# king159/Pair-Net

Measured on AMD Instinct MI355X. Metric: images/sec (whole node), 100-query 800x1333, 1/2/4/8 MI355X, higher is better.
Workload: dtype f32

## Files before the change

### include/pairnet_hip.h

```cpp
#ifndef PAIRNET_HIP_H_
#define PAIRNET_HIP_H_

#include <stdint.h>

#ifdef __cplusplus
extern "C" {
#endif

#define PN_ABI_VERSION 29
int pn_abi_version(void);

#define PN_GEMM_RELU       1
#define PN_GEMM_A_COLMAJOR 2
#define PN_GEMM_FORCE_TILE 4
#define PN_GEMM_FORCE_SKINNY 8
#define PN_GEMM_FORCE_TILE64 16
#define PN_GEMM_FORCE_TILE128x64 32
#define PN_GEMM_RELU_AFTER_RES 128
#define PN_GEMM_GELU 256
#define PN_GEMM_RESERVE_SHIFT 16
#define PN_GEMM_RESERVE(n) ((((n) / 8) & 0x3ff) << PN_GEMM_RESERVE_SHIFT)
#define PN_GEMM_KSPLIT_SHIFT 26
#define PN_GEMM_KSPLIT(n) (((n) & 31) << PN_GEMM_KSPLIT_SHIFT)

typedef struct pn_gemm_desc {
  const float* A;     int64_t lda;    int64_t strideA;
  const float* Aadd;  int64_t ldaadd; int32_t aadd_rows;
  int32_t aadd_from_col;
  const float* W;     int64_t ldw;    int64_t strideW;
  const float* bias;
  const float* Res;   int64_t ldres;  int64_t strideRes;
  float*       C;     int64_t ldc;    int64_t strideC;
  int32_t M, N, K, batch, flags;
  float* splitk_scratch;  int64_t splitk_scratch_floats;
} pn_gemm_desc;

int pn_gemm_f32(const pn_gemm_desc* d, void* stream);

int pn_gemm_group_f32(const pn_gemm_desc* d, int count, void* stream);

int pn_gemm_wgs_per_cu(void);

#define PN_GEMM_VARIANT_SKINNY        0
#define PN_GEMM_VARIANT_TILE_128x64   2
#define PN_GEMM_VARIANT_TILE_128x128  4
#define PN_GEMM_VARIANT_TILE_64x64    6
int pn_gemm_variant(const pn_gemm_desc* d);
int pn_gemm_grid_size(const pn_gemm_desc* d);

int pn_conv2d_nhwc_f32(const float* in, const float* Wp, const float* bias,
                       float* out, int B, int H, int W, int Cin, int Cout,
                       int KH, int KW, int pad, int relu, int flags , void* stream);

int pn_winograd_f23_input_f32(const float* in, float* V, int B, int H, int W, int C,
                              void* stream);
int pn_winograd_f23_output_f32(const float* M, const float* bias, float* out, int B, int H,
                               int W, int C, int relu, void* stream);
int pn_winograd_weights_f32(const float* w, float* U, int Co, int Ci, int form, void* stream);
int pn_winograd_f43_input_f32(const float* in, float* V, int B, int H, int W, int C,
                              void* stream);
int pn_winograd_f43_output_f32(const float* M, const float* bias, float* out, int B, int H,
                               int W, int C, int relu, void* stream);

int pn_conv2d_nhwc_ex_f32(const float* in, const float* Wp, const float* bias,
                          const float* res, float* out, int B, int H, int W, int Cin,
                          int Cout, int KH, int KW, int stride, int pad, int flags,
                          float* splitk_scratch ,
                          int64_t splitk_scratch_floats, void* stream);
int pn_stem7x7s2_f32(const float* img_nchw, const float* Wp, const float* bias,
                     float* out, int B, int H, int W, int flags ,
                     void* stream);
int pn_maxpool3x3s2_nhwc_f32(const float* in, float* out, int B, int H, int W, int C,
                             void* stream);

int pn_layernorm_f32(const float* x, const float* gamma, const float* beta,
                     float* y, int64_t rows, int C, float eps, void* stream);

int pn_layernorm_rows_f32(const float* x, int64_t ldx, const float* gamma, const float* beta,
                          float* y, int64_t ldy, int64_t rows, int C, float eps, void* stream);
int pn_layernorm_rows_s3_f32(const float* x, int64_t ldx, const float* gamma, const float* beta,
                             void* y_s3, int64_t rows, int C, float eps, void* stream);

int pn_patch_merge_ln_f32(const float* x, const float* gamma, const float* beta, float* y,
                          int B, int H, int W, int C, float eps, void* stream);

int pn_patch_im2col4_f32(const float* img, float* out, int B, int H, int W, void* stream);

int pn_window_attention_f32(const float* qkv, int64_t ldqkv, const float* qkv_bias,
                            const float* bias_table, float* out, int64_t ldo, int B, int H,
                            int W, int C, int heads, int ws, int shift, float scale,
                            void* stream);
int pn_window_attention_s3_f32(const float* qkv, int64_t ldqkv, const float* qkv_bias,
                               const float* bias_table, void* out_s3, int B, int H, int W, int C,
                               int heads, int ws, int shift, float scale, void* stream);

int pn_groupnorm_nblk(int64_t HW);
int pn_groupnorm_nhwc_f32(const float* x, const float* gamma, const float* beta,
                          float* y, double* partials, int B, int64_t HW, int C,
                          int G, float eps, int relu, int64_t x_bstride,
                          int64_t y_bstride, void* stream);

int pn_linear_res_ln_f32(const float* x, int64_t ldx, const float* W, int64_t ldw,
                         const float* bias , const float* res, int64_t ldres,
                         const float* gamma, const float* beta, float* y, int64_t ldy,
                         int M, int N, int K, float eps, void* stream);

int64_t pn_ffn_scratch_floats(int M, int hidden);
int pn_ffn_ln_f32(const float* x, const float* W1, const float* b1, const float* W2,
                  const float* b2, const float* gamma, const float* beta, float* y,
                  float* scratch, int M, int C, int hidden, float eps, void* stream);
int pn_ffn_ln2_f32(const float* x, const float* W1, const float* b1, const float* W2,
                   const float* b2, const float* gamma, const float* beta, float* y,
                   const float* gamma2, const float* beta2, float* y2, float* scratch, int M,
                   int C, int hidden, float eps, void* stream);

int pn_l2normalize_f32(const float* x, float* y, int64_t rows, int C, float eps,
                       void* stream);

int pn_msda_f32(const float* value, int64_t ld_value, const float* offaw,
                int64_t ld_offaw, float* out, int B, int L,
                const int32_t* level_h , const int32_t* level_w ,
                void* stream);
#define PN_MSDA_PERSISTENT 1
#define PN_MSDA_PERSISTENT_BATCHED 2
#define PN_MSDA_LOW_OCCUPANCY 4
#define PN_MSDA_S3_OUT 8
int pn_msda_ex_f32(const float* value, int64_t ld_value, const float* offaw,
                   int64_t ld_offaw, float* out, int B, int L,
                   const int32_t* level_h , const int32_t* level_w ,
                   int flags, void* stream);

int pn_msda_loc_f32(const float* value, int64_t ld_value, const int64_t* spatial_shapes,
                    const int64_t* level_start_index, const float* sampling_locations,
                    const float* attention_weights, float* out, int B, int N, int Nq, int L,
                    void* stream);

int pn_msda_bwd_f32(const float* value, int64_t ld_value, const int64_t* spatial_shapes,
                    const int64_t* level_start_index, const float* sampling_locations,
                    const float* attention_weights, const float* grad_output, float* grad_value,
                    float* grad_sampling_loc, float* grad_attn_weight, int B, int N, int Nq, int L,
                    void* stream);

int pn_gather_probe_f32(const float* lines, const int32_t* idx, float* out, int workgroups,
                        int line_mask, void* stream);

int pn_sine_pe_f32(float* out, const float* add, int h, int w, int C,
                   float temperature, void* stream);
int pn_sine_pe_offset_f32(float* out, const float* add, int h, int w, int C, float temperature,
                          float offset, void* stream);
int pn_sine_pe_valid_f32(float* out, const float* add, int h, int w, int valid_h, int valid_w,
                         int C, float temperature, float offset, void* stream);

int pn_bilinear_nhwc_f32(const float* in, float* out, int B, int hi, int wi,
                         int ho, int wo, int C, int accumulate, int64_t in_bstride,
                         int64_t out_bstride, void* stream);
int pn_bilinear_planar_f32(const float* in, float* out, int64_t P, int hi,
                           int wi, int ho, int wo, void* stream);
int pn_bilinear_stencil_rows_f32(const float* in, float* out, int B, int hi, int wi, int ho,
                                 int wo, int C, int64_t in_bstride, int64_t out_bstride,
                                 void* stream);
int pn_bilinear_planar_gt0_u8(const float* in, uint8_t* out, int64_t P, int hi,
                              int wi, int ho, int wo, void* stream);

int pn_mask_pack(const float* logits, uint32_t* bits, int32_t* rowall,
                 int64_t R, int Nk, void* stream);
int pn_mask_pack_stencil(const float* logits4, uint32_t* bits, int32_t* rowall, int64_t R,
                         int hi, int wi, int ho, int wo, void* stream);

int pn_mask_stencil_gemm_f32(const float* me, int64_t ld_me, int64_t stride_me, const float* rows,
                             int64_t ld_rows, int64_t stride_rows, uint32_t* bits,
                             int32_t* rowall, int B, int Q, int Nk, int K, int hi, int wi, int ho,
                             int wo, int flags, void* stream);

int64_t pn_attn_scratch_floats(int B, int Q, int Nk);
int pn_attention_f32(const float* q, int64_t ldq, const float* k, int64_t ldk,
                     const float* v, int64_t ldv, const uint32_t* maskbits,
                     const int32_t* rowall, float* out, int64_t ldo,
                     float* scratch, int B, int Q, int Nk, float scale,
                     void* stream);

int pn_mlearner_first_f32(const float* in, const float* w1, const float* b1,
                          float* out, int B, int S, int C, void* stream);
int pn_ppn_front_f32(const float* sub_embed, const float* obj_embed, const float* w1,
                     const float* b1, float* importance_raw, float* c1, int B, int Q, float eps,
                     void* stream);
int pn_mlearner_last_f32(const float* in, const float* w3, const float* b3,
                         float* out, int B, int S, int C, void* stream);

int pn_topk_pairs(const float* scores, int64_t* idx, int64_t* sub, int64_t* obj,
                  int64_t* pair, int B, int Q, int k, void* stream);
int pn_topk_f32(const float* scores, int64_t* idx, int64_t* quot, int64_t* rem, int B,
                int n, int div, int k, void* stream);
int pn_topk_strided_f32(const float* scores, int64_t elem_stride, int64_t row_stride,
                        int64_t* idx, int64_t* quot, int64_t* rem, int B, int n, int div, int k,
                        void* stream);

int pn_gather_rows_f32(const float* in, const int64_t* index, float* out, int B,
                       int rows_in, int rows_out, int64_t len, void* stream);

int pn_cls_argmax_f32(const float* logits, int64_t* label, float* score,
                      int64_t rows, int C, int label_offset, void* stream);
int pn_rel_dists_f32(const float* logits, float* out, int64_t rows, int C,
                     void* stream);
int pn_softmax_fg_f32(const float* logits, float* probs, float* fg, int64_t rows,
                      int C, void* stream);
int pn_row_argmax_f32(const float* x, int64_t* idx, int64_t rows, int n,
                      void* stream);
int pn_triplet_finish(const int64_t* s_label, const int64_t* o_label,
                      const float* probs, const int64_t* tri, const int64_t* rem,
                      int64_t* labels, int64_t* r_labels, float* r_scores,
                      float* r_dists, int k, int C, void* stream);
int pn_panoptic_f32(const float* masks, const int64_t* labels,
                    const int32_t* remap, int64_t* seg, int32_t* area, int n,
                    int64_t HW, void* stream);

int64_t pn_panoptic_state_bytes(void);
int pn_panoptic_device_f32(const float* masks, const int64_t* labels, const float* scores,
                           int Q, int num_classes, int hi, int wi, int ho, int wo,
                           void* state, float* up_scratch, int32_t* area_scratch,
                           int64_t* seg, int rounds, void* stream);
int pn_panoptic_continue_f32(void* state, const float* up_scratch, int32_t* area_scratch,
                             int64_t* seg, int ho, int wo, int rounds, void* stream);

int pn_pack_triplets_f32(const int64_t* labels, const float* r_dists, const int64_t* sub_pos,
                         const int64_t* obj_pos, float* rec, int R, int C1, void* stream);

int pn_copy_stream(const void* src, void* dst, int64_t bytes, int wgs, void* stream);

int pn_pack_bool_bits(const uint8_t* bools, uint8_t* bits, int64_t n, void* stream);
int pn_unpack_bits_host(const uint8_t* bits, uint8_t* bools, int64_t n, int threads);

int pn_pan_masks_u8(const uint8_t* rgb, const int* ids, const int* cats, uint8_t* masks, int* sem,
                    int G, int H, int W, void* stream);

int pn_preprocess_u8_f32(const uint8_t* img, int H, int W, float* out, int Hn, int Wn, int Hp,
                         int Wp, const float* mean3, const float* stdinv3, int to_rgb,
                         void* stream);

int pn_pack_mask_bits(const uint8_t* masks, uint64_t* words, int64_t rows, int64_t HW,
                      void* stream);
int pn_mask_iou_counts(const uint64_t* pred_words, int P, const uint64_t* gt_words, int G,
                       int64_t nwords, int32_t* inter, int32_t* area_pred, int32_t* area_gt,
                       void* stream);

int pn_pred_triplets(const int64_t* labels, const float* r_dists, int32_t* triplets,
                     float* scores, int R, int C1, void* stream);
int pn_mask_or_rows(const uint64_t* words, const int32_t* a, const int32_t* b, uint64_t* out,
                    int rows, int64_t nwords, void* stream);
int pn_triplet_match(const int32_t* pred_triplets, const int32_t* gt_triplets, int P, int G,
                     const int32_t* inter, const int32_t* area_pred, const int32_t* area_gt,
                     int ld_inter, const int32_t* pred_sub_row, const int32_t* pred_obj_row,
                     const int32_t* gt_sub_row, const int32_t* gt_obj_row, double iou_thr,
                     int phrdet, int ignore_rel, uint8_t* match, void* stream);
int pn_triplet_match_boxes(const int32_t* pred_triplets, const int32_t* gt_triplets, int P, int G,
                           const float* pred_boxes, int ld_pred, const float* gt_boxes, int ld_gt,
                           const int32_t* pred_sub_row, const int32_t* pred_obj_row,
                           const int32_t* gt_sub_row, const int32_t* gt_obj_row, float iou_thr,
                           int phrdet, int ignore_rel, uint8_t* match, void* stream);

int pn_zero_rows_f32(const float* x, const uint8_t* valid, float* out, int B, int64_t rows,
                     int C, int64_t ld, int64_t valid_bstride, void* stream);
int pn_sigmoid_f32(const float* x, float* y, int64_t n, void* stream);
int pn_box_pos_embed_f32(const float* unact, float* ref, float* emb, int64_t rows, void* stream);
int pn_box_sampling_f32(const float* offaw, int64_t ld, const float* ref,
                        const float* valid_ratios, int rows_per_image, float* loc, float* aw,
                        int64_t rows, int L, void* stream);
int pn_token_sampling_f32(const float* offaw, int64_t ld, const float* valid_ratios, float* loc,
                          float* aw, int B, int L, const int32_t* level_h, const int32_t* level_w,
                          void* stream);
int pn_box_refine_f32(const float* delta, const float* ref_in, float* ref_out, int64_t rows,
                      void* stream);
int pn_query_score_f32(const float* logits, float* score, int B, int Nq, int C, void* stream);
int pn_box_triplets_f32(const float* s_cls, const float* o_cls, const float* s_box,
                        const float* o_box, float* det, int64_t* labels, int R, int C,
                        float img_h, float img_w, const float* scale_factor, int rescale,
                        void* stream);

int pn_gt_mask_prepare_u8(const uint8_t* masks, uint8_t* out, int G, int h, int w, int H, int W,
                          int Ho, int Wo, void* stream);

int pn_point_sample_f32(const void* maps, int maps_are_u8, const float* pts, float* out, int P,
                        int h, int w, int Np, void* stream);
int pn_mask_match_cost_f32(const float* cls , int ncls,
                           const int64_t* gt_labels , const float* pred_pts ,
                           const float* gt_pts , float* cost, int Q, int G, int Np,
                           float w_cls, float w_mask, float w_dice, float dice_eps, void* stream);
int pn_id_match_cost_f32(const float* sub, const float* obj , const float* rel
                         , int ncls, int nrel, const int64_t* gt_sub,
                         const int64_t* gt_obj, const int64_t* gt_rel, float* cost, int R, int G,
                         float w_sub, float w_obj, float w_rel, void* stream);
int pn_ce_mean_f32(const float* logits, int64_t ld, const int64_t* target,
                   const float* class_weight , float* out, int rows, int C,
                   float loss_weight, void* stream);
int pn_seesaw_mean_f32(const float* logits, int64_t ld, const int64_t* target,
                       const float* cum_samples, float* out, int rows, int C, float p, float q,
                       float eps, float loss_weight, void* stream);
int pn_bce_posw_mean_f32(const float* logits, const float* target, float* out , int64_t n,
                         float loss_weight, void* stream);

int pn_ce_mean_grad_f32(const float* logits, int64_t ld, const int64_t* target,
                        const float* class_weight , float* grad, int64_t ldg,
                        int rows, int C, float loss_weight, void* stream);
int pn_seesaw_mean_grad_f32(const float* logits, int64_t ld, const int64_t* target,
                            const float* cum_samples, float* grad, int64_t ldg, int rows, int C,
                            float p, float q, float eps, float loss_weight, void* stream);
int pn_bce_posw_mean_grad_f32(const float* logits, const float* target, float* grad, int64_t n,
                              float loss_weight, void* stream);

int pn_transpose_f32(const float* in, int64_t ldi, float* out, int64_t ldo, int rows, int cols,
                     int out_cols, void* stream);
int pn_colsum_f32(const float* x, int64_t ld, float* out, int rows, int cols, int accumulate,
                  float* scratch, int64_t scratch_floats, void* stream);
int pn_relu_bwd_f32(const float* dy, const float* y, float* dx, int64_t n, void* stream);
int pn_add_periodic_f32(const float* a, const float* b, float* out, int64_t n, int64_t bn,
                        void* stream);
int pn_batch_sum_f32(const float* x, float* out, int B, int64_t n, int accumulate, void* stream);
int pn_layernorm256_bwd_f32(const float* dy, const float* x, const float* gamma, float* dx,
                            float* gxhat, int rows, float eps, void* stream);
int pn_mha_bwd_f32(const float* q, int64_t ldq, const float* k, int64_t ldk, const float* v,
                   int64_t ldv, const float* dout, int64_t ldo, float* dq, int64_t lddq, float* dk,
                   int64_t lddk, float* dv, int64_t lddv, const uint32_t* bits,
                   const int32_t* rowall, float* scratch, int B, int Nq, int Nk, float scale,
                   void* stream);
int pn_scatter_rows_add_f32(const float* src, int64_t ld_src, const int64_t* index, float* out,
                            int64_t ld_out, int B, int rows_out, int slots, int length,
// ... 65 lines not shown
```

### pair-net_amd/backbone.py

```python
from collections import OrderedDict

import torch

from . import hip
from . import plans
from .plans import Arena, PlanCache, measure_bytes

BLOCKS = {50: (3, 4, 6, 3), 101: (3, 4, 23, 3)}
EPS = 1e-5


def _stages(depth):
    return tuple(zip((64, 128, 256, 512), BLOCKS[depth]))


def _param_shapes(depth=50):
    STAGES = _stages(depth)
    s = OrderedDict()

    def bn(prefix, c):
        for n in ("weight", "bias", "running_mean", "running_var"):
            s["%s.%s" % (prefix, n)] = (c,)
        s[prefix + ".num_batches_tracked"] = ()

    s["conv1.weight"] = (64, 3, 7, 7)
    bn("bn1", 64)
    cin = 64
    for i, (planes, blocks) in enumerate(STAGES):
        for b in range(blocks):
            p = "layer%d.%d." % (i + 1, b)
            s[p + "conv1.weight"] = (planes, cin, 1, 1)
            bn(p + "bn1", planes)
            s[p + "conv2.weight"] = (planes, planes, 3, 3)
            bn(p + "bn2", planes)
            s[p + "conv3.weight"] = (planes * 4, planes, 1, 1)
            bn(p + "bn3", planes * 4)
            if b == 0:
                s[p + "downsample.0.weight"] = (planes * 4, cin, 1, 1)
                bn(p + "downsample.1", planes * 4)
            cin = planes * 4
    return s


class ResNet50Hip:

    def __init__(self, depth=50, **unused):
        if depth not in BLOCKS:
            raise NotImplementedError("bottleneck ResNets: depth 50 or 101")
        self.depth, self.stages = depth, _stages(depth)
        self._params = OrderedDict(
            (k, torch.zeros(shape, dtype=torch.int64 if k.endswith("tracked") else torch.float32))
            for k, shape in _param_shapes(depth).items())
        for k, v in self._params.items():
            if k.endswith(("running_var",)) or (k.endswith(".weight") and v.dim() == 1):
                v.fill_(1.0)
        g = torch.Generator().manual_seed(0)
        for k, v in self._params.items():
            if v.dim() == 4:
                fan_in = v.shape[1] * v.shape[2] * v.shape[3]
                v.copy_(torch.randn(v.shape, generator=g) * (2.0 / fan_in) ** 0.5)
        self.device, self.w, self._plans, self._arenas = None, None, PlanCache(), {}
        self.use_graphs = False
        self.graph_after = 1
        self.grid_reserve = 0
        self.conv_algo = "winograd4"
        self.wino_min_planes = 128
        self.s3_conv3_min_planes = 0

    def _weights_version(self):
        return sum(p._version for p in self._params.values())

    def parameters(self):
        return list(self._params.values())

    def state_dict(self):
        return OrderedDict((k, v.clone()) for k, v in self._params.items())

    def load_state_dict(self, sd, strict=True):
        missing = [k for k in self._params if k not in sd]
        unexpected = [k for k in sd if k not in self._params]
        if strict and (missing or unexpected):
            raise RuntimeError("state_dict mismatch: missing %s unexpected %s"
                               % (missing[:5], unexpected[:5]))
        for k, p in self._params.items():
            if k in sd:
                if tuple(sd[k].shape) != tuple(p.shape):
                    raise RuntimeError("shape mismatch for %s" % k)
                p.copy_(sd[k].detach().to(p.dtype).cpu())
        self.w, self._plans = None, PlanCache()
        return missing, unexpected

    def to(self, device):
        self.device, self.w, self._plans = torch.device(device), None, PlanCache()
        self._arenas = {}
        return self

    def eval(self):
        return self

    def _fold(self, conv, bn):
        P = self._params
        w = P[conv + ".weight"].double()
        s = P[bn + ".weight"].double() / torch.sqrt(P[bn + ".running_var"].double() + EPS)
        b = P[bn + ".bias"].double() - P[bn + ".running_mean"].double() * s
        w = (w * s.view(-1, 1, 1, 1)).float()
        return w, b.float()

    def _pack(self):
        if self.device is None or self.device.type != "cuda":
            raise RuntimeError("ResNet50Hip runs on an MI355X only: call .to('cuda:0'); there "
                               "is no CPU path")
        hip.lib()
        dev, w = self.device, {}
        cw, cb = self._fold("conv1", "bn1")
        stem = torch.zeros(64, 160)
        stem[:, :147] = cw.reshape(64, 147)
        w["stem.w"], w["stem.b"] = stem.to(dev), cb.to(dev)
        for i, (planes, blocks) in enumerate(self.stages):
            for b in range(blocks):
                p = "layer%d.%d." % (i + 1, b)
                for conv, bn in (("conv1", "bn1"), ("conv2", "bn2"), ("conv3", "bn3"),
                                 ("downsample.0", "downsample.1")):
                    if p + conv + ".weight" not in self._params:
                        continue
                    cw, cb = self._fold(p + conv, p + bn)
                    co = cw.shape[0]
                    w[p + conv + ".w"] = cw.permute(0, 2, 3, 1).reshape(co, -1).contiguous().to(dev)
                    w[p + conv + ".b"] = cb.to(dev)
                    if conv == "conv2" and co >= 64 and not (b == 0 and i > 0):
                        w[p + "conv2.wino"] = hip.winograd_weights(cw.to(dev))
                        w[p + "conv2.wino4"] = hip.winograd43_weights(cw.to(dev))
        for k in list(w):
            if k.endswith("conv3.w"):
                s3 = torch.empty(hip.s3_floats(*w[k].shape), device=dev, dtype=torch.float32)
                hip.s3_split(w[k], s3)
                w[k + ".s3"] = s3
        self.w = w
        self._packed_version = self._weights_version()

    class _Plan:

        def busy_events(self):
            out = []
            for st in self.streams.values():
                ev = torch.cuda.Event()
                ev.record(st)
                out.append(ev)
            return out

    def _arena(self, slot):
        a = self._arenas.get(slot)
        if a is None:
            a = self._arenas[slot] = Arena(self.device, on_grow=lambda a, s=slot: self._plans.drop(
                lambda k: k[3] == s))
        return a

    def _layout_for(self, dims):
        def layout(E):
            pl = ResNet50Hip._Plan()
            self._layout(pl, E, *dims)
            return pl
        return layout

    def _measure(self, dims):
        return measure_bytes(self._layout_for(dims))

    def reserve(self, batch, H, W, slots=(0,)):
        if self.w is None:
            self._pack()
        for s in slots:
            self._arena(s).reserve((batch, H, W), self._measure)

    def arena_bytes(self):
        return sum(a.capacity for a in self._arenas.values())

    @staticmethod
    def feature_shapes(H, W):
        h, w = (H - 1) // 2 + 1, (W - 1) // 2 + 1
        out = []
        for i in range(4):
            h, w = (h - 1) // 2 + 1, (w - 1) // 2 + 1
            out.append((h, w))
        return out

    def _plan(self, B, H, W, slot=0):
        key = (B, H, W, slot, self.conv_algo, self.wino_min_planes, self.s3_conv3_min_planes)
        if key in self._plans:
            return self._plans[key]
        if self.w is None:
            self._pack()

        dims = (B, H, W)
        pl = self._arena(slot).carve(self._layout_for(dims), dims, self._measure)
        pl.graph = pl.outs = pl.last_img = None
        pl.calls, pl.staged, pl.streams = 0, False, {}
        self._plans[key] = pl
        return pl

    def _layout(self, pl, E, B, H, W):
        pl.B = B
        pl.img = E(B, 3, H, W)
        h1, w1 = (H - 1) // 2 + 1, (W - 1) // 2 + 1
        h, wd = (h1 - 1) // 2 + 1, (w1 - 1) // 2 + 1
        pl.stem, pl.hw_stem = E(B, h1, w1, 64), (h1, w1)
        pl.pool = E(B, h, wd, 64)
        pl.scratch = E(B * 16 * 1024 * 1024 // 2)
        pl.hw, pl.out, pl.t1, pl.t2, pl.idt, pl.ping, pl.f43 = [], [], [], [], [], [], []
        nwino = 0
        for i, (planes, blocks) in enumerate(self.stages):
            hin, win = h, wd
            if i > 0:
                h, wd = (h - 1) // 2 + 1, (wd - 1) // 2 + 1
            pl.hw.append(((hin, win), (h, wd)))
            pl.t1.append(E(B, hin, win, planes))
            pl.t2.append(E(B, h, wd, planes))
            pl.idt.append(E(B, h, wd, planes * 4))
            pl.ping.append(E(B, h, wd, planes * 4))
            pl.out.append(E(B, h, wd, planes * 4))
            if planes >= self.wino_min_planes:
                t2, t4 = B * ((h + 1) // 2) * ((wd + 1) // 2), B * ((h + 3) // 4) * ((wd + 3) // 4)
                nwino = max(nwino, 16 * t2 * planes, 36 * t4 * planes)
                pl.f43.append(36 * (-(-t4 // 64)) < 16 * (-(-t2 // 64)))
            else:
                pl.f43.append(False)
        pl.wV, pl.wM = E(max(nwino, 4)), E(max(nwino, 4))
        pl.t2_s3 = E(max(hip.s3_floats(B * hw[1][0] * hw[1][1], planes)
                         for hw, (planes, _) in zip(pl.hw, self.stages)))

    @torch.no_grad()
    @hip.on_device
    def forward(self, img, slot=0):
        if not img.is_cuda or img.dtype != torch.float32 or img.dim() != 4 or img.shape[1] != 3:
            raise RuntimeError("img must be a [B,3,H,W] fp32 device tensor")
        if self.device is None:
            self.to(img.device)
        if self.w is not None and self._packed_version != self._weights_version():
            self.w, self._plans = None, PlanCache(self._plans.max_plans)
        img = img.contiguous()
        B, _, H, W = img.shape
        pl = self._plan(B, H, W, slot)
        if getattr(pl, "reserve", None) != self.grid_reserve:
            pl.reserve, pl.graph = self.grid_reserve, None
        cur = torch.cuda.current_stream(self.device)
        pl.streams[cur.cuda_stream] = cur
        try:
            return self._forward_on(img, pl, cur)
        finally:
            plans.note_use(cur)

    def _forward_on(self, img, pl, cur):
        if not self.use_graphs:
            return self._run(img, pl)
        ptr = img.data_ptr()
        if pl.graph is not None and not pl.staged and ptr != pl.static_img.data_ptr():
            pl.graph, pl.staged = None, True
        if pl.graph is None:
            if pl.calls < self.graph_after or not plans.quiet(cur):
                pl.calls += 1
                pl.last_img = ptr
                return self._run(img, pl)
            if not pl.staged and pl.last_img is not None and ptr != pl.last_img:
                pl.staged = True
            pl.static_img = pl.img if pl.staged else img
            pl.graph, pl.outs = self._capture(lambda: self._run(pl.static_img, pl))
        pl.last_img = ptr
        if pl.staged:
            pl.static_img.copy_(img)
        pl.graph.replay()
        return pl.outs

    @staticmethod
    def _capture(fn):
        from .head import CrossHead2
        box = {}
        g = CrossHead2._capture(lambda: box.update(out=fn()))
        return g, box["out"]

    def _run(self, img, pl):
        with hip.reserve_slots(self.grid_reserve):
            return self._run_layers(img, pl)

    def _run_layers(self, img, pl):
        B, _, H, W = img.shape
        w = self.w
        hip.stem7x7s2(img, w["stem.w"], w["stem.b"], pl.stem, B, H, W)
        hip.maxpool3x3s2(pl.stem, pl.pool, B, pl.hw_stem[0], pl.hw_stem[1], 64)
        x, cin = pl.pool, 64
        for i, (planes, blocks) in enumerate(self.stages):
            (hin, win), (h, wd) = pl.hw[i]
            for b in range(blocks):
                p = "layer%d.%d." % (i + 1, b)
                stride = 2 if (b == 0 and i > 0) else 1
                hi, wi = (hin, win) if b == 0 else (h, wd)
                t1 = pl.t1[i].view(-1)[:B * hi * wi * planes].view(B, hi, wi, planes)
                hip.linear(x.view(-1, cin), w[p + "conv1.w"], w[p + "conv1.b"],
                           t1.view(-1, planes), relu=True, scratch=pl.scratch)
                wino = self.conv_algo in ("winograd", "winograd4") and p + "conv2.wino" in w \
                    and stride == 1 and planes >= self.wino_min_planes
                if wino and self.conv_algo == "winograd4" and pl.f43[i]:
                    hip.conv3x3_winograd43(t1, w[p + "conv2.wino4"], w[p + "conv2.b"], pl.t2[i],
                                           pl.wV, pl.wM, B, hi, wi, planes, planes, True)
                elif wino:
                    hip.conv3x3_winograd(t1, w[p + "conv2.wino"], w[p + "conv2.b"], pl.t2[i],
                                         pl.wV, pl.wM, B, hi, wi, planes, planes, True)
                else:
                    hip.conv2d_ex(t1, w[p + "conv2.w"], w[p + "conv2.b"], None, pl.t2[i], B, hi,
                                  wi, planes, planes, 3, 3, stride, 1, relu=True,
                                  scratch=pl.scratch)
                if b == 0:
                    if stride == 1:
                        hip.linear(x.view(-1, cin), w[p + "downsample.0.w"],
                                   w[p + "downsample.0.b"], pl.idt[i].view(-1, planes * 4),
                                   scratch=pl.scratch)
                    else:
                        hip.conv2d_ex(x, w[p + "downsample.0.w"], w[p + "downsample.0.b"], None,
                                      pl.idt[i], B, hi, wi, cin, planes * 4, 1, 1, stride, 0,
                                      scratch=pl.scratch)
                    idt = pl.idt[i]
                else:
                    idt = x
                if b == blocks - 1:
                    dst = pl.out[i]
                else:
                    dst = pl.ping[i] if idt is not pl.ping[i] else pl.idt[i]
                if self.s3_conv3_min_planes and planes >= self.s3_conv3_min_planes:
                    t2 = pl.t2[i].view(-1, planes)
                    hip.s3_split(t2, pl.t2_s3)
                    hip.gemm_s3(pl.t2_s3, w[p + "conv3.w.s3"], t2.shape[0], planes * 4, planes,
                                bias=w[p + "conv3.b"], out=dst.view(-1, planes * 4),
                                res=idt.view(-1, planes * 4), relu_after=True)
                else:
                    hip.linear(pl.t2[i].view(-1, planes), w[p + "conv3.w"], w[p + "conv3.b"],
                               dst.view(-1, planes * 4), res=idt.view(-1, planes * 4),
                               relu_after=True, scratch=pl.scratch)
                x, cin = dst, planes * 4
        return tuple(o.permute(0, 3, 1, 2) for o in pl.out)

    __call__ = forward
```

### pair-net_amd/csrc/gemm.hip

```cpp
#include "common.h"
#include "gemm_common.h"

#ifndef PN_GEMM_WGS64
#define PN_GEMM_WGS64 5
#endif
#ifndef PN_GEMM_WGS128x64
#define PN_GEMM_WGS128x64 3
#endif
#ifndef PN_GEMM_BIGM_128x64
#define PN_GEMM_BIGM_128x64 0
#endif
#ifndef PN_GEMM_WGS64_SPILLING
#define PN_GEMM_WGS64_SPILLING 5
#endif

#ifndef PN_GEMM_LDS2
#define PN_GEMM_LDS2 0
#endif

template <int BM, int BN, int AMODE>
struct TileSmem {
  static constexpr int A_ELEMS = (AMODE == A_COL) ? 32 * (BM + 4) : BM * 36;
  static constexpr int STAGE = A_ELEMS + BN * 36;
  static constexpr int FLOATS = STAGE * (PN_GEMM_LDS2 ? 2 : 1);
};

#ifndef PN_GEMM_W2
#define PN_GEMM_W2 0
#endif
#ifndef PN_GEMM_W2_WGS
#define PN_GEMM_W2_WGS 8
#endif

template <int BM, int BN, int AMODE, bool ADD>
struct TileWgs {
  static constexpr int value =
      (BM * BN > 128 * 64) ? 2 : (BM * BN > 64 * 64) ? PN_GEMM_WGS128x64
      : ((AMODE == A_ROW && !ADD) || AMODE == A_CONV) ? PN_GEMM_WGS64 : PN_GEMM_WGS64_SPILLING;
  static constexpr int min_waves = (BM * BN <= 64 * 64 && value > 4) ? value : 1;
};

struct TileRef {
  int pi;
  int bz, tm, tn;
};

template <int BM, int BN, int WM, int WN, int AMODE, bool ADD, typename Locator, int EPI = 0>
__device__ __forceinline__ void gemm_persistent(const Locator& loc, const int ntiles,
                                                float* smem) {
  constexpr int BK = 32, LD = BK + 4;
  constexpr int WAVES_N = BN / WN;
  constexpr int TM = WM / 32, TN = WN / 32;
  constexpr int LDK = BM + 4;
  constexpr int A_ELEMS = TileSmem<BM, BN, AMODE>::A_ELEMS;
  constexpr int NT = 64 * (BM / WM) * WAVES_N;
  constexpr int RPP = NT / 8;
  constexpr int NA = (BM * BK / 4) / NT;
  constexpr int NB = (BN * BK / 4) / NT;
  constexpr int QM = BM / 4;
  constexpr int KSTEP = NT / QM;
  static_assert(NT == 128 || NT == 256 || NT == 512, "2, 4 or 8 waves");

  const int xcd = blockIdx.x & 7, slot = blockIdx.x >> 3, per = gridDim.x >> 3;
  const int q8 = ntiles >> 3, r8 = ntiles & 7;
  const int base = (xcd < r8) ? xcd * (q8 + 1) : r8 * (q8 + 1) + (xcd - r8) * q8;
  const int cnt = q8 + (xcd < r8 ? 1 : 0);
  if (slot >= cnt) return;

  const int tid = threadIdx.x, lane = tid & 63, wave = tid >> 6;
  const int li = lane & 31, lh = lane >> 5;
  const int wm = wave / WAVES_N, wn = wave % WAVES_N;
  const int kc = (tid & 7) * 4;
  float* const sA = smem;
  float* const sB = smem + A_ELEMS;

  int lpi = 0, lK = 0, lkt0 = 0;
  const float* bA = nullptr;
  const float* bW = nullptr;
  const float* bAdd = nullptr;
  __amdgpu_buffer_rsrc_t rA = make_rsrc(nullptr), rW = rA, rAdd = rA;
  unsigned a_off[NA], add_off[ADD ? NA : 1], w_off[NB];
  int cy[NA], cx[NA];
  unsigned a_tap[AMODE == A_CONV ? NA : 1];
  unsigned a_off1[AMODE == A_COL ? NA : 1][4];
  unsigned in_mask = 0;
  bool l_add = false;
  bool l_vec = false;
  auto set_tile = [&](const TileRef& tr) {
    const GemmP& p = loc.P(tr.pi);
    lpi = tr.pi;
    lK = p.K;
    const int m0 = tr.tm * BM, n0 = tr.tn * BN;
    const int ks = max(p.ksplit, 1);
    const int bb = tr.bz / ks;
    lkt0 = (tr.bz - bb * ks) * p.split_chunks;
    bA = p.A + (int64_t)bb * p.sA;
    bW = p.W + (int64_t)bb * p.sW;
    bAdd = p.Aadd ? p.Aadd : bA;
    rA = make_rsrc(bA);
    rW = make_rsrc(bW);
    if (ADD) rAdd = make_rsrc(bAdd);
    l_add = p.Aadd && n0 >= p.aadd_from_col;
    l_vec = p.a_vec && m0 + BM <= p.M;
    if (AMODE == A_COL) {
      const int mq = m0 + (tid % QM) * 4;
#pragma unroll
      for (int j = 0; j < NA; ++j) {
        const unsigned krow = (unsigned)(min(tid / QM + KSTEP * j, p.K - 1)) * (unsigned)p.lda;
        a_off[j] = (krow + (unsigned)min(mq, p.M - 1)) * 4u;
#pragma unroll
        for (int e = 0; e < 4; ++e) a_off1[j][e] = (krow + (unsigned)min(mq + e, p.M - 1)) * 4u;
      }
    } else {
#pragma unroll
      for (int j = 0; j < NA; ++j) {
        const int gm = min(m0 + (tid >> 3) + RPP * j, p.M - 1);
        if (AMODE == A_CONV) {
          const int oy = gm / p.Wo, ox = gm - oy * p.Wo;
          cy[j] = oy * p.stride;
          cx[j] = ox * p.stride;
          a_off[j] = ((unsigned)(cy[j] * p.Wd + cx[j]) * (unsigned)p.Cin + kc) * 4u;
        } else {
          a_off[j] = ((unsigned)gm * (unsigned)p.lda + kc) * 4u;
        }
        if (ADD) add_off[j] = ((unsigned)(p.Aadd ? gm % p.aadd_rows : gm) *
                                   (unsigned)(p.Aadd ? p.ldaadd : p.lda) + kc) * 4u;
      }
    }
    if constexpr (EPI == 1) {
      const StencilP& st = loc.st;
#pragma unroll
      for (int j = 0; j < NB; ++j) {
        const int c = (tid >> 3) + RPP * j;
        const int key = min(tr.tn * 16 + (c >> 5) * 8 + (c & 7), st.nk - 1);
        w_off[j] = ((unsigned)(((c >> 3) & 3) * st.nk + key) * (unsigned)p.ldw + kc) * 4u;
      }
    } else {
#pragma unroll
      for (int j = 0; j < NB; ++j)
        w_off[j] = ((unsigned)min(n0 + (tid >> 3) + RPP * j, p.N - 1) * (unsigned)p.ldw + kc) * 4u;
    }
  };

  float4 ra[NA], rad[ADD ? NA : 1], rb[NB];
  bool st_ragged = false, st_add = false;
  int st_k0 = 0;
  unsigned st_in = 0;
  auto load_chunk = [&](int kt) {
    const int k0 = (lkt0 + kt) * BK;
    const bool ragged = k0 + BK > lK;
    st_ragged = ragged;
    st_add = l_add;
    st_k0 = k0;
    if (AMODE == A_COL) {
      const GemmP& p = loc.P(lpi);
      const int soff = (ragged ? 0 : k0) * (int)p.lda * 4;
      if (l_vec) {
#pragma unroll
        for (int j = 0; j < NA; ++j) ra[j] = buf_ld4(rA, a_off[j], soff);
      } else {
#pragma unroll
        for (int j = 0; j < NA; ++j) {
          ra[j].x = buf_ld1(rA, a_off1[j][0], soff);
          ra[j].y = buf_ld1(rA, a_off1[j][1], soff);
          ra[j].z = buf_ld1(rA, a_off1[j][2], soff);
          ra[j].w = buf_ld1(rA, a_off1[j][3], soff);
        }
      }
    } else if (AMODE == A_CONV) {
      const GemmP& p = loc.P(lpi);
      const int tap = k0 / p.Cin;
      const int ci0 = k0 - tap * p.Cin;
      const int dy = tap / p.KW - p.pad, dx = tap % p.KW - p.pad;
      if (ci0 == 0 || kt == 0) {
        in_mask = 0;
        const int tap_off = (dy * p.Wd + dx) * p.Cin;
#pragma unroll
        for (int j = 0; j < NA; ++j) {
          const int yy = cy[j] + dy, xx = cx[j] + dx;
          const bool in = yy >= 0 && yy < p.H && xx >= 0 && xx < p.Wd;
          in_mask |= (in ? 1u : 0u) << j;
          a_tap[j] = a_off[j] + (unsigned)(in ? tap_off : 0) * 4u;
        }
      }
      st_in = in_mask;
#pragma unroll
      for (int j = 0; j < NA; ++j) ra[j] = buf_ld4(rA, a_tap[j], ci0 * 4);
    } else {
#pragma unroll
      for (int j = 0; j < NA; ++j) ra[j] = buf_ld4(rA, a_off[j], ragged ? 0 : k0 * 4);
      if (ADD) {
#pragma unroll
        for (int j = 0; j < NA; ++j)
          rad[j] = buf_ld4(rAdd, add_off[j], ragged ? 0 : k0 * 4);
      }
    }
#pragma unroll
    for (int j = 0; j < NB; ++j) rb[j] = buf_ld4(rW, w_off[j], ragged ? 0 : k0 * 4);
  };
  auto store_chunk = [&](const int so = 0) {
    float* const sA = smem + so;
    float* const sB = smem + so + A_ELEMS;
    const float4 zero4 = make_float4(0.f, 0.f, 0.f, 0.f);
#pragma unroll
    for (int j = 0; j < NA; ++j) {
      if (ADD && st_add) ra[j] = add4(ra[j], rad[j]);
      if (AMODE == A_CONV && !((st_in >> j) & 1u)) ra[j] = zero4;
    }
    if (st_ragged) {
      const GemmP& p = loc.P(lpi);
#pragma unroll
      for (int j = 0; j < NA; ++j) {
        if (AMODE == A_COL) {
          const int kk = st_k0 + tid / QM + KSTEP * j;
          const int mq = (int)(a_off1[j][0] / 4u) - (int)min(tid / QM + KSTEP * j, lK - 1) * (int)p.lda;
          float4 v = zero4;
          if (kk < lK) {
            const float* src = bA + (int64_t)kk * p.lda;
            v.x = src[min(mq + 0, p.M - 1)];
            v.y = src[min(mq + 1, p.M - 1)];
            v.z = src[min(mq + 2, p.M - 1)];
            v.w = src[min(mq + 3, p.M - 1)];
          }
          ra[j] = v;
        } else if (AMODE == A_ROW) {
          const bool ok = st_k0 + kc < lK;
          float4 v = ok ? ld4(bA + st_k0 + a_off[j] / 4u) : zero4;
          if (ADD && st_add && ok) v = add4(v, ld4(bAdd + st_k0 + add_off[j] / 4u));
          ra[j] = v;
        } else {
          ra[j] = zero4;
        }
      }
      (void)p;
#pragma unroll
      for (int j = 0; j < NB; ++j)
        rb[j] = st_k0 + kc < lK ? ld4(bW + st_k0 + w_off[j] / 4u) : zero4;
    }
    if (AMODE == A_COL) {
#pragma unroll
      for (int j = 0; j < NA; ++j)
        st4(sA + (tid / QM + KSTEP * j) * LDK + (tid % QM) * 4, ra[j]);
#pragma unroll
      for (int j = 0; j < NB; ++j) st4(sB + ((tid >> 3) + RPP * j) * LD + kc, rb[j]);
    } else {
#pragma unroll
      for (int j = 0; j < NA; ++j) st4(sA + ((tid >> 3) + RPP * j) * LD + kc, ra[j]);
#pragma unroll
      for (int j = 0; j < NB; ++j) st4(sB + ((tid >> 3) + RPP * j) * LD + kc, rb[j]);
    }
  };

  f32x16 acc[TM][TN];
  const float* fA0 = (AMODE == A_COL) ? sA + (4 * lh) * LDK + wm * WM + li
                                      : sA + (wm * WM + li) * LD + 4 * lh;
  const float* fB0 = sB + (wn * WN + li) * LD + 4 * lh;
  int rso = 0;
  auto read_frag = [&](int kb, float4 (&fa)[TM], float4 (&fb)[TN]) {
    const float* const fA = fA0 + rso;
    const float* const fB = fB0 + rso;
#pragma unroll
    for (int mi = 0; mi < TM; ++mi) {
      if (AMODE == A_COL) {
        const float* s = fA + (kb * 8) * LDK + mi * 32;
        fa[mi] = make_float4(s[0], s[LDK], s[2 * LDK], s[3 * LDK]);
      } else {
        fa[mi] = ld4(fA + mi * 32 * LD + kb * 8);
      }
    }
#pragma unroll
    for (int ni = 0; ni < TN; ++ni) fb[ni] = ld4(fB + ni * 32 * LD + kb * 8);
  };
  auto compute = [&]() {
    float4 fa[2][TM], fb[2][TN];
    read_frag(0, fa[0], fb[0]);
#pragma unroll
    for (int kb = 0; kb < BK / 8; ++kb) {
      const int cur = kb & 1;
      if (kb + 1 < BK / 8) read_frag(kb + 1, fa[cur ^ 1], fb[cur ^ 1]);
#pragma unroll
      for (int t = 0; t < 4; ++t)
#pragma unroll
        for (int mi = 0; mi < TM; ++mi)
#pragma unroll
          for (int ni = 0; ni < TN; ++ni) {
            const float4 av = fa[cur][mi], bv = fb[cur][ni];
            acc[mi][ni] = mfma32(t == 0 ? av.x : t == 1 ? av.y : t == 2 ? av.z : av.w,
                                 t == 0 ? bv.x : t == 1 ? bv.y : t == 2 ? bv.z : bv.w,
                                 acc[mi][ni]);
          }
    }
  };

  TileRef cur = loc(base + slot);
  set_tile(cur);
  load_chunk(0);
#if PN_GEMM_LDS2
  constexpr int STAGE = TileSmem<BM, BN, AMODE>::STAGE;
  int wso = 0;
  {
    const GemmP& p0 = loc.P(cur.pi);
    int nk0 = (p0.K + BK - 1) / BK;
    if (p0.ksplit > 1) nk0 = min(p0.split_chunks, nk0 - (cur.bz % p0.ksplit) * p0.split_chunks);
    store_chunk(0);
    wso = STAGE;
    if (nk0 > 1) {
      load_chunk(1);
    } else {
      set_tile(loc(base + min(slot + per, cnt - 1)));
      load_chunk(0);
    }
    __syncthreads();
  }
#endif
  for (int t = slot; t < cnt; t += per) {
    const GemmP& p = loc.P(cur.pi);
    const TileRef nxt = loc(base + min(t + per, cnt - 1));
    int nk = (p.K + BK - 1) / BK;
    if (p.ksplit > 1) {
      const int sidx = cur.bz % p.ksplit;
      nk = min(p.split_chunks, nk - sidx * p.split_chunks);
    }
#pragma unroll
    for (int mi = 0; mi < TM; ++mi)
#pragma unroll
      for (int ni = 0; ni < TN; ++ni)
#pragma unroll
        for (int r = 0; r < 16; ++r) acc[mi][ni][r] = 0.f;
#if PN_GEMM_LDS2
    for (int kt = 0; kt < nk; ++kt) {
      store_chunk(wso);
      if (kt + 2 < nk) {
        load_chunk(kt + 2);
      } else if (kt + 2 == nk) {
        set_tile(nxt);
        load_chunk(0);
      } else {
        const GemmP& pn = loc.P(nxt.pi);
        int nkn = (pn.K + BK - 1) / BK;
        if (pn.ksplit > 1) nkn = min(pn.split_chunks, nkn - (nxt.bz % pn.ksplit) * pn.split_chunks);
        if (nkn > 1) {
          load_chunk(1);
        } else {
          set_tile(loc(base + min(t + 2 * per, cnt - 1)));
          load_chunk(0);
        }
      }
      compute();
      __syncthreads();
      rso = wso;
      wso = STAGE - wso;
    }
#else
    for (int kt = 0; kt < nk; ++kt) {
      __syncthreads();
      store_chunk();
      __syncthreads();
      const bool last = kt + 1 == nk;
      if (last) set_tile(nxt);
      load_chunk(last ? 0 : kt + 1);
      compute();
    }
#endif
    const int m0 = cur.tm * BM, n0 = cur.tn * BN;
    if constexpr (EPI == 1) {
      const StencilP& st = loc.st;
      static_assert(EPI == 0 || (TM == 1 && TN == 1 && BN == 64), "stencil mode: 64x64 tiles of 32x32 waves");
      const int pl = li & 7;
      const int key0 = cur.tn * 16 + wn * 8;
      const int key = key0 + pl;
      const bool kvalid = key < st.nk;
      const int kk = min(key, st.nk - 1);
      const int oy = kk / st.wo, ox = kk - oy * st.wo;
      const Tap ty = make_tap(oy, st.hi, st.ho), tx = make_tap(ox, st.wi, st.wo);
      const int src = (lane & 32) | pl;
      const int nwords = (st.nk + 31) / 32;
      const int nvalid = min(max(st.nk - key0, 0), 8);
      const unsigned vm = (1u << nvalid) - 1u;
      const int rbase = m0 + wm * WM;
      const bool writer = li == 0;
      const bool last_tile = (cur.tn + 1) * 16 >= st.nk && wn == WAVES_N - 1;
#pragma unroll
      for (int r = 0; r < 16; ++r) {
        const float a = acc[0][0][r];
        const float v00 = __shfl(a, src, 64), v01 = __shfl(a, src + 8, 64);
        const float v10 = __shfl(a, src + 16, 64), v11 = __shfl(a, src + 24, 64);
        const float res = tap_blend(ty, tx, v00, v01, v10, v11);
        const unsigned long long bal = __ballot(kvalid && res < 0.f);
        const int row = rbase + mfma32_row(r, lh);
        if (writer && row < p.M) {
          const unsigned byte = (unsigned)(bal >> (32 * lh)) & 0xffu;
          const int64_t grow = (int64_t)cur.bz * p.M + row;
          unsigned char* bp = reinterpret_cast<unsigned char*>(st.bits + grow * nwords);
          bp[cur.tn * 2 + wn] = (unsigned char)byte;
          if (last_tile)
            for (int e = cur.tn * 2 + wn + 1; e < nwords * 4; ++e) bp[e] = 0;
          if (~byte & vm) st.rowall[grow] = 0;
        }
      }
      cur = nxt;
      continue;
    }
    float* __restrict__ C = p.C + (int64_t)cur.bz * p.sC;
    const float* __restrict__ Res = p.Res ? p.Res + (int64_t)cur.bz * p.sRes : nullptr;
    const bool full = m0 + BM <= p.M && n0 + BN <= p.N;
#pragma unroll
    for (int ni = 0; ni < TN; ++ni) {
      const int col = n0 + wn * WN + ni * 32 + li;
      const int colc = min(col, p.N - 1);
      const float bv = p.bias ? p.bias[colc] : 0.f;
#pragma unroll
      for (int mi = 0; mi < TM; ++mi) {
        const int rbase = m0 + wm * WM + mi * 32;
        float rv[16];
        if (Res) {
#pragma unroll
          for (int r = 0; r < 16; ++r)
            rv[r] = Res[(int64_t)min(rbase + mfma32_row(r, lh), p.M - 1) * p.ldres + colc];
        }
        float ov[16];
#pragma unroll
        for (int r = 0; r < 16; ++r) {
          float v = acc[mi][ni][r] + bv;
          v = gemm_act(v, p.relu);
          if (Res) v += rv[r];
          if (p.relu_after) v = fmaxf(v, 0.f);
          ov[r] = v;
        }
        float* cp = C + (int64_t)(rbase + 4 * lh) * p.ldc + col;
        if (full) {
#pragma unroll
          for (int r = 0; r < 16; ++r) cp[(int64_t)((r & 3) + 8 * (r >> 2)) * p.ldc] = ov[r];
        } else {
#pragma unroll
          for (int r = 0; r < 16; ++r)
            if (rbase + mfma32_row(r, lh) < p.M && col < p.N)
              cp[(int64_t)((r & 3) + 8 * (r >> 2)) * p.ldc] = ov[r];
        }
      }
    }
    cur = nxt;
  }
}

struct SingleLocator {
  const GemmP& p;
  int mt, nt;
  __device__ __forceinline__ const GemmP& P(int) const { return p; }
  __device__ __forceinline__ TileRef operator()(int T) const {
    const int per_b = mt * nt;
    const int bz = T / per_b, r = T - bz * per_b;
    const int tm = r / nt;
    return TileRef{0, bz, tm, r - tm * nt};
  }
};

template <int BM, int BN, int WM, int WN, int AMODE, bool ADD = false>
__global__ __launch_bounds__(64 * (BM / WM) * (BN / WN),
                             ((BM == 64 && WM == 64) ? PN_GEMM_W2_WGS / 2
                                                     : TileWgs<BM, BN, AMODE, ADD>::min_waves))
void k_gemm_tile(const GemmP p, const int batch) {
  __shared__ __attribute__((aligned(16))) float smem[TileSmem<BM, BN, AMODE>::FLOATS];
  const SingleLocator loc{p, (p.M + BM - 1) / BM, (p.N + BN - 1) / BN};
  gemm_persistent<BM, BN, WM, WN, AMODE, ADD>(loc, loc.mt * loc.nt * batch, smem);
}

__global__ __launch_bounds__(256) void k_fill_i32(int32_t* __restrict__ p, const int v, const int n) {
  const int i = blockIdx.x * 256 + threadIdx.x;
  if (i < n) p[i] = v;
}

struct StencilLocator {
  const GemmP& p;
  const StencilP& st;
  int mt, nt;
  __device__ __forceinline__ const GemmP& P(int) const { return p; }
  __device__ __forceinline__ TileRef operator()(int T) const {
    const int per_b = mt * nt;
    const int bz = T / per_b, r = T - bz * per_b;
    const int tm = r / nt;
    return TileRef{0, bz, tm, r - tm * nt};
  }
};

__global__ __launch_bounds__(256, (TileWgs<64, 64, A_ROW, false>::min_waves))
void k_gemm_stencil(const GemmP p, const StencilP st, const int batch) {
  __shared__ __attribute__((aligned(16))) float smem[TileSmem<64, 64, A_ROW>::FLOATS];
  const StencilLocator loc{p, st, (p.M + 63) / 64, (p.N + 63) / 64};
  gemm_persistent<64, 64, 32, 32, A_ROW, false, StencilLocator, 1>(loc, loc.mt * loc.nt * batch, smem);
}

#define GEMM_GROUP_MAX 18
struct GroupP {
  int n;
  int tile_start[GEMM_GROUP_MAX + 1];
  int mt[GEMM_GROUP_MAX], nt[GEMM_GROUP_MAX];
  GemmP p[GEMM_GROUP_MAX];
};

static_assert(sizeof(GroupP) <= 4096, "k_gemm_group's argument block must fit the kernarg segment");

struct GroupLocator {
  const GroupP& g;
  __device__ __forceinline__ const GemmP& P(int i) const { return g.p[i]; }
  __device__ __forceinline__ TileRef operator()(int T) const {
    int i = 0;
#pragma unroll
    for (int j = 1; j < GEMM_GROUP_MAX; ++j)
      if (j < g.n && T >= g.tile_start[j]) i = j;
    const int local = T - g.tile_start[i];
    const int per_b = g.mt[i] * g.nt[i];
    const int bz = local / per_b, r = local - bz * per_b;
    const int tm = r / g.nt[i];
    return TileRef{i, bz, tm, r - tm * g.nt[i]};
  }
};

__global__ __launch_bounds__(256, (TileWgs<64, 64, A_ROW, true>::min_waves)) void k_gemm_group(const GroupP g) {
  __shared__ __attribute__((aligned(16))) float smem[TileSmem<64, 64, A_ROW>::FLOATS];
  const GroupLocator loc{g};
  gemm_persistent<64, 64, 32, 32, A_ROW, true>(loc, g.tile_start[GEMM_GROUP_MAX], smem);
}

template <int AMODE, int NW>
__global__ __launch_bounds__(64 * NW) void k_gemm_skinny(const GemmP p) {
  __shared__ float red[NW * 1024];
  const int tid = threadIdx.x, lane = tid & 63, wave = tid >> 6;
  const int li = lane & 31, lh = lane >> 5;
  const int m0 = blockIdx.y * 32, n0 = blockIdx.x * 32, bz = blockIdx.z;
  const float* __restrict__ A = p.A + (int64_t)bz * p.sA;
  const float* __restrict__ W = p.W + (int64_t)bz * p.sW;
  const int am = min(m0 + li, p.M - 1);
  const int wn_ = min(n0 + li, p.N - 1);
  const float* arow = (AMODE == A_ROW) ? A + (int64_t)am * p.lda : A + am;
  const bool has_add = p.Aadd && n0 >= p.aadd_from_col;
  const float* addrow = has_add ? p.Aadd + (int64_t)(am % p.aadd_rows) * p.ldaadd : arow;
  const float* wrow = W + (int64_t)wn_ * p.ldw;

  int ks = (p.K + NW - 1) / NW;
  ks = (ks + 31) & ~31;
  const int kbeg = min(wave * ks, p.K), kend = min(kbeg + ks, p.K);

  auto load_chunk = [&](int kc, float4 (&a)[4], float4 (&b)[4]) {
    const float4 zero4 = make_float4(0.f, 0.f, 0.f, 0.f);
    const int k0 = min(kc + 4 * lh, p.K - 4), k1 = min(kc + 8 + 4 * lh, p.K - 4);
    const int k2 = min(kc + 16 + 4 * lh, p.K - 4), k3 = min(kc + 24 + 4 * lh, p.K - 4);
    const bool ok0 = kc + 4 * lh < kend, ok1 = kc + 8 + 4 * lh < kend;
    const bool ok2 = kc + 16 + 4 * lh < kend, ok3 = kc + 24 + 4 * lh < kend;
    const float4 w0 = ld4(wrow + k0), w1 = ld4(wrow + k1), w2 = ld4(wrow + k2), w3 = ld4(wrow + k3);
    float4 x0, x1, x2, x3;
    if (AMODE == A_ROW) {
      x0 = ld4(arow + k0); x1 = ld4(arow + k1); x2 = ld4(arow + k2); x3 = ld4(arow + k3);
      if (has_add) {
        const float4 d0 = ld4(addrow + k0), d1 = ld4(addrow + k1);
        const float4 d2 = ld4(addrow + k2), d3 = ld4(addrow + k3);
        x0 = add4(x0, d0); x1 = add4(x1, d1); x2 = add4(x2, d2); x3 = add4(x3, d3);
      }
    } else {
      const int64_t l = p.lda;
      x0 = make_float4(arow[k0 * l], arow[(k0 + 1) * l], arow[(k0 + 2) * l], arow[(k0 + 3) * l]);
      x1 = make_float4(arow[k1 * l], arow[(k1 + 1) * l], arow[(k1 + 2) * l], arow[(k1 + 3) * l]);
      x2 = make_float4(arow[k2 * l], arow[(k2 + 1) * l], arow[(k2 + 2) * l], arow[(k2 + 3) * l]);
      x3 = make_float4(arow[k3 * l], arow[(k3 + 1) * l], arow[(k3 + 2) * l], arow[(k3 + 3) * l]);
    }
    a[0] = ok0 ? x0 : zero4; a[1] = ok1 ? x1 : zero4; a[2] = ok2 ? x2 : zero4; a[3] = ok3 ? x3 : zero4;
    b[0] = ok0 ? w0 : zero4; b[1] = ok1 ? w1 : zero4; b[2] = ok2 ? w2 : zero4; b[3] = ok3 ? w3 : zero4;
  };
  f32x16 acc;
#pragma unroll
  for (int r = 0; r < 16; ++r) acc[r] = 0.f;
  auto mma_chunk = [&](const float4 (&a)[4], const float4 (&b)[4]) {
#pragma unroll
    for (int s = 0; s < 4; ++s) {
      acc = mfma32(a[s].x, b[s].x, acc);
      acc = mfma32(a[s].y, b[s].y, acc);
      acc = mfma32(a[s].z, b[s].z, acc);
      acc = mfma32(a[s].w, b[s].w, acc);
    }
  };

  float4 a0[4], b0[4], a1[4], b1[4];
  if (kbeg < kend) load_chunk(kbeg, a0, b0);
  for (int kc = kbeg; kc < kend; kc += 64) {
    const bool more1 = kc + 32 < kend;
    if (more1) load_chunk(kc + 32, a1, b1);
    mma_chunk(a0, b0);
    if (more1) {
      if (kc + 64 < kend) load_chunk(kc + 64, a0, b0);
      mma_chunk(a1, b1);
    }
  }
#pragma unroll
  for (int r = 0; r < 16; ++r) red[wave * 1024 + mfma32_row(r, lh) * 32 + li] = acc[r];
  __syncthreads();

  float* __restrict__ C = p.C + (int64_t)bz * p.sC;
  const float* __restrict__ Res = p.Res ? p.Res + (int64_t)bz * p.sRes : nullptr;
  for (int e = tid; e < 1024; e += 64 * NW) {
    const int row = m0 + (e >> 5), col = n0 + (e & 31);
    if (row < p.M && col < p.N) {
      float v = red[e];
#pragma unroll
      for (int w = 1; w < NW; ++w) v += red[w * 1024 + e];
      if (p.bias) v += p.bias[col];
      v = gemm_act(v, p.relu);
      if (Res) v += Res[(int64_t)row * p.ldres + col];
      if (p.relu_after) v = fmaxf(v, 0.f);
      C[(int64_t)row * p.ldc + col] = v;
    }
  }
}

#ifndef PN_SKINNY_NW256
#define PN_SKINNY_NW256 8
#endif
template <int AMODE>
static int launch_skinny(const GemmP& p, int batch, hipStream_t s) {
  dim3 grid(pn_cdiv(p.N, 32), pn_cdiv(p.M, 32), batch);
  if (p.K <= 128)
    hipLaunchKernelGGL((k_gemm_skinny<AMODE, 4>), grid, dim3(256), 0, s, p);
  else if (p.K <= 256)
    hipLaunchKernelGGL((k_gemm_skinny<AMODE, PN_SKINNY_NW256>), grid, dim3(64 * PN_SKINNY_NW256), 0, s, p);
  else
    hipLaunchKernelGGL((k_gemm_skinny<AMODE, 16>), grid, dim3(1024), 0, s, p);
  return PN_LAUNCH_CHECK();
}


static int cu_count() {
  static int cached[64] = {0};
  int dev = 0;
  if (hipGetDevice(&dev) != hipSuccess || dev < 0 || dev >= 64) return 256;
  if (cached[dev] == 0) {
    int n = 0;
    if (hipDeviceGetAttribute(&n, hipDeviceAttributeMultiprocessorCount, dev) != hipSuccess || n < 8)
      n = 256;
    cached[dev] = n;
  }
  return cached[dev];
}

static int persistent_grid(int64_t ntiles, int wg_per_cu, int flags) {
// ... 58 lines not shown
  c[0] = v.x; c[1] = v.y; c[2] = v.z; c[3] = v.w;
}

static int splitk_factor(const GemmP& p, int batch, const float* scratch, int64_t scratch_floats,
                         int* chunks_per_split, int flags) {
  const int nk = pn_cdiv(p.K, 32);
  const int64_t tiles = (int64_t)pn_cdiv(p.M, 64) * pn_cdiv(p.N, 64) * batch;
  *chunks_per_split = nk;
  const int forced = (flags >> PN_GEMM_KSPLIT_SHIFT) & 31;
  if (!scratch || (p.N & 3) || !aligned16(p.bias) || ((uintptr_t)scratch & 15) || forced == 1)
    return 1;
#ifdef PN_SPLITK_ROUND3
  if (!forced && (tiles >= 512 || nk < 8)) return 1;
  int S = forced ? forced : (int)((1024 + tiles - 1) / tiles);
  if (S > 16) S = 16;
  if (!forced && S > nk / 4) S = nk / 4;
#else
  if (!forced && (tiles >= 1024 || nk < 8)) return 1;
  int S = forced ? forced : (int)((1600 + tiles) / (2 * tiles));
  if (!forced) {
    if (S > 6) S = 6;
    const int min_chunks = tiles > 400 ? 16 : 8;
    if (S > nk / min_chunks) S = nk / min_chunks;
  }
  if (S > 16) S = 16;
#endif
  if (S > nk) S = nk;
  const int64_t per = (int64_t)batch * p.M * p.N;
  if ((int64_t)S * per > scratch_floats) S = (int)(scratch_floats / per);
  if (S < 2) return 1;
  const int cps = pn_cdiv(nk, S);
  *chunks_per_split = cps;
  return pn_cdiv(nk, cps);
}

template <int AMODE>
static int launch_tile64_splitk(const GemmP& p, int batch, float* scratch, int64_t scratch_floats,
                                hipStream_t s, int flags) {
  int cps;
  const int S = splitk_factor(p, batch, scratch, scratch_floats, &cps, flags);
#if PN_GEMM_W2
#define PN_T64_WM 64
#else
#define PN_T64_WM 32
#endif
  if (S <= 1) return launch_tile<64, 64, PN_T64_WM, 32, AMODE>(p, batch, s, flags);
  GemmP q = p;
  q.C = scratch; q.ldc = p.N; q.sC = (int64_t)p.M * p.N;
  q.bias = nullptr; q.Res = nullptr; q.relu = 0; q.relu_after = 0;
  q.ksplit = S; q.split_chunks = cps;
  if (int rc = launch_tile<64, 64, PN_T64_WM, 32, AMODE>(q, batch * S, s, flags)) return rc;
  const int64_t n = (int64_t)p.M * (p.N / 4);
  hipLaunchKernelGGL(k_splitk_reduce, dim3(pn_cdiv(n, 256), batch), dim3(256), 0, s, scratch, p, S);
  return PN_LAUNCH_CHECK();
}

static bool gemm_use_skinny(const pn_gemm_desc* d) {
  const int64_t tiles128 = (int64_t)pn_cdiv(d->M, 128) * pn_cdiv(d->N, 128) * d->batch;
  const int64_t tiles64 = (int64_t)pn_cdiv(d->M, 64) * pn_cdiv(d->N, 64) * d->batch;
  bool skinny = tiles128 < 96;
  if (d->splitk_scratch && tiles64 >= 64 && d->K >= 256 && !(d->N & 3)) skinny = false;
  if (d->flags & (PN_GEMM_FORCE_TILE | PN_GEMM_FORCE_TILE64 | PN_GEMM_FORCE_TILE128x64))
    skinny = false;
  if (d->flags & PN_GEMM_FORCE_SKINNY) skinny = true;
  if (d->K < 32) skinny = true;
  return skinny;
}

extern "C" int pn_gemm_variant(const pn_gemm_desc* d) {
  if (!d || d->M <= 0 || d->N <= 0 || d->batch <= 0) return PN_BAD_ARG;
  const int col = (d->flags & PN_GEMM_A_COLMAJOR) ? 1 : 0;
  if (gemm_use_skinny(d)) return PN_GEMM_VARIANT_SKINNY + col;
  if (d->flags & PN_GEMM_FORCE_TILE128x64) return PN_GEMM_VARIANT_TILE_128x64 + col;
  if (d->flags & PN_GEMM_FORCE_TILE) return PN_GEMM_VARIANT_TILE_128x128 + col;
  return PN_GEMM_VARIANT_TILE_64x64 + col;
}

int pn_fill_params(const pn_gemm_desc* d, GemmP* out) {
  if (!d || !d->A || !d->W || !d->C) return PN_BAD_ARG;
  if (d->M <= 0 || d->N <= 0 || d->K <= 0 || d->batch <= 0) return PN_BAD_ARG;
  const bool colmajor = d->flags & PN_GEMM_A_COLMAJOR;
  if (d->K % 4 || d->ldw % 4 || d->strideW % 4 || !aligned16(d->W)) return PN_BAD_ARG;
  if (!colmajor && (d->lda % 4 || d->strideA % 4 || !aligned16(d->A))) return PN_BAD_ARG;
  if (d->Aadd && (colmajor || d->ldaadd % 4 || !aligned16(d->Aadd) || d->aadd_rows <= 0))
    return PN_BAD_ARG;
  if (d->Aadd && (d->aadd_from_col < 0 || d->aadd_from_col % 64)) return PN_BAD_ARG;
  const int64_t lim = (int64_t)1 << 29;
  if (!colmajor && (int64_t)(d->M - 1) * d->lda + d->K >= lim) return PN_BAD_ARG;
  if (colmajor && (int64_t)(d->K - 1) * d->lda + d->M >= lim) return PN_BAD_ARG;
  if ((int64_t)(d->N - 1) * d->ldw + d->K >= lim) return PN_BAD_ARG;
  if (d->Aadd && (int64_t)d->aadd_rows * d->ldaadd >= lim) return PN_BAD_ARG;
  GemmP p{};
  p.A = d->A; p.Aadd = d->Aadd; p.W = d->W; p.bias = d->bias; p.Res = d->Res; p.C = d->C;
  p.lda = d->lda; p.ldaadd = d->ldaadd; p.ldw = d->ldw; p.ldres = d->ldres; p.ldc = d->ldc;
  p.sA = d->strideA; p.sW = d->strideW; p.sRes = d->strideRes; p.sC = d->strideC;
  p.M = d->M; p.N = d->N; p.K = d->K; p.aadd_rows = d->Aadd ? d->aadd_rows : 1;
  p.aadd_from_col = d->Aadd ? d->aadd_from_col : 0;
  p.relu = (d->flags & PN_GEMM_GELU) ? 2 : (d->flags & PN_GEMM_RELU) ? 1 : 0;
  p.relu_after = (d->flags & PN_GEMM_RELU_AFTER_RES) ? 1 : 0;
  p.a_vec = colmajor && d->lda % 4 == 0 && d->strideA % 4 == 0 && aligned16(d->A);
  *out = p;
  return 0;
}

extern "C" int pn_gemm_f32(const pn_gemm_desc* d, void* stream) {
  hipStream_t s = (hipStream_t)stream;
  GemmP p;
  if (int rc = pn_fill_params(d, &p)) return rc;
  const bool colmajor = d->flags & PN_GEMM_A_COLMAJOR;
  if (gemm_use_skinny(d)) {
    return colmajor ? launch_skinny<A_COL>(p, d->batch, s) : launch_skinny<A_ROW>(p, d->batch, s);
  }
  const bool big_m = PN_GEMM_BIGM_128x64 && !colmajor && !d->Aadd && d->M >= 16384 &&
                     d->N >= 256 && d->N % 64 == 0 && !(d->flags & PN_GEMM_FORCE_TILE64);
  if ((d->flags & PN_GEMM_FORCE_TILE128x64) || big_m)
    return colmajor ? launch_tile<128, 64, 64, 32, A_COL>(p, d->batch, s, d->flags)
                    : launch_tile<128, 64, 64, 32, A_ROW>(p, d->batch, s, d->flags);
  if (d->flags & PN_GEMM_FORCE_TILE)
    return colmajor ? launch_tile<128, 128, 64, 64, A_COL>(p, d->batch, s, d->flags)
                    : launch_tile<128, 128, 64, 64, A_ROW>(p, d->batch, s, d->flags);
  return colmajor ? launch_tile64_splitk<A_COL>(p, d->batch, d->splitk_scratch,
                                                d->splitk_scratch_floats, s, d->flags)
                  : launch_tile64_splitk<A_ROW>(p, d->batch, d->splitk_scratch,
                                                d->splitk_scratch_floats, s, d->flags);
}

extern "C" int pn_gemm_grid_size(const pn_gemm_desc* d) {
  if (!d || d->M <= 0 || d->N <= 0 || d->batch <= 0) return PN_BAD_ARG;
  const int64_t tiles = (int64_t)pn_cdiv(d->M, 64) * pn_cdiv(d->N, 64) * d->batch;
  return persistent_grid(tiles, TileWgs<64, 64, A_ROW, false>::value, d->flags);
}

extern "C" int pn_gemm_wgs_per_cu(void) { return TileWgs<64, 64, A_ROW, false>::value; }

extern "C" int pn_gemm_group_f32(const pn_gemm_desc* d, int count, void* stream) {
  if (!d || count <= 0 || count > GEMM_GROUP_MAX) return PN_BAD_ARG;
  GroupP g{};
  g.n = count;
  int tiles = 0;
  for (int i = 0; i < count; ++i) {
    if (d[i].flags & PN_GEMM_A_COLMAJOR) return PN_BAD_ARG;
    if (int rc = pn_fill_params(&d[i], &g.p[i])) return rc;
    g.tile_start[i] = tiles;
    g.mt[i] = pn_cdiv(d[i].M, 64);
    g.nt[i] = pn_cdiv(d[i].N, 64);
    tiles += g.mt[i] * g.nt[i] * d[i].batch;
  }
  for (int i = count; i <= GEMM_GROUP_MAX; ++i) g.tile_start[i] = tiles;
  hipLaunchKernelGGL(k_gemm_group, dim3(persistent_grid(tiles, TileWgs<64, 64, A_ROW, true>::value, d[0].flags)), dim3(256), 0,
                     (hipStream_t)stream, g);
  return PN_LAUNCH_CHECK();
}

extern "C" int pn_conv2d_nhwc_ex_f32(const float* in, const float* Wp, const float* bias,
                                     const float* res, float* out, int B, int H, int W,
                                     int Cin, int Cout, int KH, int KW, int stride, int pad,
                                     int flags, float* splitk_scratch,
                                     int64_t splitk_scratch_floats, void* stream) {
  if (!in || !Wp || !out || B <= 0 || H <= 0 || W <= 0 || stride <= 0 || pad < 0)
    return PN_BAD_ARG;
  if (Cin % 32 || !aligned16(in) || !aligned16(Wp)) return PN_BAD_ARG;
  if ((int64_t)H * W * Cin >= ((int64_t)1 << 29)) return PN_BAD_ARG;
  const int Ho = (H + 2 * pad - KH) / stride + 1, Wo = (W + 2 * pad - KW) / stride + 1;
  if (Ho <= 0 || Wo <= 0) return PN_BAD_ARG;
  GemmP p{};
  p.A = in; p.W = Wp; p.bias = bias; p.C = out; p.Res = res;
  p.M = Ho * Wo; p.N = Cout; p.K = KH * KW * Cin;
  p.lda = Cin; p.ldw = p.K; p.ldc = Cout; p.ldres = Cout;
  p.sA = (int64_t)H * W * Cin; p.sW = 0;
  p.sC = p.sRes = (int64_t)Ho * Wo * Cout;
  p.relu = (flags & PN_GEMM_RELU) ? 1 : 0;
  p.relu_after = (flags & PN_GEMM_RELU_AFTER_RES) ? 1 : 0;
  p.aadd_rows = 1;
  p.H = H; p.Wd = W; p.Cin = Cin; p.KW = KW; p.pad = pad; p.stride = stride; p.Wo = Wo;
  hipStream_t s = (hipStream_t)stream;
  if (flags & PN_GEMM_FORCE_TILE128x64) return launch_tile<128, 64, 64, 32, A_CONV>(p, B, s, flags);
  if (flags & PN_GEMM_FORCE_TILE) return launch_tile<128, 128, 64, 64, A_CONV>(p, B, s, flags);
  return launch_tile64_splitk<A_CONV>(p, B, splitk_scratch, splitk_scratch_floats, s, flags);
}

extern "C" int pn_conv2d_nhwc_f32(const float* in, const float* Wp, const float* bias,
                                  float* out, int B, int H, int W, int Cin, int Cout,
                                  int KH, int KW, int pad, int relu, int flags,
                                  void* stream) {
  if (KH != 2 * pad + 1 || KW != 2 * pad + 1) return PN_BAD_ARG;
  return pn_conv2d_nhwc_ex_f32(in, Wp, bias, nullptr, out, B, H, W, Cin, Cout, KH, KW, 1, pad,
                               (flags & ~PN_GEMM_RELU) | (relu ? PN_GEMM_RELU : 0), nullptr, 0,
                               stream);
}

extern "C" int pn_mask_stencil_gemm_f32(const float* me, int64_t ld_me, int64_t stride_me,
                                        const float* rows, int64_t ld_rows, int64_t stride_rows,
                                        uint32_t* bits, int32_t* rowall, int B, int Q, int Nk,
                                        int K, int hi, int wi, int ho, int wo, int flags,
                                        void* stream) {
  if (!me || !rows || !bits || !rowall || B <= 0 || Q <= 0 || Nk <= 0 || K <= 0 || K % 32)
    return PN_BAD_ARG;
  if (hi <= 0 || wi <= 0 || ho <= 0 || wo <= 0 || (int64_t)ho * wo != Nk) return PN_BAD_ARG;
  if (ld_me % 4 || ld_rows % 4 || stride_me % 4 || stride_rows % 4 || !aligned16(me) || !aligned16(rows))
    return PN_BAD_ARG;
  const int64_t lim = (int64_t)1 << 29;
  if ((int64_t)(Q - 1) * ld_me + K >= lim || ((int64_t)4 * Nk - 1) * ld_rows + K >= lim)
    return PN_BAD_ARG;
  GemmP p{};
  p.A = me; p.W = rows; p.lda = ld_me; p.ldw = ld_rows; p.sA = stride_me; p.sW = stride_rows;
  p.M = Q; p.K = K; p.aadd_rows = 1;
  p.N = pn_cdiv(Nk, 16) * 64;
  const StencilP st{bits, rowall, Nk, hi, wi, ho, wo};
  hipStream_t s = (hipStream_t)stream;
  hipLaunchKernelGGL(k_fill_i32, dim3(pn_cdiv(B * Q, 256)), dim3(256), 0, s, rowall, 1, B * Q);
  const int64_t ntiles = (int64_t)pn_cdiv(Q, 64) * (p.N / 64) * B;
  static const int wgs = resident_wgs(k_gemm_stencil, TileWgs<64, 64, A_ROW, false>::value, 256);
  hipLaunchKernelGGL(k_gemm_stencil, dim3(persistent_grid(ntiles, wgs, flags)), dim3(256), 0, s, p, st, B);
  return PN_LAUNCH_CHECK();
}

extern "C" int pn_abi_version(void) { return PN_ABI_VERSION; }
```

### pair-net_amd/csrc/norm.hip

```cpp
#include "common.h"

__global__ __launch_bounds__(256) void k_layernorm256(const float* __restrict__ x,
                                                       const float* __restrict__ g,
                                                       const float* __restrict__ b,
                                                       float* __restrict__ y,
                                                       int64_t rows, float eps) {
  const int lane = threadIdx.x & 63;
  const int64_t row = (int64_t)blockIdx.x * 4 + (threadIdx.x >> 6);
  if (row >= rows) return;
  const float4 v = ld4(x + row * 256 + lane * 4);
  const float4 gg = ld4(g + lane * 4), bb = ld4(b + lane * 4);
  st4(y + row * 256 + lane * 4, ln256_row(v, gg, bb, eps));
}

extern "C" int pn_layernorm_f32(const float* x, const float* gamma, const float* beta,
                                float* y, int64_t rows, int C, float eps, void* stream) {
  if (!x || !gamma || !beta || !y || C != 256 || rows <= 0) return PN_BAD_ARG;
  hipLaunchKernelGGL(k_layernorm256, dim3(pn_cdiv(rows, 4)), dim3(256), 0,
                     (hipStream_t)stream, x, gamma, beta, y, rows, eps);
  return PN_LAUNCH_CHECK();
}

#define GN_PIX 256
#define GN_SUB 16

extern "C" int pn_groupnorm_nblk(int64_t HW) { return pn_cdiv(HW, GN_PIX); }

__global__ __launch_bounds__(64 * GN_SUB) void k_gn_partial(const float* __restrict__ x,
                                                            double* __restrict__ partials,
                                                            int64_t HW, int G, int64_t xbs) {
  __shared__ double red[GN_SUB][64][2];
  const int tid = threadIdx.x, c4 = tid & 63, sub = tid >> 6;
  const int b = blockIdx.y;
  const int64_t p0 = (int64_t)blockIdx.x * GN_PIX;
  const float* xb = x + (int64_t)b * xbs;
  constexpr int NP = GN_PIX / GN_SUB;
  float4 v[NP];
#pragma unroll
  for (int j = 0; j < NP; ++j)
    v[j] = ld4(xb + min(p0 + sub + j * GN_SUB, HW - 1) * 256 + c4 * 4);
  double s = 0.0, ss = 0.0;
#pragma unroll
  for (int j = 0; j < NP; ++j) {
    if (p0 + sub + j * GN_SUB < HW) {
      s += ((double)v[j].x + (double)v[j].y) + ((double)v[j].z + (double)v[j].w);
      ss += ((double)v[j].x * v[j].x + (double)v[j].y * v[j].y) +
            ((double)v[j].z * v[j].z + (double)v[j].w * v[j].w);
    }
  }
  red[sub][c4][0] = s;
  red[sub][c4][1] = ss;
  __syncthreads();
  const int lanes_per_group = (256 / G) / 4;
  if (tid < G * 2) {
    const int g = tid >> 1, which = tid & 1;
    double t = 0.0;
    for (int l = 0; l < lanes_per_group; ++l)
      for (int k = 0; k < GN_SUB; ++k) t += red[k][g * lanes_per_group + l][which];
    partials[(((int64_t)b * gridDim.x + blockIdx.x) * G + g) * 2 + which] = t;
  }
}

__global__ __launch_bounds__(64 * GN_SUB) void k_gn_apply(const float* __restrict__ x,
                                                          const float* __restrict__ gamma,
                                                          const float* __restrict__ beta,
                                                          float* __restrict__ y,
                                                          const double* __restrict__ partials,
                                                          int64_t HW, int G, float eps, int relu,
                                                          int64_t xbs, int64_t ybs) {
  __shared__ double acc[GN_SUB][64];
  __shared__ float stat[64][2];
  const int tid = threadIdx.x, b = blockIdx.y;
  const int nblk = gridDim.x;
  {
    const int col = tid & 63, part = tid >> 6;
    double t = 0.0;
    if (col < 2 * G)
      for (int i = part; i < nblk; i += GN_SUB)
        t += partials[((int64_t)b * nblk + i) * G * 2 + col];
    acc[part][col] = t;
  }
  __syncthreads();
  if (tid < G) {
    const double n = (double)HW * (256 / G);
    double s = 0.0, ss = 0.0;
    for (int k = 0; k < GN_SUB; ++k) {
      s += acc[k][2 * tid];
      ss += acc[k][2 * tid + 1];
    }
    const double mean = s / n;
    double var = ss / n - mean * mean;
    if (var < 0.0) var = 0.0;
    stat[tid][0] = (float)mean;
    stat[tid][1] = (float)(1.0 / sqrt(var + (double)eps));
  }
  __syncthreads();
  const int c4 = tid & 63, sub = tid >> 6;
  const int g = (c4 * 4) / (256 / G);
  const float mean = stat[g][0], rstd = stat[g][1];
  const float4 gg = ld4(gamma + c4 * 4), bb = ld4(beta + c4 * 4);
  const int64_t p0 = (int64_t)blockIdx.x * GN_PIX;
  const float* xb = x + (int64_t)b * xbs;
  float* yb = y + (int64_t)b * ybs;
  constexpr int NP = GN_PIX / GN_SUB;
  float4 v[NP];
#pragma unroll
  for (int j = 0; j < NP; ++j)
    v[j] = ld4(xb + min(p0 + sub + j * GN_SUB, HW - 1) * 256 + c4 * 4);
#pragma unroll
  for (int j = 0; j < NP; ++j) {
    const int64_t pix = p0 + sub + j * GN_SUB;
    float4 o = make_float4((v[j].x - mean) * rstd * gg.x + bb.x, (v[j].y - mean) * rstd * gg.y + bb.y,
                           (v[j].z - mean) * rstd * gg.z + bb.z, (v[j].w - mean) * rstd * gg.w + bb.w);
    if (relu) {
      o.x = fmaxf(o.x, 0.f); o.y = fmaxf(o.y, 0.f);
      o.z = fmaxf(o.z, 0.f); o.w = fmaxf(o.w, 0.f);
    }
    if (pix < HW) st4(yb + pix * 256 + c4 * 4, o);
  }
}

extern "C" int pn_groupnorm_nhwc_f32(const float* x, const float* gamma, const float* beta,
                                     float* y, double* partials, int B, int64_t HW, int C,
                                     int G, float eps, int relu, int64_t x_bstride,
                                     int64_t y_bstride, void* stream) {
  if (!x || !gamma || !beta || !y || !partials) return PN_BAD_ARG;
  if (C != 256 || G <= 0 || G > 32 || 256 % G || (256 / G) % 4 || B <= 0 || HW <= 0)
    return PN_BAD_ARG;
  if ((x_bstride | y_bstride) & 3) return PN_BAD_ARG;
  hipStream_t s = (hipStream_t)stream;
  dim3 grid(pn_groupnorm_nblk(HW), B);
  hipLaunchKernelGGL(k_gn_partial, grid, dim3(64 * GN_SUB), 0, s, x, partials, HW, G, x_bstride);
  hipLaunchKernelGGL(k_gn_apply, grid, dim3(64 * GN_SUB), 0, s, x, gamma, beta, y, partials, HW, G,
                     eps, relu, x_bstride, y_bstride);
  return PN_LAUNCH_CHECK();
}

__global__ __launch_bounds__(256) void k_l2norm256(const float* __restrict__ x,
                                                   float* __restrict__ y, int64_t rows,
                                                   float eps) {
  const int lane = threadIdx.x & 63;
  const int64_t row = (int64_t)blockIdx.x * 4 + (threadIdx.x >> 6);
  if (row >= rows) return;
  const float4 v = ld4(x + row * 256 + lane * 4);
  const float n = sqrtf(wave_sum((v.x * v.x + v.y * v.y) + (v.z * v.z + v.w * v.w)));
  const float d = fmaxf(n, eps);
  st4(y + row * 256 + lane * 4, make_float4(v.x / d, v.y / d, v.z / d, v.w / d));
}

extern "C" int pn_l2normalize_f32(const float* x, float* y, int64_t rows, int C, float eps,
                                  void* stream) {
  if (!x || !y || C != 256 || rows <= 0) return PN_BAD_ARG;
  hipLaunchKernelGGL(k_l2norm256, dim3(pn_cdiv(rows, 4)), dim3(256), 0, (hipStream_t)stream,
                     x, y, rows, eps);
  return PN_LAUNCH_CHECK();
}
```

### pair-net_amd/head.py

```python
import math
from collections import OrderedDict

import torch

from . import hip
from . import plans
from .plans import Arena, PlanCache, measure_bytes
from .config import ConfigDict

INSTANCE_OFFSET = 1000


def _decoder_param_shapes(prefix, num_layers, ffn_dim, out):
    for i in range(num_layers):
        p = "%s.layers.%d." % (prefix, i)
        for a in (0, 1):
            out[p + "attentions.%d.attn.in_proj_weight" % a] = (768, 256)
            out[p + "attentions.%d.attn.in_proj_bias" % a] = (768,)
            out[p + "attentions.%d.attn.out_proj.weight" % a] = (256, 256)
            out[p + "attentions.%d.attn.out_proj.bias" % a] = (256,)
        out[p + "ffns.0.layers.0.0.weight"] = (ffn_dim, 256)
        out[p + "ffns.0.layers.0.0.bias"] = (ffn_dim,)
        out[p + "ffns.0.layers.1.weight"] = (256, ffn_dim)
        out[p + "ffns.0.layers.1.bias"] = (256,)
        for n in range(3):
            out[p + "norms.%d.weight" % n] = (256,)
            out[p + "norms.%d.bias" % n] = (256,)
    out[prefix + ".post_norm.weight"] = (256,)
    out[prefix + ".post_norm.bias"] = (256,)


class CrossHead2:

    RELATION_ORDER = ("cross_attn", "norm", "self_attn", "norm", "ffn", "norm")
    POST_ENTRIES = 8

    def __init__(self, num_classes, in_channels, num_relations, num_obj_query=100,
                 num_rel_query=100, mapper="conv_tiny", use_mask=True, pixel_decoder=None,
                 transformer_decoder=None, feat_channels=256, out_channels=256,
                 num_transformer_feat_level=3, embed_dims=256, relation_decoder=None,
                 enforce_decoder_input_project=False, n_heads=8,
                 positional_encoding=dict(type="SinePositionalEncoding", num_feats=128,
                                          normalize=True),
                 rel_cls_loss=None, subobj_cls_loss=None, importance_match_loss=None,
                 loss_cls=None, loss_mask=None, loss_dice=None, train_cfg=None,
                 test_cfg=dict(max_per_img=100), init_cfg=None, **kwargs):
        pixel_decoder = ConfigDict(pixel_decoder)
        transformer_decoder = ConfigDict(transformer_decoder)
        relation_decoder = ConfigDict(relation_decoder)
        if mapper != "conv_tiny":
            raise NotImplementedError("only mapper='conv_tiny' (configs/mask2former/pairnet.py:26)")
        self._loss_cfg = dict(train_cfg=train_cfg, rel_cls_loss=rel_cls_loss,
                              subobj_cls_loss=subobj_cls_loss,
                              importance_match_loss=importance_match_loss)
        self._loss = None
        assert "num_feats" in positional_encoding
        assert positional_encoding["num_feats"] * 2 == embed_dims
        enc_attn = pixel_decoder.encoder.transformerlayers.attn_cfgs
        assert enc_attn.num_levels == num_transformer_feat_level
        if (feat_channels, out_channels, embed_dims, n_heads) != (256, 256, 256, 8):
            raise NotImplementedError("kernels are built for 256 channels, 8 heads")
        if transformer_decoder.transformerlayers.attn_cfgs.num_heads != 8 or enforce_decoder_input_project:
            raise NotImplementedError("8-head decoder without input projection only")
        if (enc_attn.num_heads, enc_attn.num_points, enc_attn.embed_dims) != (8, 4, 256):
            raise NotImplementedError("MSDeformAttn kernel: 8 heads, 4 points")
        for dec, want in ((transformer_decoder, CrossHead2.RELATION_ORDER),
                          (relation_decoder, self.RELATION_ORDER)):
            got = tuple(dec.transformerlayers.get("operation_order", want))
            if got != want:
                raise NotImplementedError("operation_order %s (built for %s)" % (got, want))
        self.num_classes = num_classes
        self.num_relations = num_relations
        self.num_obj_query = self.num_queries = num_obj_query
        self.num_rel_query = num_rel_query
        self.use_mask = use_mask
        self.n_heads = self.num_heads = n_heads
        self.embed_dims = embed_dims
        self.in_channels = list(in_channels)
        self.num_transformer_feat_level = num_transformer_feat_level
        self.num_enc_layers = pixel_decoder.encoder.num_layers
        self.enc_ffn = pixel_decoder.encoder.transformerlayers.ffn_cfgs.feedforward_channels
        self.gn_groups = pixel_decoder.norm_cfg.num_groups
        self.num_dec_layers = transformer_decoder.num_layers
        self.dec_ffn = transformer_decoder.transformerlayers.ffn_cfgs.feedforward_channels
        self.num_rel_layers = relation_decoder.num_layers
        self.rel_ffn = relation_decoder.transformerlayers.ffn_cfgs.feedforward_channels
        self.test_cfg, self.train_cfg = test_cfg, train_cfg
        assert len(self.in_channels) == 4 and num_transformer_feat_level == 3
        assert num_obj_query <= 256 and num_rel_query <= 128
        self._params = OrderedDict(
            (k, torch.zeros(s)) for k, s in self.param_shapes().items())
        self.device = None
        self.w = None
        self._plans = PlanCache()
        self._arenas, self._post_arenas, self._consts, self._pe = {}, {}, {}, OrderedDict()
        self._dummies = {}
        self._post = OrderedDict()
        self._pan_jobs = []
        self.graph_after = 1
        self.exact_mask_order = True
        self.conv_algo = "winograd4"
        self.use_graphs = False
        self.grid_reserve = 0
        self.fuse_ppn_front = True
        self.fuse_mask_pack = True
        self.enc_fused_ln = ("proj", "ffn")
        self.group_input_convs = False
        self.gemm_arithmetic = "bf16x3"
        self.msda_s3_out = False
        self.init_weights()

    def param_shapes(self):
        s = OrderedDict()
        Q, R = self.num_obj_query, self.num_rel_query
        _decoder_param_shapes("relation_decoder", self.num_rel_layers, self.rel_ffn, s)
        s["rel_query_embed.weight"] = (R, 256)
        s["rel_query_embed2.weight"] = (2 * R, 256)
        s["rel_query_embed3.weight"] = (2 * R, 256)
        s["rel_query_feat.weight"] = (R, 256)
        for i, (ci, co) in enumerate(((1, 64), (64, 64), (64, 1))):
            s["update_importance.conv_layers.%d.0.weight" % i] = (co, ci, 7, 7)
            s["update_importance.conv_layers.%d.0.bias" % i] = (co,)
        pd = "pixel_decoder."
        for i in range(3):
            cin = self.in_channels[3 - i]
            s[pd + "input_convs.%d.conv.weight" % i] = (256, cin, 1, 1)
            s[pd + "input_convs.%d.conv.bias" % i] = (256,)
            s[pd + "input_convs.%d.gn.weight" % i] = (256,)
            s[pd + "input_convs.%d.gn.bias" % i] = (256,)
        for i in range(self.num_enc_layers):
            p = pd + "encoder.layers.%d." % i
            for name, n in (("sampling_offsets", 192), ("attention_weights", 96),
                            ("value_proj", 256), ("output_proj", 256)):
                s[p + "attentions.0.%s.weight" % name] = (n, 256)
                s[p + "attentions.0.%s.bias" % name] = (n,)
            s[p + "ffns.0.layers.0.0.weight"] = (self.enc_ffn, 256)
            s[p + "ffns.0.layers.0.0.bias"] = (self.enc_ffn,)
            s[p + "ffns.0.layers.1.weight"] = (256, self.enc_ffn)
            s[p + "ffns.0.layers.1.bias"] = (256,)
            for n in range(2):
                s[p + "norms.%d.weight" % n] = (256,)
                s[p + "norms.%d.bias" % n] = (256,)
        s[pd + "level_encoding.weight"] = (3, 256)
        s[pd + "lateral_convs.0.conv.weight"] = (256, self.in_channels[0], 1, 1)
        s[pd + "lateral_convs.0.gn.weight"] = (256,)
        s[pd + "lateral_convs.0.gn.bias"] = (256,)
        s[pd + "output_convs.0.conv.weight"] = (256, 256, 3, 3)
        s[pd + "output_convs.0.gn.weight"] = (256,)
        s[pd + "output_convs.0.gn.bias"] = (256,)
        s[pd + "mask_feature.weight"] = (256, 256, 1, 1)
        s[pd + "mask_feature.bias"] = (256,)
        _decoder_param_shapes("transformer_decoder", self.num_dec_layers, self.dec_ffn, s)
        s["query_embed.weight"] = (Q, 256)
        s["query_feat.weight"] = (Q, 256)
        s["level_embed.weight"] = (3, 256)
        s["cls_embed.weight"] = (self.num_classes + 1, 256)
        s["cls_embed.bias"] = (self.num_classes + 1,)
        for mlp in ("mask_embed", "sub_query_update", "obj_query_update"):
            for j in (0, 2, 4):
                s["%s.%d.weight" % (mlp, j)] = (256, 256)
                s["%s.%d.bias" % (mlp, j)] = (256,)
        s["rel_cls_embed.weight"] = (self.num_relations, 256)
        s["rel_cls_embed.bias"] = (self.num_relations,)
        return s

    def init_weights(self, seed=0):
        g = torch.Generator().manual_seed(seed)
        U = lambda shape, b: (torch.rand(shape, generator=g) * 2 - 1) * b
        N = lambda shape, std: torch.randn(shape, generator=g) * std
        for k, p in self._params.items():
            shape = tuple(p.shape)
            leaf = k.rsplit(".", 1)[-1]
            in_decoder = k.startswith(("transformer_decoder.", "relation_decoder.",
                                       "pixel_decoder.encoder."))
            if ".norms." in k or ".gn." in k or "post_norm" in k:
                v = torch.ones(shape) if leaf == "weight" else torch.zeros(shape)
            elif len(shape) == 1:
                wshape = self._params[k[:-len("bias")] + "weight"].shape
                fan_in = 1
                for d in wshape[1:]:
                    fan_in *= d
                v = torch.zeros(shape) if ("in_proj" in k or "out_proj" in k) \
                    else U(shape, 1.0 / math.sqrt(fan_in))
            elif in_decoder:
                fan_out, fan_in = shape[0], shape[1]
                v = N(shape, math.sqrt(2.0 / (fan_in + fan_out)))
            elif k.endswith(("query_embed.weight", "query_feat.weight", "query_embed2.weight",
                             "query_embed3.weight", "level_embed.weight",
                             "level_encoding.weight")):
                v = N(shape, 1.0)
            else:
                fan_in = 1
                for d in shape[1:]:
                    fan_in *= d
                v = U(shape, 1.0 / math.sqrt(fan_in))
            p.copy_(v)
        thetas = torch.arange(8, dtype=torch.float32) * (2.0 * math.pi / 8)
        grid = torch.stack([thetas.cos(), thetas.sin()], -1)
        grid = (grid / grid.abs().max(-1, keepdim=True)[0]).view(8, 1, 1, 2).repeat(1, 3, 4, 1)
        for i in range(4):
            grid[:, :, i, :] *= i + 1
        for i in range(self.num_enc_layers):
            p = "pixel_decoder.encoder.layers.%d.attentions.0." % i
            self._params[p + "sampling_offsets.weight"].zero_()
            self._params[p + "sampling_offsets.bias"].copy_(grid.reshape(-1))
            self._params[p + "attention_weights.weight"].zero_()
            self._params[p + "attention_weights.bias"].zero_()
            for n in ("value_proj", "output_proj"):
                self._params[p + n + ".weight"].copy_(U((256, 256), math.sqrt(6.0 / 512)))
                self._params[p + n + ".bias"].zero_()
        self._drop_weight_state()

    def _drop_weight_state(self):
        self.w = None
        self._plans = PlanCache(self._plans.max_plans)
        self._consts, self._pe = {}, OrderedDict()

    def _weights_version(self):
        return sum(p._version for p in self._params.values())

    def parameters(self):
        return list(self._params.values())

    def state_dict(self):
        return OrderedDict((k, v.clone()) for k, v in self._params.items())

    def load_state_dict(self, sd, strict=True):
        missing = [k for k in self._params if k not in sd]
        unexpected = [k for k in sd if k not in self._params]
        if strict and (missing or unexpected):
            raise RuntimeError("state_dict mismatch: missing %s unexpected %s"
                               % (missing[:5], unexpected[:5]))
        for k, p in self._params.items():
            if k in sd:
                if tuple(sd[k].shape) != tuple(p.shape):
                    raise RuntimeError("shape mismatch for %s: %s vs %s"
                                       % (k, tuple(sd[k].shape), tuple(p.shape)))
                p.copy_(sd[k].detach().to(torch.float32).cpu())
        self._drop_weight_state()
        return missing, unexpected

    def eval(self):
        return self

    def to(self, device):
        self.device = torch.device(device)
        self._drop_weight_state()
        self._arenas, self._post_arenas = {}, {}
        self._post.clear()
        return self

    def cuda(self, index=0):
        return self.to("cuda:%d" % index)

    def _pack(self):
        if self.device is None or self.device.type != "cuda":
            raise RuntimeError("CrossHead2 runs on an MI355X only: call .to('cuda:0'); "
                               "there is no CPU path")
# ... 146 lines not shown
                self._post_arena(s).reserve(
                    (batch, max(h * w for h, w in orig_sizes)),
                    lambda d: measure_bytes(lambda E: self._post_layout(E, [(1, d[1])] * d[0])))

    def arena_bytes(self):
        return sum(a.capacity for t in (self._arenas, self._post_arenas) for a in t.values())

    def _plan(self, B, shapes, hw2, slot=0, nhwc=False):
        key = (B, tuple(shapes), tuple(hw2), slot, getattr(self, "return_all_layers", False),
               nhwc)
        if key in self._plans:
            return self._plans[key]
        if self.w is None:
            self._pack()

        dims = self._plan_dims(B, shapes, hw2)
        pl = self._arena(slot).carve(self._layout_for(dims, nhwc), dims, self._measure)
        pl.slot, pl.key = slot, key
        pl.graph_a = pl.graph_b = pl.static_feats = pl.graph_cfg = pl.feats_read = None
        pl.graph_c = PlanCache(self.POST_VIEWS)
        pl.post_views = OrderedDict()
        pl.static_ptrs = None
        pl.graphs_a = OrderedDict()
        pl.calls_a = pl.calls_b = 0
        pl.streams = {}
        pl.enc_pos, pl.dec_kpos, pl.pe_ready, pl.enc_pos8 = self._position_tables(shapes)
        pl.pe_waited = False
        c = self._const(B)
        if c["me0"] is None:
            from types import SimpleNamespace
            BQ = B * self.num_obj_query
            tmp = SimpleNamespace(B=B, cls=None, MP=None,
                                  **{n: torch.empty(BQ, 256, device=self.device)
                                     for n in ("qn", "m1", "m2", "me")})
            self._head_embed(pl.q0, tmp, False, False)
            c["me0"] = tmp.me
            torch.cuda.current_stream(self.device).synchronize()
        pl.me0 = c["me0"]
        self._plans[key] = pl
        return pl

    def _layout(self, pl, E, B, shapes, hw2, nhwc):
        pl.B, pl.shapes, pl.hw2, pl.nhwc = B, list(shapes), tuple(hw2), nhwc
        pl.N = [h * w for h, w in shapes]
        pl.start = [0, pl.N[0], pl.N[0] + pl.N[1]]
        pl.SN = sum(pl.N)
        SN, Q, R = pl.SN, self.num_obj_query, self.num_rel_query
        HW2 = hw2[0] * hw2[1]
        pl.HW2 = HW2
        M = B * SN
        pl.X, pl.X1, pl.Y = E(B, SN, 256), E(B, SN, 256), E(B, SN, 256)
        pl.S = E(B, SN, 256)
        pl.VOA = E(B, SN, 544)
        pl.H = E(M, self.enc_ffn)
        pl.XS, pl.XPS = E(hip.s3_floats(M, 256)), E(hip.s3_floats(M, 256))
        pl.SS, pl.X1S = E(hip.s3_floats(M, 256)), E(hip.s3_floats(M, 256))
        pl.HS = E(hip.s3_floats(M, self.enc_ffn))
        pl.tmpconv = E(B, max(pl.N), 256)
        pl.splitk = E(B * 9 * 1024 * 1024)
        nblk = max(hip.groupnorm_nblk(HW2), hip.groupnorm_nblk(max(pl.N)))
        pl.gn_part = E.f64(B * nblk * 32 * 2)
        pl.T1, pl.T2 = E(B, HW2, 256), E(B, HW2, 256)
        pl.tmpconv3 = None
        if sum(pl.N) <= HW2:
            t1 = pl.T1.view(-1)
            offs = [0, B * pl.N[0] * 256, B * (pl.N[0] + pl.N[1]) * 256]
            pl.tmpconv3 = [t1[o:o + B * n * 256].view(B, n, 256) for o, n in zip(offs, pl.N)]
        pl.wino = hw2[0] % 2 == 0 and hw2[1] % 2 == 0
        t4 = B * ((hw2[0] + 3) // 4) * ((hw2[1] + 3) // 4)
        t2 = B * ((hw2[0] + 1) // 2) * ((hw2[1] + 1) // 2)
        n = max(16 * t2, 36 * t4) * 256
        pl.wV, pl.wM = E(n), E(n)
        pl.MF = E(B, HW2, 256)
        nd = self.num_dec_layers
        pl.Kp = [E(B, pl.N[i % 3], 256) for i in range(nd)]
        pl.Vp = [E(B, pl.N[i % 3], 256) for i in range(nd)]
        BQ = B * Q
        pl.q, pl.q1, pl.q2, pl.qy = E(BQ, 256), E(BQ, 256), E(BQ, 256), E(BQ, 256)
        pl.q0 = self._const(B)["q0"]
        pl.qn, pl.m1, pl.m2, pl.me = E(BQ, 256), E(BQ, 256), E(BQ, 256), E(BQ, 256)
        pl.Qp, pl.att, pl.Qp0 = E(BQ, 256), E(BQ, 256), E(BQ, 256)
        pl.VQK = E(BQ, 768)
        pl.MFd = [E(B, n, 256) for n in pl.N]
        pl.MFs = [E(B, 4 * n, 256) for n in pl.N]
        pl.ML4 = E(BQ, 4 * max(pl.N))
        pl.hq = E(hip.ffn_scratch_floats(BQ, self.dec_ffn))
        pl.MP = E(B, Q, HW2)
        pl.ML = E(BQ, max(pl.N))
        pl.bits = E.i32(BQ * ((max(pl.N) + 31) // 32))
        pl.rowall = E.i32(BQ)
        pl.cls = E(B, Q, self.num_classes + 1)
        self._plan_relation(pl, E)

    def _plan_relation(self, pl, E):
        B, Q, R = pl.B, self.num_obj_query, self.num_rel_query
        BQ, HW2 = B * Q, pl.HW2
        scr = max(hip.attn_scratch_floats(B, Q, n) for n in pl.N + [Q])
        scr = max(scr, hip.attn_scratch_floats(B, R, 2 * R), hip.attn_scratch_floats(B, R, R))
        pl.scr = E(scr)
        pl.s1, pl.s2, pl.sn, pl.on = E(BQ, 256), E(BQ, 256), E(BQ, 256), E(BQ, 256)
        pl.imp_raw, pl.imp = E(B, Q, Q), E(B, Q, Q)
        pl.c1, pl.c2 = E(B, Q * Q, 64), E(B, Q * Q, 64)
        tiles = B * ((Q * Q + 63) // 64)
        pl.ppn_splitk = E(8 * B * Q * Q * 64) if tiles < 512 else None
        pl.topk_idx, pl.sub_pos, pl.obj_pos = E.i64(B, R), E.i64(B, R), E.i64(B, R)
        pl.pair_idx = E.i64(B, 2 * R)
        pl.pair = E(B * 2 * R, 256)
        BR = B * R
        pl.r, pl.r1, pl.r2, pl.ry = E(BR, 256), E(BR, 256), E(BR, 256), E(BR, 256)
        pl.r0 = self._const(B).get("r0")
        pl.rQp, pl.ratt = E(BR, 256), E(BR, 256)
        pl.rVQK = E(BR, 768)
        pl.rh = E(hip.ffn_scratch_floats(BR, self.rel_ffn))
        pl.pVK = E(B * 2 * R, 512)
        pl.pVK_all = [E(B * 2 * R, 512) for _ in range(self.num_rel_layers)]
        pl.rQp0 = None
        pl.rel = E(B, R, self.num_relations)
        pl.sub_cls, pl.obj_cls = E(B, R, self.num_classes + 1), E(B, R, self.num_classes + 1)
        pl.sub_seg, pl.obj_seg = E(B, R, HW2), E(B, R, HW2)

    def _pixel_decoder(self, feats, pl):
        w, B, SN = self.w, pl.B, pl.SN
        pd = "pixel_decoder."
        group = self.group_input_convs and pl.nhwc and pl.tmpconv3 is not None
        if group:
            hip.gemm_group([dict(
                A=feats[3 - l], W=w[pd + "input_convs.%d.conv.weight" % l], C=pl.tmpconv3[l],
                M=pl.N[l], N=256, K=feats[3 - l].shape[1], lda=feats[3 - l].shape[1],
                ldw=feats[3 - l].shape[1], ldc=256, bias=w[pd + "input_convs.%d.conv.bias" % l],
                batch=B, sA=feats[3 - l].shape[1] * pl.N[l], sC=pl.N[l] * 256) for l in range(3)])
        for l in range(3):
            f = feats[3 - l]
            cin, n = f.shape[1], pl.N[l]
            conv = pl.tmpconv3[l] if group else pl.tmpconv
            if not group:
                hip.gemm(f, w[pd + "input_convs.%d.conv.weight" % l], conv, M=n, N=256, K=cin,
                         lda=cin if pl.nhwc else n, ldw=cin, ldc=256,
                         bias=w[pd + "input_convs.%d.conv.bias" % l], batch=B, sA=cin * n,
                         sC=n * 256, colmajor=not pl.nhwc, scratch=pl.splitk)
            hip.groupnorm_nhwc(conv, w[pd + "input_convs.%d.gn.weight" % l],
                               w[pd + "input_convs.%d.gn.bias" % l], pl.X[:, pl.start[l]:],
                               pl.gn_part, B, n, self.gn_groups, False, n * 256, SN * 256)
        X2, X12, Y2 = pl.X.view(-1, 256), pl.X1.view(-1, 256), pl.Y.view(-1, 256)
        if self.gemm_arithmetic == "bf16x3":
            self._encoder_s3(pl)
        else:
            self._encoder_fp32(pl)
        f = feats[0]
        cin, HW2 = f.shape[1], pl.HW2
        H2, W2 = pl.hw2
        hip.gemm(f, w[pd + "lateral_convs.0.conv.weight"], pl.T1, M=HW2, N=256, K=cin,
                 lda=cin if pl.nhwc else HW2, ldw=cin, ldc=256, batch=B, sA=cin * HW2,
                 sC=HW2 * 256, colmajor=not pl.nhwc)
        hip.groupnorm_nhwc(pl.T1, w[pd + "lateral_convs.0.gn.weight"],
                           w[pd + "lateral_convs.0.gn.bias"], pl.T2, pl.gn_part, B, HW2,
                           self.gn_groups, False, HW2 * 256, HW2 * 256)
        h2, w2 = pl.shapes[2]
        hip.bilinear_nhwc(pl.X[:, pl.start[2]:], pl.T2, B, h2, w2, H2, W2, 256, True, SN * 256,
                          HW2 * 256)
        if self.conv_algo == "winograd4":
            hip.conv3x3_winograd43(pl.T2, w[pd + "output_convs.0.conv.winograd4"], None, pl.T1,
                                   pl.wV, pl.wM, B, H2, W2, 256, 256, False)
        elif pl.wino and self.conv_algo == "winograd":
            hip.conv3x3_winograd(pl.T2, w[pd + "output_convs.0.conv.winograd"], None, pl.T1,
                                 pl.wV, pl.wM, B, H2, W2, 256, 256, False)
        else:
            hip.conv2d_nhwc(pl.T2, w[pd + "output_convs.0.conv.weight"], None, pl.T1, B, H2, W2,
                            256, 256, 3, 3, 1, False)
        hip.groupnorm_nhwc(pl.T1, w[pd + "output_convs.0.gn.weight"],
                           w[pd + "output_convs.0.gn.bias"], pl.T2, pl.gn_part, B, HW2,
                           self.gn_groups, True, HW2 * 256, HW2 * 256)
        hip.linear(pl.T2.view(-1, 256), w[pd + "mask_feature.weight"], w[pd + "mask_feature.bias"],
                   pl.MF.view(-1, 256))
        if not self.exact_mask_order:
            for l, (h, wd) in enumerate(pl.shapes):
                hip.bilinear_nhwc(pl.MF, pl.MFd[l], B, H2, W2, h, wd, 256, False, HW2 * 256,
                                  pl.N[l] * 256)
        elif self.exact_mask_order != "full":
            for l, (h, wd) in enumerate(pl.shapes):
                hip.bilinear_stencil_rows(pl.MF, pl.MFs[l], B, H2, W2, h, wd, 256, HW2 * 256,
                                          4 * pl.N[l] * 256)

    def _encoder_fp32(self, pl):
        w, B, SN = self.w, pl.B, pl.SN
        pd = "pixel_decoder."
        X2, X12, Y2 = pl.X.view(-1, 256), pl.X1.view(-1, 256), pl.Y.view(-1, 256)
        for i in range(self.num_enc_layers):
            p = pd + "encoder.layers.%d." % i
            a = p + "attentions.0."
            hip.gemm(X2, w[a + "voa.weight"], pl.VOA, M=B * SN, N=544, K=256, lda=256, ldw=256,
                     ldc=544, bias=w[a + "voa.bias"], aadd=pl.enc_pos, ldaadd=256, aadd_rows=SN,
                     aadd_from_col=256)
            hip.msda(pl.VOA, 544, pl.VOA.view(-1)[256:], 544, pl.S, B, pl.shapes)
            if "proj" in self.enc_fused_ln:
                hip.linear_res_ln(pl.S.view(-1, 256), w[a + "output_proj.weight"],
                                  w[a + "output_proj.bias"], X2, w[p + "norms.0.weight"],
                                  w[p + "norms.0.bias"], X12)
            else:
                hip.linear(pl.S.view(-1, 256), w[a + "output_proj.weight"],
                           w[a + "output_proj.bias"], Y2, res=X2)
                hip.layernorm(Y2, w[p + "norms.0.weight"], w[p + "norms.0.bias"], X12)
            hip.linear(X12, w[p + "ffns.0.layers.0.0.weight"], w[p + "ffns.0.layers.0.0.bias"],
                       pl.H, relu=True)
            if "ffn" in self.enc_fused_ln:
                hip.linear_res_ln(pl.H, w[p + "ffns.0.layers.1.weight"],
                                  w[p + "ffns.0.layers.1.bias"], X12, w[p + "norms.1.weight"],
                                  w[p + "norms.1.bias"], X2)
            else:
                hip.linear(pl.H, w[p + "ffns.0.layers.1.weight"], w[p + "ffns.0.layers.1.bias"],
                           Y2, res=X12)
                hip.layernorm(Y2, w[p + "norms.1.weight"], w[p + "norms.1.bias"], X2)

    def _encoder_s3(self, pl):
        w, B, SN = self.w, pl.B, pl.SN
        pd = "pixel_decoder."
        M, F = B * SN, self.enc_ffn
        X2 = pl.X.view(-1, 256)
        pos8 = (pl.enc_pos8, SN)
        hip.s3_split(X2, pl.XS)
        hip.s3_split(X2, pl.XPS, add=pl.enc_pos)
        for i in range(self.num_enc_layers):
            p = pd + "encoder.layers.%d." % i
            a = p + "attentions.0."
            last = i + 1 == self.num_enc_layers
            hip.gemm_s3(pl.XS, w[a + "voa.weight.s3"], M, 544, 256, bias=w[a + "voa.bias"],
                        out=pl.VOA.view(-1, 544), a2=pl.XPS, a2_from_col=256)
            if self.msda_s3_out:
                hip.msda(pl.VOA, 544, pl.VOA.view(-1)[256:], 544, pl.SS, B, pl.shapes, s3_out=True)
            else:
                hip.msda(pl.VOA, 544, pl.VOA.view(-1)[256:], 544, pl.S, B, pl.shapes)
                hip.s3_split(pl.S.view(-1, 256), pl.SS)
            hip.gemm_s3(pl.SS, w[a + "output_proj.weight.s3"], M, 256, 256,
                        bias=w[a + "output_proj.bias"], out_s3=pl.X1S, res_s3=pl.XS,
                        gamma=w[p + "norms.0.weight"], beta=w[p + "norms.0.bias"])
            hip.gemm_s3(pl.X1S, w[p + "ffns.0.layers.0.0.weight.s3"], M, F, 256,
                        bias=w[p + "ffns.0.layers.0.0.bias"], relu=True, out_s3=pl.HS)
            hip.gemm_s3(pl.HS, w[p + "ffns.0.layers.1.weight.s3"], M, 256, F,
                        bias=w[p + "ffns.0.layers.1.bias"], res_s3=pl.X1S,
                        gamma=w[p + "norms.1.weight"], beta=w[p + "norms.1.bias"],
                        out=X2 if last else None, out_s3=None if last else pl.XS,
                        out_s3_pos=None if last else pl.XPS, pos=pos8)

    def _mlp3(self, prefix, src, dst, pl):
        w = self.w
        hip.linear(src, w[prefix + ".0.weight"], w[prefix + ".0.bias"], pl.m1, relu=True)
        hip.linear(pl.m1, w[prefix + ".2.weight"], w[prefix + ".2.bias"], pl.m2, relu=True)
        hip.linear(pl.m2, w[prefix + ".4.weight"], w[prefix + ".4.bias"], dst)

    def _mask_logits(self, me, pl, out):
        Q = self.num_obj_query
        hip.gemm(me, pl.MF, out, M=Q, N=pl.HW2, K=256, lda=256, ldw=256, ldc=pl.HW2,
                 batch=pl.B, sA=Q * 256, sW=pl.HW2 * 256, sC=Q * pl.HW2)

    def _head_embed(self, q, pl, with_cls, full_mask, cls_out=None, mp_out=None, normed=False):
        w, B, Q = self.w, pl.B, self.num_obj_query
        cls_out = pl.cls if cls_out is None else cls_out
        mp_out = pl.MP if mp_out is None else mp_out
        if not normed:
            hip.layernorm(q, w["transformer_decoder.post_norm.weight"],
                          w["transformer_decoder.post_norm.bias"], pl.qn)
        if with_cls:
            hip.linear(pl.qn, w["cls_embed.weight"], w["cls_embed.bias"], cls_out.view(B * Q, -1))
        self._mlp3("mask_embed", pl.qn, pl.me, pl)
        if full_mask:
            self._mask_logits(pl.me, pl, mp_out)

    def _attn_mask(self, pl, lvl, mp=None, me=None):
        B, Q = pl.B, self.num_obj_query
        h, wd = pl.shapes[lvl]
        n = h * wd
        if self.exact_mask_order == "full":
            hip.bilinear_planar(pl.MP if mp is None else mp, pl.ML, B * Q, pl.hw2[0], pl.hw2[1],
                                h, wd)
        elif self.exact_mask_order and self.fuse_mask_pack:
            hip.mask_stencil_gemm(pl.me if me is None else me, pl.MFs[lvl], pl.bits, pl.rowall,
                                  B, Q, pl.hw2[0], pl.hw2[1], h, wd)
            return
        elif self.exact_mask_order:
            hip.gemm(pl.me if me is None else me, pl.MFs[lvl], pl.ML4, M=Q, N=4 * n, K=256,
                     lda=256, ldw=256, ldc=4 * n, batch=B, sA=Q * 256, sW=4 * n * 256,
                     sC=Q * 4 * n, force="tile64")
            hip.mask_pack_stencil(pl.ML4, pl.bits, pl.rowall, B * Q, pl.hw2[0], pl.hw2[1], h, wd)
            return
        else:
            hip.gemm(pl.me if me is None else me, pl.MFd[lvl], pl.ML, M=Q, N=n, K=256, lda=256,
                     ldw=256, ldc=n, batch=B, sA=Q * 256, sW=n * 256, sC=Q * n)
        hip.mask_pack(pl.ML, pl.bits, pl.rowall, B * Q, n)

    def _layer(self, pre, x, xpos, x1, x2, y, Qp, VQK, att, hbuf, Kp, ldk, Vp, ldv, Nk, B, nq,
               bits, rowall, scr, ffn, self_first=False, post=None, x_in=None):
        w = self.w
        scale = 1.0 / math.sqrt(32.0)
        ac = pre + "attentions.%d.attn." % (1 if self_first else 0)
        as_ = pre + "attentions.%d.attn." % (0 if self_first else 1)
        nc, ns = ("norms.1.", "norms.0.") if self_first else ("norms.0.", "norms.1.")

        def cross(src, dst):
            hip.linear(src, w[ac + "in_proj_weight"][:256], w[ac + "in_proj_bias"][:256], Qp,
                       aadd=xpos)
            hip.attention(Qp, 256, Kp, ldk, Vp, ldv, bits, rowall, att, 256, scr, B, nq, Nk, scale)
            hip.linear(att, w[ac + "out_proj.weight"], w[ac + "out_proj.bias"], y, res=src)
            hip.layernorm(y, w[pre + nc + "weight"], w[pre + nc + "bias"], dst)

        def self_attn(src, dst):
            hip.linear(src, w[as_ + "vqk.weight"], w[as_ + "vqk.bias"], VQK, aadd=xpos,
                       aadd_from_col=256)
            hip.attention(VQK[:, 256:], 768, VQK[:, 512:], 768, VQK, 768, None, None, att, 256,
                          scr, B, nq, nq, scale)
            hip.linear(att, w[as_ + "out_proj.weight"], w[as_ + "out_proj.bias"], y, res=src)
            hip.layernorm(y, w[pre + ns + "weight"], w[pre + ns + "bias"], dst)

        x_in = x if x_in is None else x_in
        if self_first:
            self_attn(x_in, x1)
            cross(x1, x2)
        else:
            cross(x_in, x1)
            self_attn(x1, x2)
        hip.ffn_ln(x2, w[pre + "ffns.0.layers.0.0.weight"], w[pre + "ffns.0.layers.0.0.bias"],
                   w[pre + "ffns.0.layers.1.weight"], w[pre + "ffns.0.layers.1.bias"],
                   w[pre + "norms.2.weight"], w[pre + "norms.2.bias"], x, hbuf, B * nq, ffn,
                   post=post)

    def _stage_a(self, feats, pl):
        with hip.reserve_slots(self.grid_reserve):
            self._stage_a_launches(feats, pl)

    def _stage_a_launches(self, feats, pl):
        self._pixel_decoder(feats, pl)
        probs = self._kv_problems(pl)
        for j in range(0, len(probs), hip.GEMM_GROUP_MAX):
            hip.gemm_group(probs[j:j + hip.GEMM_GROUP_MAX])

    def _memory_kv(self, pl, attn_prefix, l, Kp, Vp):
        w, B = self.w, pl.B
        mem = pl.X[:, pl.start[l]:]
        common = dict(A=mem, M=pl.N[l], N=256, K=256, lda=256, ldw=256, ldc=256, batch=B,
                      sA=pl.SN * 256, sC=pl.N[l] * 256, ldaadd=256)
        return [dict(W=w[attn_prefix + "in_proj_weight"][256:512], C=Kp,
                     bias=w[attn_prefix + "in_proj_bias"][256:512], aadd=pl.dec_kpos[l],
                     aadd_rows=pl.N[l], **common),
                dict(W=w[attn_prefix + "in_proj_weight"][512:], C=Vp,
                     bias=w[attn_prefix + "in_proj_bias"][512:],
                     aadd=w["level_embed.weight"][l:l + 1], aadd_rows=1, **common)]

    def _kv_problems(self, pl):
        probs = []
        for i in range(self.num_dec_layers):
            probs += self._memory_kv(pl, "transformer_decoder.layers.%d.attentions.0.attn." % i,
                                     i % 3, pl.Kp[i], pl.Vp[i])
        return probs

    def _stage_b(self, pl):
        self._object_decoder(pl)
        self._relation_stage(pl)

    def _object_decoder(self, pl, all_layers=False, final_head=True):
        w, B, Q = self.w, pl.B, self.num_obj_query
        qpos = w["query_embed.weight"]
        exact = self.exact_mask_order == "full"
        if exact:
            self._head_embed(pl.q0, pl, False, True)
        last = self.num_dec_layers - 1
        mp = None
        post = (w["transformer_decoder.post_norm.weight"], w["transformer_decoder.post_norm.bias"],
                pl.qn)
        for i in range(self.num_dec_layers):
            l = i % 3
            self._attn_mask(pl, l, mp, me=pl.me0 if (i == 0 and not exact) else None)
            self._layer("transformer_decoder.layers.%d." % i, pl.q, qpos, pl.q1, pl.q2, pl.qy,
                        pl.Qp, pl.VQK, pl.att, pl.hq, pl.Kp[i], 256, pl.Vp[i], 256, pl.N[l], B,
                        Q, pl.bits, pl.rowall, pl.scr, self.dec_ffn, post=post,
                        x_in=pl.q0 if i == 0 else None)
            if all_layers:
                mp = pl.MP_all[i]
                self._head_embed(pl.q, pl, True, True, pl.cls_all[i], mp, normed=True)
            elif final_head:
                self._head_embed(pl.q, pl, i == last, exact or i == last, normed=True)
            elif i != last:
                self._head_embed(pl.q, pl, False, exact, normed=True)

    def _relation_stage(self, pl):
        self._pair_proposal(pl)
        self._relation_decoder(pl)

    def _pair_proposal(self, pl):
        w, B, Q, R = self.w, pl.B, self.num_obj_query, self.num_rel_query
        for mlp, dst in (("sub_query_update", pl.sn), ("obj_query_update", pl.on)):
            hip.linear(pl.q, w[mlp + ".0.weight"], w[mlp + ".0.bias"], pl.s1, relu=True)
            hip.linear(pl.s1, w[mlp + ".2.weight"], w[mlp + ".2.bias"], pl.s2, relu=True)
            if self.fuse_ppn_front:
                hip.linear(pl.s2, w[mlp + ".4.weight"], w[mlp + ".4.bias"], dst)
                continue
            hip.linear(pl.s2, w[mlp + ".4.weight"], w[mlp + ".4.bias"], pl.s1)
            hip.l2normalize(pl.s1, dst)
        ml = "update_importance.conv_layers."
        if self.fuse_ppn_front:
            hip.ppn_front(pl.sn, pl.on, w[ml + "0.0.weight"], w[ml + "0.0.bias"], pl.imp_raw,
                          pl.c1, B, Q)
        else:
            hip.gemm(pl.sn, pl.on, pl.imp_raw, M=Q, N=Q, K=256, lda=256, ldw=256, ldc=Q, batch=B,
                     sA=Q * 256, sW=Q * 256, sC=Q * Q)
            hip.mlearner_first(pl.imp_raw, w[ml + "0.0.weight"], w[ml + "0.0.bias"], pl.c1, B, Q)
        hip.conv2d_ex(pl.c1, w[ml + "1.0.weight"], w[ml + "1.0.bias"], None, pl.c2, B, Q, Q, 64,
                      64, 7, 7, 1, 3, relu=True, scratch=pl.ppn_splitk)
        hip.mlearner_last(pl.c2, w[ml + "2.0.weight"], w[ml + "2.0.bias"], pl.imp, B, Q)
        hip.topk_pairs(pl.imp, pl.topk_idx, pl.sub_pos, pl.obj_pos, B, Q, R, pair=pl.pair_idx)
        hip.gather_rows(pl.q, pl.pair_idx, pl.pair, B, Q, 2 * R, 256)

    def _relation_decoder(self, pl):
        w, B, Q, R = self.w, pl.B, self.num_obj_query, self.num_rel_query
        rpos, ppos = w["rel_query_embed.weight"], w["rel_query_embed2.weight"]
        hip.gemm_group([dict(
            A=pl.pair, W=w["relation_decoder.layers.%d.attentions.0.attn.vk.weight" % i],
            C=pl.pVK_all[i], bias=w["relation_decoder.layers.%d.attentions.0.attn.vk.bias" % i],
            M=B * 2 * R, N=512, K=256, lda=256, ldw=256, ldc=512, aadd=ppos, ldaadd=256,
            aadd_rows=2 * R, aadd_from_col=256) for i in range(self.num_rel_layers)])
        for i in range(self.num_rel_layers):
            pre = "relation_decoder.layers.%d." % i
            pvk = pl.pVK_all[i]
            self._layer(pre, pl.r, rpos, pl.r1, pl.r2, pl.ry, pl.rQp, pl.rVQK, pl.ratt, pl.rh,
                        pvk[:, 256:], 512, pvk, 512, 2 * R, B, R, None, None, pl.scr,
                        self.rel_ffn, x_in=pl.r0 if i == 0 else None)
        hip.linear(pl.r, w["rel_cls_embed.weight"], w["rel_cls_embed.bias"], pl.rel.view(B * R, -1))
        self._gather_outputs(pl)

    def _gather_outputs(self, pl):
        B, Q, R = pl.B, self.num_obj_query, self.num_rel_query
        nc = self.num_classes + 1
        hip.gather_rows(pl.cls, pl.sub_pos, pl.sub_cls, B, Q, R, nc)
        hip.gather_rows(pl.cls, pl.obj_pos, pl.obj_cls, B, Q, R, nc)
        hip.gather_rows(pl.MP, pl.sub_pos, pl.sub_seg, B, Q, R, pl.HW2)
        hip.gather_rows(pl.MP, pl.obj_pos, pl.obj_seg, B, Q, R, pl.HW2)

    def _outputs(self, pl):
        B, Q, R = pl.B, self.num_obj_query, self.num_rel_query
        H2, W2 = pl.hw2
        return (dict(sub=pl.sub_cls, obj=pl.obj_cls, cls=pl.cls, rel=pl.rel, importance=pl.imp),
                dict(mask=pl.MP.view(B, Q, H2, W2), sub_seg=pl.sub_seg.view(B, R, H2, W2),
                     obj_seg=pl.obj_seg.view(B, R, H2, W2)))

    def _check_feats(self, feats, img_metas):
        pv = getattr(self, "_packed_version", None)
        if self.w is not None and pv is not None and pv != self._weights_version():
            self._drop_weight_state()
        B = len(img_metas)
        assert len(feats) == 4 and all(f.shape[0] == B for f in feats)
        nchw = all(f.is_contiguous() for f in feats)
        nhwc = not nchw and all(f.is_contiguous(memory_format=torch.channels_last) for f in feats)
        for f, c in zip(feats, self.in_channels):
            if not f.is_cuda or f.dtype != torch.float32 or f.shape[1] != c or not (nchw or nhwc):
                raise RuntimeError("feats must be fp32 [B,C,H,W] device tensors with channels %s, "
                                   "all contiguous or all in channels_last memory format"
                                   % self.in_channels)
        if self.device is None:
            self.to(feats[0].device)
        shapes = [tuple(feats[3 - l].shape[-2:]) for l in range(3)]
        self._feats_nhwc = nhwc
        return B, shapes, tuple(feats[0].shape[-2:])

    def _run_stage(self, which, pl, feats=None):
        cfg = (self.exact_mask_order, self.conv_algo, self.fuse_ppn_front, self.grid_reserve,
               tuple(self.enc_fused_ln), self.group_input_convs,
               getattr(self, "fuse_mask_pack", True), self.gemm_arithmetic, self.msda_s3_out)
        if pl.graph_cfg != cfg:
            pl.graph_a = pl.graph_b = None
            pl.graphs_a = OrderedDict()
            pl.graph_c = PlanCache(self.POST_VIEWS)
            pl.graph_cfg = cfg
        cur = torch.cuda.current_stream(self.device)
        pl.streams[cur.cuda_stream] = cur
        try:
            self._run_stage_on(which, pl, feats, cur)
        finally:
            plans.note_use(cur)

    def _run_stage_on(self, which, pl, feats, cur):
        if which == "a":
            if not pl.pe_waited:
                if pl.pe_ready.query():
                    pl.pe_waited = True
                else:
                    cur.wait_event(pl.pe_ready)
            ptrs = tuple(f.data_ptr() for f in feats)
            ent = pl.graphs_a.get(ptrs)
            if ent is None:
                if len(pl.graphs_a) >= self.STAGE_A_GRAPHS:
                    for k, e in pl.graphs_a.items():
                        if e["graph"] is None:
                            del pl.graphs_a[k]
                            break
                    else:
                        if plans.quiet(cur):
                            torch.cuda.current_stream(self.device).synchronize()
                            pl.graphs_a.popitem(last=False)
                if len(pl.graphs_a) < self.STAGE_A_GRAPHS:
                    ent = pl.graphs_a[ptrs] = dict(calls=0, graph=None, feats=None)
            else:
                pl.graphs_a.move_to_end(ptrs)
            if self.use_graphs and ent is not None and ent["graph"] is None \
                    and ent["calls"] >= self.graph_after and plans.quiet(cur):
                ent["feats"] = list(feats)
                self._note_capture(pl, ("a", ptrs))
                ent["graph"] = self._capture(lambda: self._stage_a(ent["feats"], pl))
            if ent is not None:
                ent["calls"] += 1
            pl.calls_a += 1
            graph = ent["graph"] if (self.use_graphs and ent is not None) else None
            pl.graph_a, pl.static_ptrs = graph, (ptrs if graph is not None else None)
            if pl.feats_read is None:
                pl.feats_read = torch.cuda.Event()
            if graph is not None:
                graph.replay()
            else:
                self._stage_a(feats, pl)
            pl.feats_read.record()
        else:
            if self.use_graphs and pl.graph_b is None and pl.calls_b >= self.graph_after \
                    and plans.quiet(cur):
                self._note_capture(pl, "b")
                pl.graph_b = self._capture(lambda: self._stage_b(pl))
            pl.calls_b += 1
            if self.use_graphs and pl.graph_b is not None:
                pl.graph_b.replay()
            else:
                self._stage_b(pl)

    def _note_capture(self, pl, stage):
        seen = self.__dict__.setdefault("_captured", set())
        if len(seen) > 8192:
            seen.clear()
        k = (pl.key, stage)
        if k in seen:
            self.recaptures = getattr(self, "recaptures", 0) + 1
        seen.add(k)

    _capture_streams = {}
    captures = 0

    @staticmethod
    def _capture(fn):
        torch.cuda.synchronize()
        dev = torch.cuda.current_device()
        cs = CrossHead2._capture_streams.get(dev)
        if cs is None:
            cs = CrossHead2._capture_streams[dev] = torch.cuda.Stream(dev)
        g = torch.cuda.CUDAGraph()
        import gc
        gc_was_on = gc.isenabled()
        gc.disable()
        try:
            with torch.cuda.stream(cs):
                g.capture_begin(capture_error_mode="thread_local")
                try:
                    fn()
                except BaseException as first:
                    try:
                        g.capture_end()
                    except Exception:
                        pass
                    raise first
                g.capture_end()
        finally:
            if gc_was_on:
                gc.enable()
        CrossHead2.captures += 1
        return g

    @torch.no_grad()
    @hip.on_device
    def forward(self, feats, img_metas, slot=0):
        B, shapes, hw2 = self._check_feats(feats, img_metas)
        pl = self._plan(B, shapes, hw2, slot, self._feats_nhwc)
        self._run_stage("a", pl, feats)
        self._run_stage("b", pl)
        self._last_plan = pl
        return self._outputs(pl)

    __call__ = forward

    @torch.no_grad()
    @hip.on_device
    def forward_head(self, decoder_out, mask_feature, attn_mask_target_size):
        if self.w is None:
            if self.device is None:
                self.to(decoder_out.device)
            self._pack()
        w = self.w
        Q, B, _ = decoder_out.shape
        h, wd = mask_feature.shape[-2:]
        th, tw = attn_mask_target_size
        dev, f32 = self.device, torch.float32
        E = lambda *s: torch.empty(*s, device=dev, dtype=f32)
        q = decoder_out.permute(1, 0, 2).contiguous().view(B * Q, 256)
        mf = mask_feature.permute(0, 2, 3, 1).contiguous().view(B, h * wd, 256)
        qn, m1, m2, me = E(B * Q, 256), E(B * Q, 256), E(B * Q, 256), E(B * Q, 256)
        cls = E(B, Q, self.num_classes + 1)
        mp, ml = E(B, Q, h * wd), E(B * Q, th * tw)
        hip.layernorm(q, w["transformer_decoder.post_norm.weight"],
                      w["transformer_decoder.post_norm.bias"], qn)
        hip.linear(qn, w["cls_embed.weight"], w["cls_embed.bias"], cls.view(B * Q, -1))
        hip.linear(qn, w["mask_embed.0.weight"], w["mask_embed.0.bias"], m1, relu=True)
        hip.linear(m1, w["mask_embed.2.weight"], w["mask_embed.2.bias"], m2, relu=True)
        hip.linear(m2, w["mask_embed.4.weight"], w["mask_embed.4.bias"], me)
        hip.gemm(me, mf, mp, M=Q, N=h * wd, K=256, lda=256, ldw=256, ldc=h * wd, batch=B,
                 sA=Q * 256, sW=h * wd * 256, sC=Q * h * wd)
        hip.bilinear_planar(mp, ml, B * Q, h, wd, th, tw)
        attn = (ml.view(B, 1, Q, th * tw) < 0).expand(B, self.n_heads, Q, th * tw)
        return cls, mp.view(B, Q, h, wd), attn.reshape(B * self.n_heads, Q, th * tw)

    class ResultList(list):
        panoptic_jobs = ()

    def _post_buffers(self, anchor, key, build):
        k = (anchor.data_ptr(), str(anchor.device)) + tuple(key)
        table = self._post
        pb = table.get(k)
# ... 192 lines not shown
```

### pair-net_amd/hip.py

```python
import contextlib
import ctypes as C
import os
import threading

import torch

from .build import LIB_PATH

LIB_PATH = os.environ.get("PAIRNET_LIB") or LIB_PATH

_i32, _i64, _f32, _vp = C.c_int32, C.c_int64, C.c_float, C.c_void_p

GEMM_RELU, GEMM_A_COLMAJOR, GEMM_FORCE_TILE, GEMM_FORCE_SKINNY = 1, 2, 4, 8
GEMM_GELU = 256
GEMM_FORCE_TILE64, GEMM_FORCE_TILE128x64 = 16, 32
GEMM_RELU_AFTER_RES = 128
GEMM_GROUP_MAX = 18


class GemmDesc(C.Structure):
    _fields_ = [("A", _vp), ("lda", _i64), ("strideA", _i64),
                ("Aadd", _vp), ("ldaadd", _i64), ("aadd_rows", _i32),
                ("aadd_from_col", _i32),
                ("W", _vp), ("ldw", _i64), ("strideW", _i64),
                ("bias", _vp),
                ("Res", _vp), ("ldres", _i64), ("strideRes", _i64),
                ("C", _vp), ("ldc", _i64), ("strideC", _i64),
                ("M", _i32), ("N", _i32), ("K", _i32), ("batch", _i32),
                ("flags", _i32),
                ("splitk_scratch", _vp), ("splitk_scratch_floats", _i64)]


class GemmS3Desc(C.Structure):
    _fields_ = [("A", _vp), ("A2", _vp), ("a2_from_col", _i32),
                ("W", _vp), ("bias", _vp),
                ("M", _i32), ("N", _i32), ("K", _i32), ("relu", _i32),
                ("C", _vp), ("ldc", _i64),
                ("CS", _vp),
                ("CS_pos", _vp), ("pos", _vp), ("pos_rows", _i32),
                ("res_s3", _vp), ("gamma", _vp), ("beta", _vp), ("eps", _f32), ("flags", _i32),
                ("act", _i32), ("res", _vp), ("ldres", _i64)]


_SIGS = {
    "pn_abi_version": (C.c_int, []),
    "pn_s3_bytes": (_i64, [_i32, _i32]),
    "pn_s3_split_f32": (C.c_int, [_vp, _i64, _vp, _i32, _vp, _i32, _i32, _vp]),
    "pn_s3_join_f32": (C.c_int, [_vp, _vp, _i64, _i32, _i32, _vp]),
    "pn_gemm_s3_f32": (C.c_int, [C.POINTER(GemmS3Desc), _vp]),
    "pn_gemm_f32": (C.c_int, [C.POINTER(GemmDesc), _vp]),
    "pn_gemm_variant": (C.c_int, [C.POINTER(GemmDesc)]),
    "pn_gemm_grid_size": (C.c_int, [C.POINTER(GemmDesc)]),
    "pn_gemm_wgs_per_cu": (C.c_int, []),
    "pn_gemm_group_f32": (C.c_int, [C.POINTER(GemmDesc), C.c_int, _vp]),
    "pn_conv2d_nhwc_f32": (C.c_int, [_vp, _vp, _vp, _vp] + [_i32] * 10 + [_vp]),
    "pn_conv2d_nhwc_ex_f32": (C.c_int, [_vp] * 5 + [_i32] * 10 + [_vp, _i64, _vp]),
    "pn_stem7x7s2_f32": (C.c_int, [_vp, _vp, _vp, _vp, _i32, _i32, _i32, _i32, _vp]),
    "pn_maxpool3x3s2_nhwc_f32": (C.c_int, [_vp, _vp, _i32, _i32, _i32, _i32, _vp]),
    "pn_winograd_f23_input_f32": (C.c_int, [_vp, _vp, _i32, _i32, _i32, _i32, _vp]),
    "pn_winograd_f23_output_f32": (C.c_int, [_vp, _vp, _vp, _i32, _i32, _i32, _i32, _i32, _vp]),
    "pn_winograd_f43_input_f32": (C.c_int, [_vp, _vp, _i32, _i32, _i32, _i32, _vp]),
    "pn_winograd_f43_output_f32": (C.c_int, [_vp, _vp, _vp, _i32, _i32, _i32, _i32, _i32, _vp]),
    "pn_layernorm_f32": (C.c_int, [_vp, _vp, _vp, _vp, _i64, _i32, _f32, _vp]),
    "pn_layernorm_rows_s3_f32": (C.c_int, [_vp, _i64, _vp, _vp, _vp, _i64, _i32, _f32, _vp]),
    "pn_layernorm_rows_f32": (C.c_int, [_vp, _i64, _vp, _vp, _vp, _i64, _i64, _i32, _f32, _vp]),
    "pn_patch_merge_ln_f32": (C.c_int, [_vp, _vp, _vp, _vp, _i32, _i32, _i32, _i32, _f32, _vp]),
    "pn_patch_im2col4_f32": (C.c_int, [_vp, _vp, _i32, _i32, _i32, _vp]),
    "pn_window_attention_f32": (C.c_int, [_vp, _i64, _vp, _vp, _vp, _i64] + [_i32] * 7 +
                                [_f32, _vp]),
    "pn_window_attention_s3_f32": (C.c_int, [_vp, _i64, _vp, _vp, _vp] + [_i32] * 7 + [_f32, _vp]),
    "pn_groupnorm_nblk": (C.c_int, [_i64]),
    "pn_groupnorm_nhwc_f32": (C.c_int, [_vp, _vp, _vp, _vp, _vp, _i32, _i64, _i32,
                                        _i32, _f32, _i32, _i64, _i64, _vp]),
    "pn_l2normalize_f32": (C.c_int, [_vp, _vp, _i64, _i32, _f32, _vp]),
    "pn_ffn_scratch_floats": (_i64, [_i32, _i32]),
    "pn_ffn_ln_f32": (C.c_int, [_vp] * 9 + [_i32, _i32, _i32, _f32, _vp]),
    "pn_ffn_ln2_f32": (C.c_int, [_vp] * 12 + [_i32, _i32, _i32, _f32, _vp]),
    "pn_msda_f32": (C.c_int, [_vp, _i64, _vp, _i64, _vp, _i32, _i32, C.POINTER(_i32),
                              C.POINTER(_i32), _vp]),
    "pn_msda_ex_f32": (C.c_int, [_vp, _i64, _vp, _i64, _vp, _i32, _i32, C.POINTER(_i32),
                                 C.POINTER(_i32), _i32, _vp]),
    "pn_linear_res_ln_f32": (C.c_int, [_vp, _i64, _vp, _i64, _vp, _vp, _i64, _vp, _vp, _vp, _i64,
                                       _i32, _i32, _i32, _f32, _vp]),
    "pn_gt_mask_prepare_u8": (C.c_int, [_vp, _vp] + [_i32] * 7 + [_vp]),
    "pn_point_sample_f32": (C.c_int, [_vp, _i32, _vp, _vp, _i32, _i32, _i32, _i32, _vp]),
    "pn_mask_match_cost_f32": (C.c_int, [_vp, _i32, _vp, _vp, _vp, _vp, _i32, _i32, _i32, _f32,
                                         _f32, _f32, _f32, _vp]),
    "pn_id_match_cost_f32": (C.c_int, [_vp, _vp, _vp, _i32, _i32, _vp, _vp, _vp, _vp, _i32, _i32,
                                       _f32, _f32, _f32, _vp]),
    "pn_ce_mean_f32": (C.c_int, [_vp, _i64, _vp, _vp, _vp, _i32, _i32, _f32, _vp]),
    "pn_seesaw_mean_f32": (C.c_int, [_vp, _i64, _vp, _vp, _vp, _i32, _i32, _f32, _f32, _f32, _f32,
                                     _vp]),
    "pn_bce_posw_mean_f32": (C.c_int, [_vp, _vp, _vp, _i64, _f32, _vp]),
    "pn_ce_mean_grad_f32": (C.c_int, [_vp, _i64, _vp, _vp, _vp, _i64, _i32, _i32, _f32, _vp]),
    "pn_seesaw_mean_grad_f32": (C.c_int, [_vp, _i64, _vp, _vp, _vp, _i64, _i32, _i32, _f32, _f32,
                                          _f32, _f32, _vp]),
    "pn_bce_posw_mean_grad_f32": (C.c_int, [_vp, _vp, _vp, _i64, _f32, _vp]),
    "pn_transpose_f32": (C.c_int, [_vp, _i64, _vp, _i64, _i32, _i32, _i32, _vp]),
    "pn_colsum_f32": (C.c_int, [_vp, _i64, _vp, _i32, _i32, _i32, _vp, _i64, _vp]),
    "pn_relu_bwd_f32": (C.c_int, [_vp, _vp, _vp, _i64, _vp]),
    "pn_add_periodic_f32": (C.c_int, [_vp, _vp, _vp, _i64, _i64, _vp]),
    "pn_batch_sum_f32": (C.c_int, [_vp, _vp, _i32, _i64, _i32, _vp]),
    "pn_layernorm256_bwd_f32": (C.c_int, [_vp, _vp, _vp, _vp, _vp, _i32, _f32, _vp]),
    "pn_mha_bwd_f32": (C.c_int, [_vp, _i64, _vp, _i64, _vp, _i64, _vp, _i64, _vp, _i64, _vp, _i64,
                                 _vp, _i64, _vp, _vp, _vp, _i32, _i32, _i32, _f32, _vp]),
    "pn_scatter_rows_add_f32": (C.c_int, [_vp, _i64, _vp, _vp, _i64, _i32, _i32, _i32, _i32, _i32, _vp]),
    "pn_cosine_bwd_f32": (C.c_int, [_vp, _vp, _vp, _vp, _i32, _i32, _i32, _f32, _vp]),
    "pn_mlearner_last_bwd_data_f32": (C.c_int, [_vp, _vp, _vp, _vp, _i32, _i32, _vp]),
    "pn_tapcorr1_f32": (C.c_int, [_vp, _vp, _vp, _i32, _i32, _i32, _vp]),
    "pn_conv_weight_bwd_layout_f32": (C.c_int, [_vp, _vp, _i32, _i32, _i32, _vp]),
    "pn_msda_offaw_bwd_f32": (C.c_int, [_vp, _vp, _vp, _vp, _i64, _i64, _i32, C.POINTER(_i32),
                                        C.POINTER(_i32), _vp]),
    "pn_groupnorm_nhwc_bwd_f32": (C.c_int, [_vp, _vp, _vp, _vp, _vp, _vp, _i32, _i64, _i32, _f32, _i64,
                                            _i64, _vp]),
    "pn_winograd_weights_f32": (C.c_int, [_vp, _vp, _i32, _i32, _i32, _vp]),
    "pn_conv_wgrad_f32": (C.c_int, [_vp, _vp, _vp] + [_i32] * 11 + [_vp]),
    "pn_dilate2_f32": (C.c_int, [_vp, _vp] + [_i32] * 7 + [_vp]),
    "pn_subsample2_f32": (C.c_int, [_vp, _vp] + [_i32] * 6 + [_vp]),
    "pn_scale_rows_f32": (C.c_int, [_vp, _vp, _i64, _i64, _vp]),
    "pn_layernorm_rows_bwd_f32": (C.c_int, [_vp, _i64, _vp, _i64, _vp, _vp, _i64, _vp, _i64, _i64,
                                            _i32, _f32, _vp]),
    "pn_gelu_f32": (C.c_int, [_vp, _vp, _i64, _vp]),
    "pn_gelu_bwd_f32": (C.c_int, [_vp, _vp, _vp, _i64, _vp]),
    "pn_window_attention_bwd_f32": (C.c_int, [_vp, _i64, _vp, _vp, _vp, _i64, _vp, _i64, _vp, _i64, _vp]
                                    + [_i32] * 7 + [_f32, _vp]),
    "pn_grad_norm_clip_f32": (C.c_int, [_vp, _i64, _f32, _f32, _vp, _vp, _vp]),
    "pn_adamw_f32": (C.c_int, [_vp, _vp, _vp, _vp, _i64, _vp, _vp, _vp, _i32, _f32, _f32, _f32, _f32,
                               _f32, _i32, _vp, _f32, _vp]),
    "pn_msda_loc_f32": (C.c_int, [_vp, _i64, _vp, _vp, _vp, _vp, _vp, _i32, _i32, _i32, _i32, _vp]),
    "pn_msda_bwd_f32": (C.c_int, [_vp, _i64] + [_vp] * 8 + [_i32, _i32, _i32, _i32, _vp]),
    "pn_gather_probe_f32": (C.c_int, [_vp, _vp, _vp, _i32, _i32, _vp]),
    "pn_sine_pe_f32": (C.c_int, [_vp, _vp, _i32, _i32, _i32, _f32, _vp]),
    "pn_sine_pe_offset_f32": (C.c_int, [_vp, _vp, _i32, _i32, _i32, _f32, _f32, _vp]),
    "pn_bilinear_nhwc_f32": (C.c_int, [_vp, _vp] + [_i32] * 7 + [_i64, _i64, _vp]),
    "pn_bilinear_planar_f32": (C.c_int, [_vp, _vp, _i64] + [_i32] * 4 + [_vp]),
    "pn_bilinear_planar_gt0_u8": (C.c_int, [_vp, _vp, _i64] + [_i32] * 4 + [_vp]),
    "pn_mask_pack": (C.c_int, [_vp, _vp, _vp, _i64, _i32, _vp]),
    "pn_mask_pack_stencil": (C.c_int, [_vp, _vp, _vp, _i64, _i32, _i32, _i32, _i32, _vp]),
    "pn_mask_stencil_gemm_f32": (C.c_int, [_vp, _i64, _i64, _vp, _i64, _i64, _vp, _vp] +
                                 [_i32] * 9 + [_vp]),
    "pn_bilinear_stencil_rows_f32": (C.c_int, [_vp, _vp] + [_i32] * 6 + [_i64, _i64, _vp]),
    "pn_attn_scratch_floats": (_i64, [_i32, _i32, _i32]),
    "pn_attention_f32": (C.c_int, [_vp, _i64, _vp, _i64, _vp, _i64, _vp, _vp, _vp,
                                   _i64, _vp, _i32, _i32, _i32, _f32, _vp]),
    "pn_ppn_front_f32": (C.c_int, [_vp] * 6 + [_i32, _i32, _f32, _vp]),
    "pn_mlearner_first_f32": (C.c_int, [_vp, _vp, _vp, _vp, _i32, _i32, _i32, _vp]),
    "pn_mlearner_last_f32": (C.c_int, [_vp, _vp, _vp, _vp, _i32, _i32, _i32, _vp]),
    "pn_topk_pairs": (C.c_int, [_vp, _vp, _vp, _vp, _vp, _i32, _i32, _i32, _vp]),
    "pn_topk_f32": (C.c_int, [_vp, _vp, _vp, _vp, _i32, _i32, _i32, _i32, _vp]),
    "pn_topk_strided_f32": (C.c_int, [_vp, _i64, _i64, _vp, _vp, _vp, _i32, _i32, _i32, _i32, _vp]),
    "pn_gather_rows_f32": (C.c_int, [_vp, _vp, _vp, _i32, _i32, _i32, _i64, _vp]),
    "pn_cls_argmax_f32": (C.c_int, [_vp, _vp, _vp, _i64, _i32, _i32, _vp]),
    "pn_rel_dists_f32": (C.c_int, [_vp, _vp, _i64, _i32, _vp]),
    "pn_softmax_fg_f32": (C.c_int, [_vp, _vp, _vp, _i64, _i32, _vp]),
    "pn_row_argmax_f32": (C.c_int, [_vp, _vp, _i64, _i32, _vp]),
    "pn_triplet_finish": (C.c_int, [_vp] * 9 + [_i32, _i32, _vp]),
    "pn_panoptic_f32": (C.c_int, [_vp, _vp, _vp, _vp, _vp, _i32, _i64, _vp]),
    "pn_panoptic_state_bytes": (_i64, []),
    "pn_panoptic_device_f32": (C.c_int, [_vp, _vp, _vp] + [_i32] * 6 + [_vp, _vp, _vp, _vp,
                                                                        _i32, _vp]),
    "pn_panoptic_continue_f32": (C.c_int, [_vp, _vp, _vp, _vp, _i32, _i32, _i32, _vp]),
    "pn_pack_triplets_f32": (C.c_int, [_vp] * 5 + [_i32, _i32, _vp]),
    "pn_copy_stream": (C.c_int, [_vp, _vp, _i64, _i32, _vp]),
    "pn_pack_bool_bits": (C.c_int, [_vp, _vp, _i64, _vp]),
    "pn_unpack_bits_host": (C.c_int, [_vp, _vp, _i64, _i32]),
    "pn_pred_triplets": (C.c_int, [_vp, _vp, _vp, _vp, _i32, _i32, _vp]),
    "pn_mask_or_rows": (C.c_int, [_vp, _vp, _vp, _vp, _i32, _i64, _vp]),
    "pn_triplet_match": (C.c_int, [_vp, _vp, _i32, _i32, _vp, _vp, _vp, _i32, _vp, _vp, _vp, _vp,
                                   C.c_double, _i32, _i32, _vp, _vp]),
    "pn_triplet_match_boxes": (C.c_int, [_vp, _vp, _i32, _i32, _vp, _i32, _vp, _i32, _vp, _vp, _vp,
                                         _vp, _f32, _i32, _i32, _vp, _vp]),
    "pn_pan_masks_u8": (C.c_int, [_vp] * 5 + [_i32] * 3 + [_vp]),
    "pn_preprocess_u8_f32": (C.c_int, [_vp, _i32, _i32, _vp] + [_i32] * 4 + [C.POINTER(_f32),
                                                                            C.POINTER(_f32), _i32, _vp]),
    "pn_pack_mask_bits": (C.c_int, [_vp, _vp, _i64, _i64, _vp]),
    "pn_mask_iou_counts": (C.c_int, [_vp, _i32, _vp, _i32, _i64, _vp, _vp, _vp, _vp]),
    "pn_zero_rows_f32": (C.c_int, [_vp, _vp, _vp, _i32, _i64, _i32, _i64, _i64, _vp]),
    "pn_token_sampling_f32": (C.c_int, [_vp, _i64, _vp, _vp, _vp, _i32, _i32, C.POINTER(_i32),
                                        C.POINTER(_i32), _vp]),
    "pn_sine_pe_valid_f32": (C.c_int, [_vp, _vp, _i32, _i32, _i32, _i32, _i32, _f32, _f32, _vp]),
    "pn_sigmoid_f32": (C.c_int, [_vp, _vp, _i64, _vp]),
    "pn_box_pos_embed_f32": (C.c_int, [_vp, _vp, _vp, _i64, _vp]),
    "pn_box_sampling_f32": (C.c_int, [_vp, _i64, _vp, _vp, _i32, _vp, _vp, _i64, _i32, _vp]),
    "pn_box_refine_f32": (C.c_int, [_vp, _vp, _vp, _i64, _vp]),
    "pn_query_score_f32": (C.c_int, [_vp, _vp, _i32, _i32, _i32, _vp]),
    "pn_box_triplets_f32": (C.c_int, [_vp] * 5 + [_vp, _i32, _i32, _f32, _f32, C.POINTER(_f32),
                                                _i32, _vp]),
}
EXPORTS = tuple(_SIGS)
ABI_VERSION = 29

_lib = None


def lib():
    global _lib
    if _lib is None:
        if not os.path.exists(LIB_PATH):
            raise RuntimeError(
                "libpairnet_hip.so is missing (%s): run __graft_entry__.build(); "
                "there is no CPU / PyTorch fallback for the Pair-Net hot path" % LIB_PATH)
        handle = C.CDLL(LIB_PATH)
        for name, (res, args) in _SIGS.items():
            fn = getattr(handle, name)
            fn.restype, fn.argtypes = res, args
        if handle.pn_abi_version() != ABI_VERSION:
            raise RuntimeError("libpairnet_hip.so ABI mismatch; rebuild")
        _lib = handle
    return _lib


class _Reserve(threading.local):
    slots = 0


_reserve = _Reserve()


@contextlib.contextmanager
def reserve_slots(n):
    old = _reserve.slots
    _reserve.slots = max(0, int(n)) // 8 * 8
    try:
        yield
    finally:
        _reserve.slots = old


def with_reserve(fn):
    import functools

    @functools.wraps(fn)
    def wrapper(self, *args, **kw):
        with reserve_slots(getattr(self, "grid_reserve", 0)):
            return fn(self, *args, **kw)
    return wrapper


def _reserve_flag():
    return ((_reserve.slots // 8) & 0x3ff) << 16


def _stream():
    return torch.cuda.current_stream().cuda_stream


def on_device(fn):
    import functools

    def first_tensor(objs):
        for o in objs:
            if isinstance(o, torch.Tensor) and o.is_cuda:
                return o.device
            if isinstance(o, (list, tuple)):
                d = first_tensor(o)
                if d is not None:
                    return d
            if isinstance(o, dict):
                d = first_tensor(o.values())
                if d is not None:
                    return d
        return None

    @functools.wraps(fn)
    def wrapper(self, *args, **kw):
        dev = getattr(self, "device", None)
        if dev is None or dev.type != "cuda":
            dev = first_tensor(args)
        if dev is None or dev.type != "cuda" or dev.index == torch.cuda.current_device():
            return fn(self, *args, **kw)
        with torch.cuda.device(dev):
            return fn(self, *args, **kw)
    return wrapper


GEMM_KERNELS = {0: "k_gemm_skinny<A_ROW>", 1: "k_gemm_skinny<A_COL>",
                2: "k_gemm_tile<128,64,64,32,A_ROW>", 3: "k_gemm_tile<128,64,64,32,A_COL>",
                4: "k_gemm_tile<128,128,64,64,A_ROW>", 5: "k_gemm_tile<128,128,64,64,A_COL>",
                6: "k_gemm_tile<64,64,32,32,A_ROW>", 7: "k_gemm_tile<64,64,32,32,A_COL>"}


class KernelTimer:

    def __init__(self, only=None):
        self.only = set(only) if only else None
        self.records = []
        self.meta = []

    def summary(self):
        torch.cuda.synchronize()
        agg = {}
        for name, flops, nbytes, s, e in self.records:
            a = agg.setdefault(name, dict(launches=0, ms=0.0, flops=0.0, bytes=0.0))
            a["launches"] += 1
            a["ms"] += s.elapsed_time(e)
            a["flops"] += flops
            a["bytes"] += nbytes
        return agg


TIMER = None


def _launch(name, flops, nbytes, fn, meta=None):
    t = TIMER
    if t is None or (t.only is not None and name not in t.only):
        return fn()
    s, e = torch.cuda.Event(enable_timing=True), torch.cuda.Event(enable_timing=True)
    s.record()
    r = fn()
    e.record()
    t.records.append((name, flops, nbytes, s, e))
    t.meta.append(meta)
    return r


def _ptr(t, dtype=torch.float32):
    if t is None:
        return None
    if not t.is_cuda:
        raise RuntimeError("pairnet_hip kernels take device tensors (got %s)" % t.device)
    if t.dtype != dtype:
        raise RuntimeError("expected %s, got %s" % (dtype, t.dtype))
    return t.data_ptr()


def _check(code, what):
    if code != 0:
        raise RuntimeError("%s failed: %s" % (
            what, "argument contract violated" if code == -1 else "hipError %d" % code))


def _rowmajor(t):
    assert t.dim() == 2 and t.stride(1) == 1, (t.shape, t.stride())
    return t.shape[0], t.stride(0)


def gemm_desc(A, W, Cout, *, M, N, K, lda, ldw, ldc, bias=None, aadd=None, ldaadd=0,
              aadd_rows=0, aadd_from_col=0, res=None, ldres=0, batch=1, sA=0, sW=0, sC=0,
              sRes=0, relu=False, colmajor=False, force=None, into=None,
              relu_after=False, scratch=None, gelu=False, ksplit=0):
    d = into if into is not None else GemmDesc()
    d.A, d.lda, d.strideA = _ptr(A), lda, sA
    d.Aadd, d.ldaadd, d.aadd_rows, d.aadd_from_col = _ptr(aadd), ldaadd, aadd_rows, aadd_from_col
    d.W, d.ldw, d.strideW = _ptr(W), ldw, sW
    d.bias = _ptr(bias)
    d.Res, d.ldres, d.strideRes = _ptr(res), ldres, sRes
    d.C, d.ldc, d.strideC = _ptr(Cout), ldc, sC
    d.M, d.N, d.K, d.batch = M, N, K, batch
    d.flags = (GEMM_RELU if relu else 0) | (GEMM_A_COLMAJOR if colmajor else 0) | \
        {None: 0, "tile": GEMM_FORCE_TILE, "skinny": GEMM_FORCE_SKINNY, "tile64": 16,
         "tile128x64": 32}[force] | _reserve_flag() | ((ksplit & 31) << 26) | \
        (GEMM_RELU_AFTER_RES if relu_after else 0) | (GEMM_GELU if gelu else 0)
    d.splitk_scratch = _ptr(scratch)
    d.splitk_scratch_floats = scratch.numel() if scratch is not None else 0
    return d


def gemm(A, W, Cout, **kw):
    d = gemm_desc(A, W, Cout, **kw)
    if TIMER is None:
        _check(lib().pn_gemm_f32(C.byref(d), _stream()), "pn_gemm_f32")
        return
    name = GEMM_KERNELS[lib().pn_gemm_variant(C.byref(d))]
    nbytes = 4.0 * d.batch * (d.M * d.K + d.N * d.K + d.M * d.N)
    if d.Res:
        nbytes += 4.0 * d.batch * d.M * d.N
    if d.Aadd:
        nbytes += 4.0 * min(d.aadd_rows, d.M) * d.K
    _check(_launch(name, 2.0 * d.M * d.N * d.K * d.batch, nbytes,
                   lambda: lib().pn_gemm_f32(C.byref(d), _stream()),
                   meta=(d.M, d.N, d.K, d.batch, bool(d.splitk_scratch))), "pn_gemm_f32")


def gemm_group(problems):
    n = len(problems)
    arr = (GemmDesc * n)()
    flops = nbytes = 0.0
    for i, pr in enumerate(problems):
        pr = dict(pr)
        d = gemm_desc(pr.pop("A"), pr.pop("W"), pr.pop("C"), into=arr[i], **pr)
        flops += 2.0 * d.M * d.N * d.K * d.batch
        nbytes += 4.0 * d.batch * (d.M * d.K + d.N * d.K + d.M * d.N)
    _check(_launch("k_gemm_group", flops, nbytes,
                   lambda: lib().pn_gemm_group_f32(arr, n, _stream())), "pn_gemm_group_f32")


def linear(x, weight, bias, out, *, aadd=None, aadd_from_col=0, res=None, relu=False,
           force=None, relu_after=False, scratch=None, gelu=False):
    M, lda = _rowmajor(x)
    N, ldw = _rowmajor(weight)
    Mo, ldc = _rowmajor(out)
    assert Mo == M and out.shape[1] == N and weight.shape[1] == x.shape[1]
    kw = {}
    if aadd is not None:
        ra, lda2 = _rowmajor(aadd)
        kw.update(aadd=aadd, ldaadd=lda2, aadd_rows=ra, aadd_from_col=aadd_from_col)
    if res is not None:
        rr, ldr = _rowmajor(res)
        assert rr == M
        kw.update(res=res, ldres=ldr)
    gemm(x, weight, out, M=M, N=N, K=x.shape[1], lda=lda, ldw=ldw, ldc=ldc, bias=bias,
         relu=relu, force=force, relu_after=relu_after, scratch=scratch, gelu=gelu,
         **kw)


def conv2d_nhwc(x, wp, bias, out, B, H, W, Cin, Cout, KH, KW, pad, relu, big_tile=False,
                tile=None):
    tflag = {None: 0, "128": GEMM_FORCE_TILE, "128x64": GEMM_FORCE_TILE128x64}[tile]
    name = ("k_gemm_tile<128,64,64,32,A_CONV>" if tile == "128x64" else
            "k_gemm_tile<128,128,64,64,A_CONV>" if tile == "128" else
            "k_gemm_tile<64,64,32,32,A_CONV>")
    flops = 2.0 * B * H * W * Cout * KH * KW * Cin
    nbytes = 4.0 * (B * H * W * (Cin + Cout) + Cout * KH * KW * Cin)
    _check(_launch(name, flops, nbytes, lambda: lib().pn_conv2d_nhwc_f32(
        _ptr(x), _ptr(wp), _ptr(bias), _ptr(out), B, H, W, Cin, Cout, KH, KW, pad, int(relu),
        (GEMM_FORCE_TILE if big_tile else 0) | tflag | _reserve_flag(),
        _stream())), "pn_conv2d_nhwc_f32")


def conv2d_ex(x, wp, bias, res, out, B, H, W, Cin, Cout, KH, KW, stride, pad, relu=False,
              relu_after=False, scratch=None):
    Ho, Wo = (H + 2 * pad - KH) // stride + 1, (W + 2 * pad - KW) // stride + 1
    flops = 2.0 * B * Ho * Wo * Cout * KH * KW * Cin
    nbytes = 4.0 * (B * (H * W * Cin + Ho * Wo * Cout * (2 if res is not None else 1))
                    + Cout * KH * KW * Cin)
    flags = (GEMM_RELU if relu else 0) | (GEMM_RELU_AFTER_RES if relu_after else 0) | \
        _reserve_flag()
    _check(_launch("k_gemm_tile<64,64,32,32,A_CONV>", flops, nbytes,
                   lambda: lib().pn_conv2d_nhwc_ex_f32(
                       _ptr(x), _ptr(wp), _ptr(bias), _ptr(res), _ptr(out), B, H, W, Cin, Cout,
                       KH, KW, stride, pad, flags, _ptr(scratch),
                       scratch.numel() if scratch is not None else 0, _stream())),
           "pn_conv2d_nhwc_ex_f32")


def stem7x7s2(img, wp, bias, out, B, H, W):
    Ho, Wo = (H - 1) // 2 + 1, (W - 1) // 2 + 1
    _check(_launch("k_stem7x7s2", 2.0 * B * Ho * Wo * 64 * 147,
                   4.0 * B * (3 * H * W + Ho * Wo * 64),
                   lambda: lib().pn_stem7x7s2_f32(_ptr(img), _ptr(wp), _ptr(bias), _ptr(out), B,
                                                  H, W, _reserve_flag(), _stream())),
           "pn_stem7x7s2_f32")


def maxpool3x3s2(x, out, B, H, W, Cc):
    _check(lib().pn_maxpool3x3s2_nhwc_f32(_ptr(x), _ptr(out), B, H, W, Cc, _stream()),
           "pn_maxpool3x3s2_nhwc_f32")


def _winograd_weights_dev(w, form):
    w = w.contiguous()
    co, ci = w.shape[0], w.shape[1]
    U = torch.empty((16 if form == 2 else 36), co, ci, device=w.device, dtype=torch.float32)
    _check(lib().pn_winograd_weights_f32(_ptr(w), _ptr(U), co, ci, form, _stream()),
           "pn_winograd_weights_f32")
    return U


def winograd_weights(w):
    if w.is_cuda:
        return _winograd_weights_dev(w, 2)
    G = torch.tensor([[1.0, 0.0, 0.0], [0.5, 0.5, 0.5], [0.5, -0.5, 0.5], [0.0, 0.0, 1.0]],
                     dtype=torch.float64, device=w.device)
    U = torch.einsum("ik,ockl,jl->ijoc", G, w.double(), G)
    return U.reshape(16, w.shape[0], w.shape[1]).float().contiguous()


def winograd43_weights(w):
    if w.is_cuda:
        return _winograd_weights_dev(w, 4)
    G = torch.tensor([[1 / 4, 0, 0], [-1 / 6, -1 / 6, -1 / 6], [-1 / 6, 1 / 6, -1 / 6],
                      [1 / 24, 1 / 12, 1 / 6], [1 / 24, -1 / 12, 1 / 6], [0, 0, 1]],
                     dtype=torch.float64, device=w.device)
    U = torch.einsum("ik,ockl,jl->ijoc", G, w.double(), G)
    return U.reshape(36, w.shape[0], w.shape[1]).float().contiguous()


def conv3x3_winograd43(x, U, bias, out, V, Mbuf, B, H, W, Cin, Cout, relu):
    T = B * ((H + 3) // 4) * ((W + 3) // 4)
    _check(lib().pn_winograd_f43_input_f32(_ptr(x), _ptr(V), B, H, W, Cin, _stream()),
           "pn_winograd_f43_input_f32")
    gemm(V, U, Mbuf, M=T, N=Cout, K=Cin, lda=Cin, ldw=Cin, ldc=Cout, batch=36, sA=T * Cin,
         sW=Cout * Cin, sC=T * Cout)
    _check(lib().pn_winograd_f43_output_f32(_ptr(Mbuf), _ptr(bias), _ptr(out), B, H, W, Cout,
                                            int(relu), _stream()), "pn_winograd_f43_output_f32")


def conv3x3_winograd(x, U, bias, out, V, Mbuf, B, H, W, Cin, Cout, relu):
    T = B * ((H + 1) // 2) * ((W + 1) // 2)
    _check(lib().pn_winograd_f23_input_f32(_ptr(x), _ptr(V), B, H, W, Cin, _stream()),
           "pn_winograd_f23_input_f32")
    gemm(V, U, Mbuf, M=T, N=Cout, K=Cin, lda=Cin, ldw=Cin, ldc=Cout, batch=16, sA=T * Cin,
         sW=Cout * Cin, sC=T * Cout)
    _check(lib().pn_winograd_f23_output_f32(_ptr(Mbuf), _ptr(bias), _ptr(out), B, H, W, Cout,
                                            int(relu), _stream()), "pn_winograd_f23_output_f32")


def layernorm(x, gamma, beta, out, eps=1e-5):
    rows = x.numel() // 256
    _check(lib().pn_layernorm_f32(_ptr(x), _ptr(gamma), _ptr(beta), _ptr(out), rows, 256,
                                  eps, _stream()), "pn_layernorm_f32")


def linear_res_ln(x, weight, bias, res, gamma, beta, out, eps=1e-5):
    M, ldx = _rowmajor(x)
    N, ldw = _rowmajor(weight)
    Mr, ldr = _rowmajor(res)
    Mo, ldo = _rowmajor(out)
    K = x.shape[1]
    assert Mr == M and Mo == M and N == 256 and weight.shape[1] == K
    nbytes = 4.0 * (M * K + N * K + 2 * M * N)
    _check(_launch("k_gemm_rowln", 2.0 * M * N * K, nbytes,
                   lambda: lib().pn_linear_res_ln_f32(_ptr(x), ldx, _ptr(weight), ldw, _ptr(bias),
                                                      _ptr(res), ldr, _ptr(gamma), _ptr(beta),
                                                      _ptr(out), ldo, M, N, K, eps, _stream()),
                   meta=(M, N, K, 1, False)), "pn_linear_res_ln_f32")


def s3_floats(rows, K):
    return ((rows + 31) // 32) * (K // 16) * 768


def pos8(pos):
    rows, cols = pos.shape
    rb = (rows + 31) // 32
    p = pos.new_zeros(rb * 32, cols)
    p[:rows] = pos
    return p.view(rb, 32, cols // 16, 2, 8).permute(0, 2, 3, 1, 4).contiguous()


def s3_split(x, out, add=None):
    rows, ld = _rowmajor(x)
    K = x.shape[1]
    assert out.numel() * out.element_size() >= s3_floats(rows, K) * 4
    ar = 0
    if add is not None:
        ar, lda = _rowmajor(add)
        assert lda == K and add.shape[1] == K
    _check(_launch("k_s3_split", 0.0, 10.0 * rows * K,
                   lambda: lib().pn_s3_split_f32(_ptr(x), ld, _ptr(add), ar, _ptr(out), rows, K,
                                                 _stream())), "pn_s3_split_f32")


def s3_join(s3, out):
    rows, ld = _rowmajor(out)
    _check(_launch("k_s3_join", 0.0, 10.0 * rows * out.shape[1],
                   lambda: lib().pn_s3_join_f32(_ptr(s3), _ptr(out), ld, rows, out.shape[1],
                                                _stream())), "pn_s3_join_f32")


def gemm_s3(a, w, M, N, K, *, bias=None, relu=False, out=None, out_s3=None, out_s3_pos=None,
            pos=None, a2=None, a2_from_col=0, res_s3=None, gamma=None, beta=None, eps=1e-5,
            tile96=False, tile192=False, gelu=False, res=None, relu_after=False):
    d = GemmS3Desc()
    d.A, d.A2, d.a2_from_col = _ptr(a), _ptr(a2), a2_from_col
    d.W, d.bias = _ptr(w), _ptr(bias)
    d.M, d.N, d.K, d.relu = M, N, K, int(relu)
    if out is not None:
        Mo, ldc = _rowmajor(out)
        assert Mo == M and out.shape[1] >= N
        d.C, d.ldc = _ptr(out), ldc
    d.CS, d.CS_pos = _ptr(out_s3), _ptr(out_s3_pos)
    if out_s3_pos is not None:
        pos, pr = pos
        assert pos.numel() == (pr + 31) // 32 * 32 * N
        d.pos, d.pos_rows = _ptr(pos), pr
    d.res_s3, d.gamma, d.beta, d.eps = _ptr(res_s3), _ptr(gamma), _ptr(beta), eps
    d.flags = (1 if tile96 else 0) | (2 if tile192 else 0)
    d.act = 3 if relu_after else 2 if gelu else 0
    if res is not None:
        Mr, ldr = _rowmajor(res)
        assert Mr == M and res.shape[1] >= N
        d.res, d.ldres = _ptr(res), ldr
    nbytes = 6.0 * (M * K + N * K) + (4.0 * M * N if out is not None else 0.0) + \
        6.0 * M * N * ((out_s3 is not None) + (out_s3_pos is not None) + (res_s3 is not None))
    name = "k_gemm_s3<ln>" if gamma is not None else "k_gemm_s3"
    _check(_launch(name, 2.0 * M * N * K, nbytes, lambda: lib().pn_gemm_s3_f32(C.byref(d), _stream()),
                   meta=(M, N, K, 1, False)), "pn_gemm_s3_f32")


def layernorm_rows(x, gamma, beta, out, eps=1e-5):
    rows, ldx = _rowmajor(x)
    ro, ldo = _rowmajor(out)
    assert ro == rows and out.shape[1] == x.shape[1]
    _check(_launch("k_ln_rows", 0.0, 8.0 * rows * x.shape[1],
                   lambda: lib().pn_layernorm_rows_f32(_ptr(x), ldx, _ptr(gamma), _ptr(beta),
                                                       _ptr(out), ldo, rows, x.shape[1], eps,
                                                       _stream())), "pn_layernorm_rows_f32")


def layernorm_rows_s3(x, gamma, beta, out_s3, eps=1e-5):
    rows, ldx = _rowmajor(x)
    Cc = x.shape[1]
    assert out_s3.numel() >= s3_floats(rows, Cc)
    _check(_launch("k_ln_rows<s3>", 0.0, 10.0 * rows * Cc,
                   lambda: lib().pn_layernorm_rows_s3_f32(_ptr(x), ldx, _ptr(gamma), _ptr(beta),
                                                          _ptr(out_s3), rows, Cc, eps, _stream())),
           "pn_layernorm_rows_s3_f32")


def patch_merge_ln(x, gamma, beta, out, B, H, W, C, eps=1e-5):
    _check(_launch("k_ln_rows<merge>", 0.0, 8.0 * B * H * W * C,
                   lambda: lib().pn_patch_merge_ln_f32(_ptr(x), _ptr(gamma), _ptr(beta), _ptr(out),
                                                       B, H, W, C, eps, _stream())),
           "pn_patch_merge_ln_f32")


def patch_im2col4(img, out, B, H, W):
    _check(_launch("k_patch_im2col", 0.0, 4.0 * B * H * W * 3 * 2.4,
                   lambda: lib().pn_patch_im2col4_f32(_ptr(img), _ptr(out), B, H, W, _stream())),
           "pn_patch_im2col4_f32")


def window_attention(qkv, qkv_bias, table, out, B, H, W, C, heads, ws, shift):
    n, ldq = _rowmajor(qkv)
    no, ldo = _rowmajor(out)
    assert n == no == B * H * W and qkv.shape[1] == 3 * C
    hp, wp = -(-H // ws) * ws, -(-W // ws) * ws
    flops = 4.0 * B * hp * wp * (ws * ws) * C
    _check(_launch("k_window_attn", flops, 16.0 * n * C,
                   lambda: lib().pn_window_attention_f32(_ptr(qkv), ldq, _ptr(qkv_bias),
                                                         _ptr(table), _ptr(out), ldo, B, H, W, C,
                                                         heads, ws, shift, 32 ** -0.5, _stream())),
           "pn_window_attention_f32")


def window_attention_s3(qkv, qkv_bias, table, out_s3, B, H, W, C, heads, ws, shift):
    n, ldq = _rowmajor(qkv)
    assert n == B * H * W and qkv.shape[1] == 3 * C and out_s3.numel() >= s3_floats(n, C)
    hp, wp = -(-H // ws) * ws, -(-W // ws) * ws
    flops = 4.0 * B * hp * wp * (ws * ws) * C
    _check(_launch("k_window_attn", flops, 18.0 * n * C,
                   lambda: lib().pn_window_attention_s3_f32(_ptr(qkv), ldq, _ptr(qkv_bias), _ptr(table),
                                                            _ptr(out_s3), B, H, W, C, heads, ws, shift,
                                                            32 ** -0.5, _stream())),
           "pn_window_attention_s3_f32")


def groupnorm_nblk(hw):
    return lib().pn_groupnorm_nblk(hw)


def groupnorm_nhwc(x, gamma, beta, out, partials, B, HW, G, relu, x_bstride, y_bstride,
                   eps=1e-5):
    _check(lib().pn_groupnorm_nhwc_f32(
        _ptr(x), _ptr(gamma), _ptr(beta), _ptr(out), _ptr(partials, torch.float64), B, HW,
        256, G, eps, int(relu), x_bstride, y_bstride, _stream()), "pn_groupnorm_nhwc_f32")


def ffn_scratch_floats(M, hidden):
    return lib().pn_ffn_scratch_floats(M, hidden)


def ffn_ln(x, W1, b1, W2, b2, gamma, beta, out, scratch, M, hidden, eps=1e-5, post=None):
    g2, b2n, y2 = post if post is not None else (None, None, None)
    _check(_launch("k_ffn_partial+k_reduce_ln", 4.0 * M * 256 * hidden,
                   4.0 * (2 * 256 * hidden + 2 * M * 256),
                   lambda: lib().pn_ffn_ln2_f32(_ptr(x), _ptr(W1), _ptr(b1), _ptr(W2), _ptr(b2),
                                                _ptr(gamma), _ptr(beta), _ptr(out), _ptr(g2),
                                                _ptr(b2n), _ptr(y2), _ptr(scratch), M, 256, hidden,
                                                eps, _stream())), "pn_ffn_ln2_f32")


def l2normalize(x, out, eps=1e-12):
    _check(lib().pn_l2normalize_f32(_ptr(x), _ptr(out), x.numel() // 256, 256, eps,
                                    _stream()), "pn_l2normalize_f32")


MSDA_PERSISTENT, MSDA_PERSISTENT_BATCHED, MSDA_LOW_OCCUPANCY = 1, 2, 4


MSDA_S3_OUT = 8


def msda(value, ld_value, offaw, ld_offaw, out, B, shapes, flags=0, s3_out=False):
    if s3_out:
        flags |= MSDA_S3_OUT
    L = len(shapes)
    hs = (_i32 * L)(*[s[0] for s in shapes])
    ws = (_i32 * L)(*[s[1] for s in shapes])
    n = sum(h * w for h, w in shapes)
    nbytes = 4.0 * B * n * (256 + 8 * L * 4 * 3 + 256)
    _check(_launch("k_msda", 2.0 * B * n * 8 * L * 4 * 4 * 32 * 2, nbytes,
                   lambda: lib().pn_msda_ex_f32(_ptr(value), ld_value, _ptr(offaw), ld_offaw,
                                                _ptr(out), B, L, hs, ws, flags, _stream())),
           "pn_msda_ex_f32")


def msda_loc(value, ld_value, spatial_shapes, level_start_index, loc, aw, out, B, N, Nq, L):
    nbytes = 4.0 * B * (N * 256 + Nq * (8 * L * 4 * 3 + 256))
    _check(_launch("k_msda_loc", 2.0 * B * Nq * 8 * L * 4 * 4 * 32 * 2, nbytes,
                   lambda: lib().pn_msda_loc_f32(_ptr(value), ld_value,
                                                 _ptr(spatial_shapes, torch.int64),
                                                 _ptr(level_start_index, torch.int64), _ptr(loc),
                                                 _ptr(aw), _ptr(out), B, N, Nq, L, _stream())),
           "pn_msda_loc_f32")


def msda_bwd(value, ld_value, spatial_shapes, level_start_index, loc, aw, grad_out, grad_value,
             grad_loc, grad_aw, B, N, Nq, L):
    _check(lib().pn_msda_bwd_f32(_ptr(value), ld_value, _ptr(spatial_shapes, torch.int64),
                                 _ptr(level_start_index, torch.int64), _ptr(loc), _ptr(aw),
                                 _ptr(grad_out), _ptr(grad_value), _ptr(grad_loc), _ptr(grad_aw),
                                 B, N, Nq, L, _stream()), "pn_msda_bwd_f32")


def gather_probe(lines, idx, out, workgroups, line_mask):
    _check(lib().pn_gather_probe_f32(_ptr(lines), _ptr(idx, torch.int32), _ptr(out), workgroups,
                                     line_mask, _stream()), "pn_gather_probe_f32")


def sine_pe(out, add, h, w, C_=256, temperature=10000.0, offset=0.0, valid=None):
    vh, vw = valid if valid is not None else (h, w)
    _check(lib().pn_sine_pe_valid_f32(_ptr(out), _ptr(add), h, w, vh, vw, C_, temperature, offset,
                                      _stream()), "pn_sine_pe_valid_f32")


def bilinear_nhwc(x, out, B, hi, wi, ho, wo, Cc, accumulate, in_bstride, out_bstride):
    _check(lib().pn_bilinear_nhwc_f32(_ptr(x), _ptr(out), B, hi, wi, ho, wo, Cc,
                                      int(accumulate), in_bstride, out_bstride, _stream()),
           "pn_bilinear_nhwc_f32")


def bilinear_planar(x, out, P, hi, wi, ho, wo):
    _check(lib().pn_bilinear_planar_f32(_ptr(x), _ptr(out), P, hi, wi, ho, wo, _stream()),
           "pn_bilinear_planar_f32")


def bilinear_planar_gt0(x, out, P, hi, wi, ho, wo):
    _check(lib().pn_bilinear_planar_gt0_u8(_ptr(x), _ptr(out, torch.uint8), P, hi, wi, ho,
                                           wo, _stream()), "pn_bilinear_planar_gt0_u8")


def mask_pack(logits, bits, rowall, R, Nk):
    _check(lib().pn_mask_pack(_ptr(logits), _ptr(bits, torch.int32),
                              _ptr(rowall, torch.int32), R, Nk, _stream()), "pn_mask_pack")


def mask_pack_stencil(logits4, bits, rowall, R, hi, wi, ho, wo):
    _check(lib().pn_mask_pack_stencil(_ptr(logits4), _ptr(bits, torch.int32),
                                      _ptr(rowall, torch.int32), R, hi, wi, ho, wo, _stream()),
           "pn_mask_pack_stencil")


def mask_stencil_gemm(me, rows, bits, rowall, B, Q, hi, wi, ho, wo, K=256):
    Nk = ho * wo
    _check(_launch("k_gemm_stencil", 2.0 * B * Q * 4 * Nk * K,
                   4.0 * B * (Q * K + 4 * Nk * K) + B * Q * Nk / 8.0,
                   lambda: lib().pn_mask_stencil_gemm_f32(
                       _ptr(me), me.stride(0), Q * me.stride(0), _ptr(rows), rows.stride(-2),
                       rows.stride(0) if rows.dim() == 3 else 4 * Nk * rows.stride(-2),
                       _ptr(bits, torch.int32), _ptr(rowall, torch.int32), B, Q, Nk, K, hi, wi,
                       ho, wo, _reserve_flag(), _stream()),
                   meta=(Q, 4 * Nk, K, B, False)), "pn_mask_stencil_gemm_f32")


def bilinear_stencil_rows(x, out, B, hi, wi, ho, wo, Cc, in_bstride, out_bstride):
    _check(lib().pn_bilinear_stencil_rows_f32(_ptr(x), _ptr(out), B, hi, wi, ho, wo, Cc,
                                              in_bstride, out_bstride, _stream()),
           "pn_bilinear_stencil_rows_f32")


def attn_scratch_floats(B, Q, Nk):
    return lib().pn_attn_scratch_floats(B, Q, Nk)


def attention(q, ldq, k, ldk, v, ldv, bits, rowall, out, ldo, scratch, B, Q, Nk, scale):
    _check(_launch("k_attn_chunk", 8.0 * B * 8 * Q * Nk * 32 / 2,
                   4.0 * B * 256 * (2 * Q + 2 * Nk),
                   lambda: lib().pn_attention_f32(
                       _ptr(q), ldq, _ptr(k), ldk, _ptr(v), ldv, _ptr(bits, torch.int32),
                       _ptr(rowall, torch.int32), _ptr(out), ldo, _ptr(scratch), B, Q, Nk, scale,
                       _stream())), "pn_attention_f32")


def ppn_front(sub_embed, obj_embed, w1, b1, imp_raw, c1, B, Q, eps=1e-12):
    _check(lib().pn_ppn_front_f32(_ptr(sub_embed), _ptr(obj_embed), _ptr(w1), _ptr(b1),
                                  _ptr(imp_raw), _ptr(c1), B, Q, eps, _stream()),
           "pn_ppn_front_f32")


def mlearner_first(x, w1, b1, out, B, S):
    _check(lib().pn_mlearner_first_f32(_ptr(x), _ptr(w1), _ptr(b1), _ptr(out), B, S, 64,
                                       _stream()), "pn_mlearner_first_f32")


def mlearner_last(x, w3, b3, out, B, S):
    _check(lib().pn_mlearner_last_f32(_ptr(x), _ptr(w3), _ptr(b3), _ptr(out), B, S, 64,
                                      _stream()), "pn_mlearner_last_f32")


def topk_pairs(scores, idx, sub, obj, B, Q, k, pair=None):
    _check(lib().pn_topk_pairs(_ptr(scores), _ptr(idx, torch.int64), _ptr(sub, torch.int64),
                               _ptr(obj, torch.int64), _ptr(pair, torch.int64), B, Q, k,
                               _stream()), "pn_topk_pairs")


def topk(scores, idx, quot, rem, B, n, div, k):
    _check(lib().pn_topk_f32(_ptr(scores), _ptr(idx, torch.int64), _ptr(quot, torch.int64),
                             _ptr(rem, torch.int64), B, n, div, k, _stream()), "pn_topk_f32")


def topk_strided(scores, elem_stride, row_stride, idx, quot, rem, B, n, div, k):
    _check(lib().pn_topk_strided_f32(_ptr(scores), elem_stride, row_stride, _ptr(idx, torch.int64),
                                     _ptr(quot, torch.int64), _ptr(rem, torch.int64), B, n, div,
                                     k, _stream()), "pn_topk_strided_f32")


def gather_rows(x, index, out, B, rows_in, rows_out, length):
    _check(lib().pn_gather_rows_f32(_ptr(x), _ptr(index, torch.int64), _ptr(out), B, rows_in,
                                    rows_out, length, _stream()), "pn_gather_rows_f32")


def cls_argmax(logits, label, score, rows, Cc, label_offset=0):
    _check(lib().pn_cls_argmax_f32(_ptr(logits), _ptr(label, torch.int64), _ptr(score), rows,
                                   Cc, label_offset, _stream()), "pn_cls_argmax_f32")


def rel_dists(logits, out, rows, Cc):
    _check(lib().pn_rel_dists_f32(_ptr(logits), _ptr(out), rows, Cc, _stream()),
           "pn_rel_dists_f32")


def softmax_fg(logits, probs, fg, rows, Cc):
    _check(lib().pn_softmax_fg_f32(_ptr(logits), _ptr(probs), _ptr(fg), rows, Cc, _stream()),
           "pn_softmax_fg_f32")


def row_argmax(x, idx, rows, n):
    _check(lib().pn_row_argmax_f32(_ptr(x), _ptr(idx, torch.int64), rows, n, _stream()),
           "pn_row_argmax_f32")


def triplet_finish(s_label, o_label, probs, tri, rem, labels, r_labels, r_scores, r_dists, k,
                   Cc):
    i64 = torch.int64
    _check(lib().pn_triplet_finish(_ptr(s_label, i64), _ptr(o_label, i64), _ptr(probs),
                                   _ptr(tri, i64), _ptr(rem, i64), _ptr(labels, i64),
                                   _ptr(r_labels, i64), _ptr(r_scores), _ptr(r_dists), k, Cc,
                                   _stream()),
           "pn_triplet_finish")


def panoptic(masks, labels, remap, seg, area, n, HW):
    _check(lib().pn_panoptic_f32(_ptr(masks), _ptr(labels, torch.int64),
                                 _ptr(remap, torch.int32), _ptr(seg, torch.int64),
                                 _ptr(area, torch.int32), n, HW, _stream()), "pn_panoptic_f32")


PAN_ROUNDS = 4


def panoptic_state_bytes():
    return lib().pn_panoptic_state_bytes()


def panoptic_device(masks, labels, scores, Q, num_classes, hi, wi, ho, wo, state, up, area, seg,
                    rounds=None):
    rounds = PAN_ROUNDS if rounds is None else rounds
    _check(lib().pn_panoptic_device_f32(
        _ptr(masks), _ptr(labels, torch.int64), _ptr(scores), Q, num_classes, hi, wi, ho, wo,
        _ptr(state, torch.uint8), _ptr(up), _ptr(area, torch.int32), _ptr(seg, torch.int64),
        rounds, _stream()), "pn_panoptic_device_f32")


def panoptic_continue(state, up, area, seg, ho, wo, rounds=None):
    rounds = PAN_ROUNDS if rounds is None else rounds
    _check(lib().pn_panoptic_continue_f32(
        _ptr(state, torch.uint8), _ptr(up), _ptr(area, torch.int32), _ptr(seg, torch.int64),
        ho, wo, rounds, _stream()), "pn_panoptic_continue_f32")


def pack_triplets(labels, r_dists, sub_pos, obj_pos, rec, R, C1):
    i64 = torch.int64
    _check(lib().pn_pack_triplets_f32(_ptr(labels, i64), _ptr(r_dists), _ptr(sub_pos, i64),
                                      _ptr(obj_pos, i64), _ptr(rec), R, C1, _stream()),
           "pn_pack_triplets_f32")


def copy_stream(src, dst, wgs=16):
    if src.dtype != dst.dtype or src.numel() != dst.numel() or not (
            src.is_contiguous() and dst.is_contiguous()):
        raise RuntimeError("copy_stream takes contiguous tensors of one dtype and size")
    if not src.is_cuda or not (dst.is_cuda or dst.is_pinned()):
        raise RuntimeError("copy_stream: device source, device or pinned-host destination")
    nbytes = src.numel() * src.element_size()
    if nbytes:
        _check(lib().pn_copy_stream(src.data_ptr(), dst.data_ptr(), nbytes, int(wgs), _stream()),
               "pn_copy_stream")


def pack_bool_bits(src, bits):
    n = src.numel()
    if not src.is_cuda or not bits.is_cuda or src.element_size() != 1 or not src.is_contiguous() \
            or bits.dtype != torch.uint8 or bits.numel() < (n + 7) // 8 or not bits.is_contiguous():
        raise RuntimeError("pack_bool_bits: contiguous 1-byte device source, uint8 device "
                           "destination of (n + 7) // 8 bytes")
    if n:
        _check(lib().pn_pack_bool_bits(src.data_ptr(), bits.data_ptr(), n, _stream()),
               "pn_pack_bool_bits")


def unpack_bits_host(bits, out, threads=4):
    n = out.numel()
    if bits.is_cuda or out.is_cuda or out.element_size() != 1 or bits.dtype != torch.uint8 \
            or not (bits.is_contiguous() and out.is_contiguous()) or bits.numel() < (n + 7) // 8:
        raise RuntimeError("unpack_bits_host: contiguous host tensors, uint8 bits of "
# ... 386 lines not shown
```

Baseline: 222.5.

## Fuse bottleneck projection shortcut, gather mask stencil in GEMM, add GN+upsample-add kernel

Adds a two-phase persistent GEMM that computes the downsample shortcut and conv3 of each first bottleneck block in one kernel, keeping the shortcut result in registers as the residual. It also adds a stencil GEMM that gathers the bilinear tap rows of the mask features inside the kernel, so the separate stencil-rows materialisation is skipped. A fused groupnorm plus upsample-add kernel is added behind a flag that is off by default. These changes aim to cut kernel launches and intermediate memory traffic, but they add complexity and address arithmetic inside the GEMM inner setup.

New measurement: 225.8, median of 6. +1.5%, better.

```diff
diff --git a/include/pairnet_hip.h b/include/pairnet_hip.h
--- a/include/pairnet_hip.h
+++ b/include/pairnet_hip.h
@@ -7,7 +7,7 @@
 extern "C" {
 #endif
 
-#define PN_ABI_VERSION 29
+#define PN_ABI_VERSION 30
 int pn_abi_version(void);
 
 #define PN_GEMM_RELU       1
@@ -67,6 +67,11 @@
                           int Cout, int KH, int KW, int stride, int pad, int flags,
                           float* splitk_scratch ,
                           int64_t splitk_scratch_floats, void* stream);
+int pn_bottleneck_proj_f32(const float* x, const float* Wsc, const float* bsc, const float* t2,
+                           const float* W3, const float* b3, float* idt, float* out, int B,
+                           int H, int W, int Cin, int planes, int Cout, int stride, int flags,
+                           float* splitk_scratch , int64_t splitk_scratch_floats,
+                           void* stream);
 int pn_stem7x7s2_f32(const float* img_nchw, const float* Wp, const float* bias,
                      float* out, int B, int H, int W, int flags ,
                      void* stream);
@@ -99,6 +104,11 @@
                           float* y, double* partials, int B, int64_t HW, int C,
                           int G, float eps, int relu, int64_t x_bstride,
                           int64_t y_bstride, void* stream);
+
+int pn_groupnorm_upadd_nhwc_f32(const float* x, const float* gamma, const float* beta, float* y,
+                                double* partials, const float* coarse, int B, int H, int W,
+                                int hc, int wc, int C, int G, float eps, int64_t x_bstride,
+                                int64_t y_bstride, int64_t coarse_bstride, void* stream);
 
 int pn_linear_res_ln_f32(const float* x, int64_t ldx, const float* W, int64_t ldw,
                          const float* bias , const float* res, int64_t ldres,
@@ -171,6 +181,11 @@
                              int64_t ld_rows, int64_t stride_rows, uint32_t* bits,
                              int32_t* rowall, int B, int Q, int Nk, int K, int hi, int wi, int ho,
                              int wo, int flags, void* stream);
+
+int pn_mask_stencil_gather_gemm_f32(const float* me, int64_t ld_me, int64_t stride_me,
+                                    const float* mf, int64_t ld_mf, int64_t stride_mf,
+                                    uint32_t* bits, int32_t* rowall, int B, int Q, int Nk, int K,
+                                    int hi, int wi, int ho, int wo, int flags, void* stream);
 
 int64_t pn_attn_scratch_floats(int B, int Q, int Nk);
 int pn_attention_f32(const float* q, int64_t ldq, const float* k, int64_t ldk,
diff --git a/pair-net_amd/backbone.py b/pair-net_amd/backbone.py
--- a/pair-net_amd/backbone.py
+++ b/pair-net_amd/backbone.py
@@ -66,6 +66,7 @@
         self.conv_algo = "winograd4"
         self.wino_min_planes = 128
         self.s3_conv3_min_planes = 0
+        self.fuse_proj_shortcut = True
 
     def _weights_version(self):
         return sum(p._version for p in self._params.values())
@@ -184,7 +185,8 @@
         return out
 
     def _plan(self, B, H, W, slot=0):
-        key = (B, H, W, slot, self.conv_algo, self.wino_min_planes, self.s3_conv3_min_planes)
+        key = (B, H, W, slot, self.conv_algo, self.wino_min_planes, self.s3_conv3_min_planes,
+               self.fuse_proj_shortcut)
         if key in self._plans:
             return self._plans[key]
         if self.w is None:
@@ -307,6 +309,14 @@
                     hip.conv2d_ex(t1, w[p + "conv2.w"], w[p + "conv2.b"], None, pl.t2[i], B, hi,
                                   wi, planes, planes, 3, 3, stride, 1, relu=True,
                                   scratch=pl.scratch)
+                s3 = self.s3_conv3_min_planes and planes >= self.s3_conv3_min_planes
+                if b == 0 and self.fuse_proj_shortcut and not s3:
+                    dst = pl.out[i] if blocks == 1 else pl.ping[i]
+                    hip.bottleneck_proj(x, w[p + "downsample.0.w"], w[p + "downsample.0.b"],
+                                        pl.t2[i], w[p + "conv3.w"], w[p + "conv3.b"], pl.idt[i],
+                                        dst, B, hi, wi, cin, planes, stride, scratch=pl.scratch)
+                    x, cin = dst, planes * 4
+                    continue
                 if b == 0:
                     if stride == 1:
                         hip.linear(x.view(-1, cin), w[p + "downsample.0.w"],
@@ -323,7 +333,7 @@
                     dst = pl.out[i]
                 else:
                     dst = pl.ping[i] if idt is not pl.ping[i] else pl.idt[i]
-                if self.s3_conv3_min_planes and planes >= self.s3_conv3_min_planes:
+                if s3:
                     t2 = pl.t2[i].view(-1, planes)
                     hip.s3_split(t2, pl.t2_s3)
                     hip.gemm_s3(pl.t2_s3, w[p + "conv3.w.s3"], t2.shape[0], planes * 4, planes,
diff --git a/pair-net_amd/csrc/gemm.hip b/pair-net_amd/csrc/gemm.hip
--- a/pair-net_amd/csrc/gemm.hip
+++ b/pair-net_amd/csrc/gemm.hip
@@ -127,13 +127,21 @@
                                    (unsigned)(p.Aadd ? p.ldaadd : p.lda) + kc) * 4u;
       }
     }
-    if constexpr (EPI == 1) {
+    if constexpr (EPI == 1 || EPI == 3) {
       const StencilP& st = loc.st;
 #pragma unroll
       for (int j = 0; j < NB; ++j) {
         const int c = (tid >> 3) + RPP * j;
         const int key = min(tr.tn * 16 + (c >> 5) * 8 + (c & 7), st.nk - 1);
-        w_off[j] = ((unsigned)(((c >> 3) & 3) * st.nk + key) * (unsigned)p.ldw + kc) * 4u;
+        if constexpr (EPI == 3) {
+          const int t = (c >> 3) & 3;
+          const int oy = key / st.wo, ox = key - oy * st.wo;
+          const Tap ty = make_tap(oy, st.hi, st.ho), tx = make_tap(ox, st.wi, st.wo);
+          const int sy = (t & 2) ? ty.i1 : ty.i0, sx = (t & 1) ? tx.i1 : tx.i0;
+          w_off[j] = ((unsigned)(sy * st.wi + sx) * (unsigned)p.ldw + kc) * 4u;
+        } else {
+          w_off[j] = ((unsigned)(((c >> 3) & 3) * st.nk + key) * (unsigned)p.ldw + kc) * 4u;
+        }
       }
     } else {
 #pragma unroll
@@ -292,6 +300,8 @@
     }
   };
 
+  static_assert(EPI != 2 || (TM == 1 && TN == 1 && !PN_GEMM_LDS2), "two-phase mode: 32x32 waves, one LDS stage");
+  float keep[EPI == 2 ? 16 : 1];
   TileRef cur = loc(base + slot);
   set_tile(cur);
   load_chunk(0);
@@ -313,9 +323,10 @@
     __syncthreads();
   }
 #endif
-  for (int t = slot; t < cnt; t += per) {
+  for (int t = slot; t < cnt;) {
     const GemmP& p = loc.P(cur.pi);
-    const TileRef nxt = loc(base + min(t + per, cnt - 1));
+    const bool ph0 = EPI == 2 && cur.pi == 0;
+    const TileRef nxt = ph0 ? TileRef{1, cur.bz, cur.tm, cur.tn} : loc(base + min(t + per, cnt - 1));
     int nk = (p.K + BK - 1) / BK;
     if (p.ksplit > 1) {
       const int sidx = cur.bz % p.ksplit;
@@ -363,9 +374,9 @@
     }
 #endif
     const int m0 = cur.tm * BM, n0 = cur.tn * BN;
-    if constexpr (EPI == 1) {
+    if constexpr (EPI == 1 || EPI == 3) {
       const StencilP& st = loc.st;
-      static_assert(EPI == 0 || (TM == 1 && TN == 1 && BN == 64), "stencil mode: 64x64 tiles of 32x32 waves");
+      static_assert((EPI != 1 && EPI != 3) || (TM == 1 && TN == 1 && BN == 64), "stencil mode: 64x64 tiles of 32x32 waves");
       const int pl = li & 7;
       const int key0 = cur.tn * 16 + wn * 8;
       const int key = key0 + pl;
@@ -399,7 +410,18 @@
         }
       }
       cur = nxt;
+      t += per;
       continue;
+    }
+    if constexpr (EPI == 2) {
+      if (ph0) {
+        const int colc = min(n0 + wn * WN + li, p.N - 1);
+        const float bv = p.bias ? p.bias[colc] : 0.f;
+#pragma unroll
+        for (int r = 0; r < 16; ++r) keep[r] = acc[0][0][r] + bv;
+        cur = nxt;
+        continue;
+      }
     }
     float* __restrict__ C = p.C + (int64_t)cur.bz * p.sC;
     const float* __restrict__ Res = p.Res ? p.Res + (int64_t)cur.bz * p.sRes : nullptr;
@@ -413,7 +435,10 @@
       for (int mi = 0; mi < TM; ++mi) {
         const int rbase = m0 + wm * WM + mi * 32;
         float rv[16];
-        if (Res) {
+        if constexpr (EPI == 2) {
+#pragma unroll
+          for (int r = 0; r < 16; ++r) rv[r] = keep[r];
+        } else if (Res) {
 #pragma unroll
           for (int r = 0; r < 16; ++r)
             rv[r] = Res[(int64_t)min(rbase + mfma32_row(r, lh), p.M - 1) * p.ldres + colc];
@@ -423,7 +448,7 @@
         for (int r = 0; r < 16; ++r) {
           float v = acc[mi][ni][r] + bv;
           v = gemm_act(v, p.relu);
-          if (Res) v += rv[r];
+          if (EPI == 2 || Res) v += rv[r];
           if (p.relu_after) v = fmaxf(v, 0.f);
           ov[r] = v;
         }
@@ -440,6 +465,7 @@
       }
     }
     cur = nxt;
+    t += per;
   }
 }
 
@@ -488,6 +514,34 @@
   __shared__ __attribute__((aligned(16))) float smem[TileSmem<64, 64, A_ROW>::FLOATS];
   const StencilLocator loc{p, st, (p.M + 63) / 64, (p.N + 63) / 64};
   gemm_persistent<64, 64, 32, 32, A_ROW, false, StencilLocator, 1>(loc, loc.mt * loc.nt * batch, smem);
+}
+
+__global__ __launch_bounds__(256, (TileWgs<64, 64, A_ROW, false>::min_waves))
+void k_gemm_stencil_gather(const GemmP p, const StencilP st, const int batch) {
+  __shared__ __attribute__((aligned(16))) float smem[TileSmem<64, 64, A_ROW>::FLOATS];
+  const StencilLocator loc{p, st, (p.M + 63) / 64, (p.N + 63) / 64};
+  gemm_persistent<64, 64, 32, 32, A_ROW, false, StencilLocator, 3>(loc, loc.mt * loc.nt * batch, smem);
+}
+
+#define PN_GEMM_WGS_PROJ PN_GEMM_WGS64
+struct ProjLocator {
+  const GemmP& p;
+  const GemmP& sc;
+  int mt, nt;
+  __device__ __forceinline__ const GemmP& P(int phase) const { return phase ? p : sc; }
+  __device__ __forceinline__ TileRef operator()(int T) const {
+    const int per_b = mt * nt;
+    const int bz = T / per_b, r = T - bz * per_b;
+    const int tm = r / nt;
+    return TileRef{0, bz, tm, r - tm * nt};
+  }
+};
+
+__global__ __launch_bounds__(256, PN_GEMM_WGS_PROJ)
+void k_gemm_proj(const GemmP p, const GemmP sc, const int batch) {
+  __shared__ __attribute__((aligned(16))) float smem[TileSmem<64, 64, A_CONV>::FLOATS];
+  const ProjLocator loc{p, sc, (p.M + 63) / 64, (p.N + 63) / 64};
+  gemm_persistent<64, 64, 32, 32, A_CONV, false, ProjLocator, 2>(loc, loc.mt * loc.nt * batch, smem);
 }
 
 #define GEMM_GROUP_MAX 18
@@ -852,11 +906,9 @@
   return PN_LAUNCH_CHECK();
 }
 
-extern "C" int pn_conv2d_nhwc_ex_f32(const float* in, const float* Wp, const float* bias,
-                                     const float* res, float* out, int B, int H, int W,
-                                     int Cin, int Cout, int KH, int KW, int stride, int pad,
-                                     int flags, float* splitk_scratch,
-                                     int64_t splitk_scratch_floats, void* stream) {
+static int fill_conv_params(const float* in, const float* Wp, const float* bias, const float* res,
+                            float* out, int B, int H, int W, int Cin, int Cout, int KH, int KW,
+                            int stride, int pad, int flags, GemmP* outp) {
   if (!in || !Wp || !out || B <= 0 || H <= 0 || W <= 0 || stride <= 0 || pad < 0)
     return PN_BAD_ARG;
   if (Cin % 32 || !aligned16(in) || !aligned16(Wp)) return PN_BAD_ARG;
@@ -873,6 +925,19 @@
   p.relu_after = (flags & PN_GEMM_RELU_AFTER_RES) ? 1 : 0;
   p.aadd_rows = 1;
   p.H = H; p.Wd = W; p.Cin = Cin; p.KW = KW; p.pad = pad; p.stride = stride; p.Wo = Wo;
+  *outp = p;
+  return 0;
+}
+
+extern "C" int pn_conv2d_nhwc_ex_f32(const float* in, const float* Wp, const float* bias,
+                                     const float* res, float* out, int B, int H, int W,
+                                     int Cin, int Cout, int KH, int KW, int stride, int pad,
+                                     int flags, float* splitk_scratch,
+                                     int64_t splitk_scratch_floats, void* stream) {
+  GemmP p;
+  if (int rc = fill_conv_params(in, Wp, bias, res, out, B, H, W, Cin, Cout, KH, KW, stride, pad,
+                                flags, &p))
+    return rc;
   hipStream_t s = (hipStream_t)stream;
   if (flags & PN_GEMM_FORCE_TILE128x64) return launch_tile<128, 64, 64, 32, A_CONV>(p, B, s, flags);
   if (flags & PN_GEMM_FORCE_TILE) return launch_tile<128, 128, 64, 64, A_CONV>(p, B, s, flags);
@@ -887,6 +952,75 @@
   return pn_conv2d_nhwc_ex_f32(in, Wp, bias, nullptr, out, B, H, W, Cin, Cout, KH, KW, 1, pad,
                                (flags & ~PN_GEMM_RELU) | (relu ? PN_GEMM_RELU : 0), nullptr, 0,
                                stream);
+}
+
+static bool gemm_single_chain(const pn_gemm_desc* d) {
+  GemmP p;
+  if (pn_fill_params(d, &p) || gemm_use_skinny(d)) return false;
+  int cps;
+  return splitk_factor(p, d->batch, d->splitk_scratch, d->splitk_scratch_floats, &cps, d->flags) <= 1;
+}
+
+extern "C" int pn_bottleneck_proj_f32(const float* x, const float* Wsc, const float* bsc,
+                                      const float* t2, const float* W3, const float* b3,
+                                      float* idt, float* out, int B, int H, int W, int Cin,
+                                      int planes, int Cout, int stride, int flags,
+                                      float* splitk_scratch, int64_t splitk_scratch_floats,
+                                      void* stream) {
+  if (!x || !Wsc || !t2 || !W3 || !out || B <= 0 || H <= 0 || W <= 0 || stride <= 0 ||
+      Cin <= 0 || planes <= 0 || Cout <= 0)
+    return PN_BAD_ARG;
+  if (Cin % 32 || planes % 32 || !aligned16(x) || !aligned16(Wsc) || !aligned16(t2) || !aligned16(W3))
+    return PN_BAD_ARG;
+  const int Ho = (H - 1) / stride + 1, Wo = (W - 1) / stride + 1;
+  const int64_t M = (int64_t)Ho * Wo;
+  const int64_t lim = (int64_t)1 << 29;
+  if (M * planes >= lim || M * B >= lim || (int64_t)Cout * Cin >= lim || (int64_t)Cout * planes >= lim)
+    return PN_BAD_ARG;
+  flags &= (0x3ff << PN_GEMM_RESERVE_SHIFT) | PN_GEMM_KSPLIT(31);
+  pn_gemm_desc d3{};
+  d3.A = t2; d3.lda = planes; d3.W = W3; d3.ldw = planes; d3.bias = b3;
+  d3.Res = idt; d3.ldres = Cout; d3.C = out; d3.ldc = Cout;
+  d3.M = (int)(M * B); d3.N = Cout; d3.K = planes; d3.batch = 1;
+  d3.flags = flags | PN_GEMM_RELU_AFTER_RES;
+  d3.splitk_scratch = splitk_scratch; d3.splitk_scratch_floats = splitk_scratch_floats;
+  pn_gemm_desc ds = d3;
+  ds.A = x; ds.lda = Cin; ds.W = Wsc; ds.ldw = Cin; ds.bias = bsc;
+  ds.Res = nullptr; ds.ldres = 0; ds.C = idt ? idt : out; ds.K = Cin; ds.flags = flags;
+  GemmP psc;
+  if (int rc = fill_conv_params(x, Wsc, bsc, nullptr, out, B, H, W, Cin, Cout, 1, 1, stride, 0,
+                                flags, &psc))
+    return rc;
+  GemmP p3;
+  if (int rc = fill_conv_params(t2, W3, b3, nullptr, out, B, 1, (int)M, planes, Cout, 1, 1, 1, 0,
+                                flags | PN_GEMM_RELU_AFTER_RES, &p3))
+    return rc;
+  hipStream_t s = (hipStream_t)stream;
+  int cps;
+  bool fused = gemm_single_chain(&d3);
+  if (stride == 1) fused = fused && gemm_single_chain(&ds);
+  else fused = fused && splitk_factor(psc, B, splitk_scratch, splitk_scratch_floats, &cps, flags) <= 1;
+  if (fused) {
+    GemmP both = p3;
+    both.K = Cin + planes;
+    fused = splitk_factor(both, B, splitk_scratch, splitk_scratch_floats, &cps, flags) <= 1;
+  }
+  if (!fused) {
+    if (!idt) return PN_BAD_ARG;
+    if (stride == 1) {
+      if (int rc = pn_gemm_f32(&ds, stream)) return rc;
+    } else if (int rc = pn_conv2d_nhwc_ex_f32(x, Wsc, bsc, nullptr, idt, B, H, W, Cin, Cout, 1, 1,
+                                              stride, 0, flags, splitk_scratch,
+                                              splitk_scratch_floats, stream)) {
+      return rc;
+    }
+    return pn_gemm_f32(&d3, stream);
+  }
+  const int64_t ntiles = (int64_t)pn_cdiv((int)M, 64) * pn_cdiv(Cout, 64) * B;
+  static const int wgs = resident_wgs(k_gemm_proj, PN_GEMM_WGS_PROJ, 256);
+  hipLaunchKernelGGL(k_gemm_proj, dim3(persistent_grid(ntiles, wgs, flags)), dim3(256), 0, s, p3,
+                     psc, B);
+  return PN_LAUNCH_CHECK();
 }
 
 extern "C" int pn_mask_stencil_gemm_f32(const float* me, int64_t ld_me, int64_t stride_me,
@@ -915,4 +1049,31 @@
   return PN_LAUNCH_CHECK();
 }
 
+extern "C" int pn_mask_stencil_gather_gemm_f32(const float* me, int64_t ld_me, int64_t stride_me,
+                                               const float* mf, int64_t ld_mf, int64_t stride_mf,
+                                               uint32_t* bits, int32_t* rowall, int B, int Q,
+                                               int Nk, int K, int hi, int wi, int ho, int wo,
+                                               int flags, void* stream) {
+  if (!me || !mf || !bits || !rowall || B <= 0 || Q <= 0 || Nk <= 0 || K <= 0 || K % 32)
+    return PN_BAD_ARG;
+  if (hi <= 0 || wi <= 0 || ho <= 0 || wo <= 0 || (int64_t)ho * wo != Nk) return PN_BAD_ARG;
+  if (ld_me % 4 || ld_mf % 4 || stride_me % 4 || stride_mf % 4 || !aligned16(me) || !aligned16(mf))
+    return PN_BAD_ARG;
+  const int64_t lim = (int64_t)1 << 29;
+  if ((int64_t)(Q - 1) * ld_me + K >= lim || ((int64_t)hi * wi - 1) * ld_mf + K >= lim)
+    return PN_BAD_ARG;
+  GemmP p{};
+  p.A = me; p.W = mf; p.lda = ld_me; p.ldw = ld_mf; p.sA = stride_me; p.sW = stride_mf;
+  p.M = Q; p.K = K; p.aadd_rows = 1;
+  p.N = pn_cdiv(Nk, 16) * 64;
+  const StencilP st{bits, rowall, Nk, hi, wi, ho, wo};
+  hipStream_t s = (hipStream_t)stream;
+  hipLaunchKernelGGL(k_fill_i32, dim3(pn_cdiv(B * Q, 256)), dim3(256), 0, s, rowall, 1, B * Q);
+  const int64_t ntiles = (int64_t)pn_cdiv(Q, 64) * (p.N / 64) * B;
+  static const int wgs = resident_wgs(k_gemm_stencil_gather, TileWgs<64, 64, A_ROW, false>::value, 256);
+  hipLaunchKernelGGL(k_gemm_stencil_gather, dim3(persistent_grid(ntiles, wgs, flags)), dim3(256), 0,
+                     s, p, st, B);
+  return PN_LAUNCH_CHECK();
+}
+
 extern "C" int pn_abi_version(void) { return PN_ABI_VERSION; }
diff --git a/pair-net_amd/csrc/norm.hip b/pair-net_amd/csrc/norm.hip
--- a/pair-net_amd/csrc/norm.hip
+++ b/pair-net_amd/csrc/norm.hip
@@ -136,6 +136,101 @@
   return PN_LAUNCH_CHECK();
 }
 
+#define GN_UP_CH 4
+__global__ __launch_bounds__(64 * GN_SUB) void k_gn_apply_up(
+    const float* __restrict__ x, const float* __restrict__ gamma, const float* __restrict__ beta,
+    float* __restrict__ y, const double* __restrict__ partials, const float* __restrict__ coarse,
+    int64_t HW, int Wf, int hc, int wc, int Hf, int G, float eps, int64_t xbs, int64_t ybs,
+    int64_t cbs) {
+  __shared__ double acc[GN_SUB][64];
+  __shared__ float stat[64][2];
+  const int tid = threadIdx.x, b = blockIdx.y;
+  const int nblk = gridDim.x;
+  {
+    const int col = tid & 63, part = tid >> 6;
+    double t = 0.0;
+    if (col < 2 * G)
+      for (int i = part; i < nblk; i += GN_SUB)
+        t += partials[((int64_t)b * nblk + i) * G * 2 + col];
+    acc[part][col] = t;
+  }
+  __syncthreads();
+  if (tid < G) {
+    const double n = (double)HW * (256 / G);
+    double s = 0.0, ss = 0.0;
+    for (int k = 0; k < GN_SUB; ++k) {
+      s += acc[k][2 * tid];
+      ss += acc[k][2 * tid + 1];
+    }
+    const double mean = s / n;
+    double var = ss / n - mean * mean;
+    if (var < 0.0) var = 0.0;
+    stat[tid][0] = (float)mean;
+    stat[tid][1] = (float)(1.0 / sqrt(var + (double)eps));
+  }
+  __syncthreads();
+  const int c4 = tid & 63, sub = tid >> 6;
+  const int g = (c4 * 4) / (256 / G);
+  const float mean = stat[g][0], rstd = stat[g][1];
+  const float4 gg = ld4(gamma + c4 * 4), bb = ld4(beta + c4 * 4);
+  const int64_t p0 = (int64_t)blockIdx.x * GN_PIX;
+  const float* xb = x + (int64_t)b * xbs;
+  float* yb = y + (int64_t)b * ybs;
+  const float* ib = coarse + (int64_t)b * cbs + c4 * 4;
+  const int64_t rs = (int64_t)wc * 256, cs = 256;
+  constexpr int NP = GN_PIX / GN_SUB;
+#pragma unroll
+  for (int j0 = 0; j0 < NP; j0 += GN_UP_CH) {
+    float4 v[GN_UP_CH], v00[GN_UP_CH], v01[GN_UP_CH], v10[GN_UP_CH], v11[GN_UP_CH];
+    Tap tys[GN_UP_CH], txs[GN_UP_CH];
+#pragma unroll
+    for (int j = 0; j < GN_UP_CH; ++j) {
+      const int pix = (int)min(p0 + sub + (j0 + j) * GN_SUB, HW - 1);
+      const int oy = pix / Wf, ox = pix - oy * Wf;
+      const Tap ty = make_tap(oy, hc, Hf), tx = make_tap(ox, wc, Wf);
+      tys[j] = ty; txs[j] = tx;
+      v[j] = ld4(xb + (int64_t)pix * 256 + c4 * 4);
+      v00[j] = ld4(ib + ty.i0 * rs + tx.i0 * cs); v01[j] = ld4(ib + ty.i0 * rs + tx.i1 * cs);
+      v10[j] = ld4(ib + ty.i1 * rs + tx.i0 * cs); v11[j] = ld4(ib + ty.i1 * rs + tx.i1 * cs);
+    }
+#pragma unroll
+    for (int j = 0; j < GN_UP_CH; ++j) {
+      const int64_t pix = p0 + sub + (j0 + j) * GN_SUB;
+      const Tap ty = tys[j], tx = txs[j];
+#define GN_O(c) fmaf((v[j].c - mean) * rstd, gg.c, bb.c)
+#define UP_R(c) fmaf(ty.l0, fmaf(tx.l1, v01[j].c, tx.l0 * v00[j].c), \
+                     ty.l1 * fmaf(tx.l0, v10[j].c, tx.l1 * v11[j].c))
+      float4 o = make_float4(GN_O(x), GN_O(y), GN_O(z), GN_O(w));
+      float4 r = make_float4(UP_R(x), UP_R(y), UP_R(z), UP_R(w));
+#undef GN_O
+#undef UP_R
+      asm volatile("" : "+v"(o.x), "+v"(o.y), "+v"(o.z), "+v"(o.w));
+      asm volatile("" : "+v"(r.x), "+v"(r.y), "+v"(r.z), "+v"(r.w));
+      if (pix < HW) st4(yb + pix * 256 + c4 * 4, add4(o, r));
+    }
+  }
+}
+
+extern "C" int pn_groupnorm_upadd_nhwc_f32(const float* x, const float* gamma, const float* beta,
+                                           float* y, double* partials, const float* coarse, int B,
+                                           int H, int W, int hc, int wc, int C, int G, float eps,
+                                           int64_t x_bstride, int64_t y_bstride,
+                                           int64_t coarse_bstride, void* stream) {
+  if (!x || !gamma || !beta || !y || !partials || !coarse) return PN_BAD_ARG;
+  if (C != 256 || G <= 0 || G > 32 || 256 % G || (256 / G) % 4 || B <= 0 || B > 65535 || H <= 0 ||
+      W <= 0 || hc <= 0 || wc <= 0)
+    return PN_BAD_ARG;
+  if ((x_bstride | y_bstride | coarse_bstride) & 3) return PN_BAD_ARG;
+  const int64_t HW = (int64_t)H * W;
+  if (HW >= ((int64_t)1 << 31)) return PN_BAD_ARG;
+  hipStream_t s = (hipStream_t)stream;
+  dim3 grid(pn_groupnorm_nblk(HW), B);
+  hipLaunchKernelGGL(k_gn_partial, grid, dim3(64 * GN_SUB), 0, s, x, partials, HW, G, x_bstride);
+  hipLaunchKernelGGL(k_gn_apply_up, grid, dim3(64 * GN_SUB), 0, s, x, gamma, beta, y, partials,
+                     coarse, HW, W, hc, wc, H, G, eps, x_bstride, y_bstride, coarse_bstride);
+  return PN_LAUNCH_CHECK();
+}
+
 __global__ __launch_bounds__(256) void k_l2norm256(const float* __restrict__ x,
                                                    float* __restrict__ y, int64_t rows,
                                                    float eps) {
diff --git a/pair-net_amd/head.py b/pair-net_amd/head.py
--- a/pair-net_amd/head.py
+++ b/pair-net_amd/head.py
@@ -104,6 +104,8 @@
         self.grid_reserve = 0
         self.fuse_ppn_front = True
         self.fuse_mask_pack = True
+        self.gather_mask_stencil = True
+        self.fuse_lateral_upadd = False
         self.enc_fused_ln = ("proj", "ffn")
         self.group_input_convs = False
         self.gemm_arithmetic = "bf16x3"
@@ -556,12 +558,18 @@
         hip.gemm(f, w[pd + "lateral_convs.0.conv.weight"], pl.T1, M=HW2, N=256, K=cin,
                  lda=cin if pl.nhwc else HW2, ldw=cin, ldc=256, batch=B, sA=cin * HW2,
                  sC=HW2 * 256, colmajor=not pl.nhwc)
-        hip.groupnorm_nhwc(pl.T1, w[pd + "lateral_convs.0.gn.weight"],
-                           w[pd + "lateral_convs.0.gn.bias"], pl.T2, pl.gn_part, B, HW2,
-                           self.gn_groups, False, HW2 * 256, HW2 * 256)
         h2, w2 = pl.shapes[2]
-        hip.bilinear_nhwc(pl.X[:, pl.start[2]:], pl.T2, B, h2, w2, H2, W2, 256, True, SN * 256,
-                          HW2 * 256)
+        if getattr(self, "fuse_lateral_upadd", False):
+            hip.groupnorm_upadd_nhwc(pl.T1, w[pd + "lateral_convs.0.gn.weight"],
+                                     w[pd + "lateral_convs.0.gn.bias"], pl.T2, pl.gn_part,
+                                     pl.X[:, pl.start[2]:], B, H2, W2, h2, w2, self.gn_groups,
+                                     HW2 * 256, HW2 * 256, SN * 256)
+        else:
+            hip.groupnorm_nhwc(pl.T1, w[pd + "lateral_convs.0.gn.weight"],
+                               w[pd + "lateral_convs.0.gn.bias"], pl.T2, pl.gn_part, B, HW2,
+                               self.gn_groups, False, HW2 * 256, HW2 * 256)
+            hip.bilinear_nhwc(pl.X[:, pl.start[2]:], pl.T2, B, h2, w2, H2, W2, 256, True, SN * 256,
+                              HW2 * 256)
         if self.conv_algo == "winograd4":
             hip.conv3x3_winograd43(pl.T2, w[pd + "output_convs.0.conv.winograd4"], None, pl.T1,
                                    pl.wV, pl.wM, B, H2, W2, 256, 256, False)
@@ -580,10 +588,14 @@
             for l, (h, wd) in enumerate(pl.shapes):
                 hip.bilinear_nhwc(pl.MF, pl.MFd[l], B, H2, W2, h, wd, 256, False, HW2 * 256,
                                   pl.N[l] * 256)
-        elif self.exact_mask_order != "full":
+        elif self.exact_mask_order != "full" and not self._gathers_stencil():
             for l, (h, wd) in enumerate(pl.shapes):
                 hip.bilinear_stencil_rows(pl.MF, pl.MFs[l], B, H2, W2, h, wd, 256, HW2 * 256,
                                           4 * pl.N[l] * 256)
+
+    def _gathers_stencil(self):
+        return bool(self.exact_mask_order and self.exact_mask_order != "full" and
+                    self.fuse_mask_pack and getattr(self, "gather_mask_stencil", True))
 
     def _encoder_fp32(self, pl):
         w, B, SN = self.w, pl.B, pl.SN
@@ -677,8 +689,12 @@
             hip.bilinear_planar(pl.MP if mp is None else mp, pl.ML, B * Q, pl.hw2[0], pl.hw2[1],
                                 h, wd)
         elif self.exact_mask_order and self.fuse_mask_pack:
-            hip.mask_stencil_gemm(pl.me if me is None else me, pl.MFs[lvl], pl.bits, pl.rowall,
-                                  B, Q, pl.hw2[0], pl.hw2[1], h, wd)
+            if self._gathers_stencil():
+                hip.mask_stencil_gather_gemm(pl.me if me is None else me, pl.MF, pl.bits,
+                                             pl.rowall, B, Q, pl.hw2[0], pl.hw2[1], h, wd)
+            else:
+                hip.mask_stencil_gemm(pl.me if me is None else me, pl.MFs[lvl], pl.bits,
+                                      pl.rowall, B, Q, pl.hw2[0], pl.hw2[1], h, wd)
             return
         elif self.exact_mask_order:
             hip.gemm(pl.me if me is None else me, pl.MFs[lvl], pl.ML4, M=Q, N=4 * n, K=256,
@@ -866,7 +882,8 @@
     def _run_stage(self, which, pl, feats=None):
         cfg = (self.exact_mask_order, self.conv_algo, self.fuse_ppn_front, self.grid_reserve,
                tuple(self.enc_fused_ln), self.group_input_convs,
-               getattr(self, "fuse_mask_pack", True), self.gemm_arithmetic, self.msda_s3_out)
+               getattr(self, "fuse_mask_pack", True), self.gemm_arithmetic, self.msda_s3_out,
+               getattr(self, "gather_mask_stencil", True), getattr(self, "fuse_lateral_upadd", False))
         if pl.graph_cfg != cfg:
             pl.graph_a = pl.graph_b = None
             pl.graphs_a = OrderedDict()
diff --git a/pair-net_amd/hip.py b/pair-net_amd/hip.py
--- a/pair-net_amd/hip.py
+++ b/pair-net_amd/hip.py
@@ -55,6 +55,7 @@
     "pn_gemm_group_f32": (C.c_int, [C.POINTER(GemmDesc), C.c_int, _vp]),
     "pn_conv2d_nhwc_f32": (C.c_int, [_vp, _vp, _vp, _vp] + [_i32] * 10 + [_vp]),
     "pn_conv2d_nhwc_ex_f32": (C.c_int, [_vp] * 5 + [_i32] * 10 + [_vp, _i64, _vp]),
+    "pn_bottleneck_proj_f32": (C.c_int, [_vp] * 8 + [_i32] * 8 + [_vp, _i64, _vp]),
     "pn_stem7x7s2_f32": (C.c_int, [_vp, _vp, _vp, _vp, _i32, _i32, _i32, _i32, _vp]),
     "pn_maxpool3x3s2_nhwc_f32": (C.c_int, [_vp, _vp, _i32, _i32, _i32, _i32, _vp]),
     "pn_winograd_f23_input_f32": (C.c_int, [_vp, _vp, _i32, _i32, _i32, _i32, _vp]),
@@ -72,6 +73,7 @@
     "pn_groupnorm_nblk": (C.c_int, [_i64]),
     "pn_groupnorm_nhwc_f32": (C.c_int, [_vp, _vp, _vp, _vp, _vp, _i32, _i64, _i32,
                                         _i32, _f32, _i32, _i64, _i64, _vp]),
+    "pn_groupnorm_upadd_nhwc_f32": (C.c_int, [_vp] * 6 + [_i32] * 7 + [_f32, _i64, _i64, _i64, _vp]),
     "pn_l2normalize_f32": (C.c_int, [_vp, _vp, _i64, _i32, _f32, _vp]),
     "pn_ffn_scratch_floats": (_i64, [_i32, _i32]),
     "pn_ffn_ln_f32": (C.c_int, [_vp] * 9 + [_i32, _i32, _i32, _f32, _vp]),
@@ -139,6 +141,8 @@
     "pn_mask_pack_stencil": (C.c_int, [_vp, _vp, _vp, _i64, _i32, _i32, _i32, _i32, _vp]),
     "pn_mask_stencil_gemm_f32": (C.c_int, [_vp, _i64, _i64, _vp, _i64, _i64, _vp, _vp] +
                                  [_i32] * 9 + [_vp]),
+    "pn_mask_stencil_gather_gemm_f32": (C.c_int, [_vp, _i64, _i64, _vp, _i64, _i64, _vp, _vp] +
+                                        [_i32] * 9 + [_vp]),
     "pn_bilinear_stencil_rows_f32": (C.c_int, [_vp, _vp] + [_i32] * 6 + [_i64, _i64, _vp]),
     "pn_attn_scratch_floats": (_i64, [_i32, _i32, _i32]),
     "pn_attention_f32": (C.c_int, [_vp, _i64, _vp, _i64, _vp, _i64, _vp, _vp, _vp,
@@ -188,7 +192,7 @@
                                                 _i32, _vp]),
 }
 EXPORTS = tuple(_SIGS)
-ABI_VERSION = 29
+ABI_VERSION = 30
 
 _lib = None
 
@@ -433,6 +437,20 @@
                        KH, KW, stride, pad, flags, _ptr(scratch),
                        scratch.numel() if scratch is not None else 0, _stream())),
            "pn_conv2d_nhwc_ex_f32")
+
+
+def bottleneck_proj(x, wsc, bsc, t2, w3, b3, idt, out, B, H, W, Cin, planes, stride,
+                    scratch=None):
+    Cout = w3.shape[0]
+    Ho, Wo = (H - 1) // stride + 1, (W - 1) // stride + 1
+    flops = 2.0 * B * Ho * Wo * Cout * (Cin + planes)
+    nbytes = 4.0 * (B * (Ho * Wo * (Cin + planes + Cout)) + Cout * (Cin + planes))
+    _check(_launch("k_gemm_proj", flops, nbytes,
+                   lambda: lib().pn_bottleneck_proj_f32(
+                       _ptr(x), _ptr(wsc), _ptr(bsc), _ptr(t2), _ptr(w3), _ptr(b3), _ptr(idt),
+                       _ptr(out), B, H, W, Cin, planes, Cout, stride, _reserve_flag(),
+                       _ptr(scratch), scratch.numel() if scratch is not None else 0, _stream())),
+           "pn_bottleneck_proj_f32")
 
 
 def stem7x7s2(img, wp, bias, out, B, H, W):
@@ -649,6 +667,14 @@
         256, G, eps, int(relu), x_bstride, y_bstride, _stream()), "pn_groupnorm_nhwc_f32")
 
 
+def groupnorm_upadd_nhwc(x, gamma, beta, out, partials, coarse, B, H, W, hc, wc, G, x_bstride,
+                         y_bstride, coarse_bstride, eps=1e-5):
+    _check(lib().pn_groupnorm_upadd_nhwc_f32(
+        _ptr(x), _ptr(gamma), _ptr(beta), _ptr(out), _ptr(partials, torch.float64), _ptr(coarse),
+        B, H, W, hc, wc, 256, G, eps, x_bstride, y_bstride, coarse_bstride, _stream()),
+        "pn_groupnorm_upadd_nhwc_f32")
+
+
 def ffn_scratch_floats(M, hidden):
     return lib().pn_ffn_scratch_floats(M, hidden)
 
@@ -754,6 +780,18 @@
                        _ptr(bits, torch.int32), _ptr(rowall, torch.int32), B, Q, Nk, K, hi, wi,
                        ho, wo, _reserve_flag(), _stream()),
                    meta=(Q, 4 * Nk, K, B, False)), "pn_mask_stencil_gemm_f32")
+
+
+def mask_stencil_gather_gemm(me, mf, bits, rowall, B, Q, hi, wi, ho, wo, K=256):
+    Nk = ho * wo
+    _check(_launch("k_gemm_stencil_gather", 2.0 * B * Q * 4 * Nk * K,
+                   4.0 * B * (Q * K + 4 * Nk * K) + B * Q * Nk / 8.0,
+                   lambda: lib().pn_mask_stencil_gather_gemm_f32(
+                       _ptr(me), me.stride(0), Q * me.stride(0), _ptr(mf), mf.stride(-2),
+                       mf.stride(0) if mf.dim() == 3 else hi * wi * mf.stride(-2),
+                       _ptr(bits, torch.int32), _ptr(rowall, torch.int32), B, Q, Nk, K, hi, wi,
+                       ho, wo, _reserve_flag(), _stream()),
+                   meta=(Q, 4 * Nk, K, B, False)), "pn_mask_stencil_gather_gemm_f32")
 
 
 def bilinear_stencil_rows(x, out, B, hi, wi, ho, wo, Cc, in_bstride, out_bstride):
```
